# RobotLocomotion/pytorch-dense-correspondence

Measured on AMD Instinct MI355X. Metric: training images/sec, 640x480 D=3 ResNet34-8s, higher is better.
Workload: dtype f32 (f16x3 products)

## Files before the change

include/dcn_hip.h:

```cpp
#ifndef DCN_HIP_H
#define DCN_HIP_H

#include <stddef.h>
#include <stdint.h>

#ifdef __cplusplus
extern "C" {
#endif

#define DCN_OK 0
#define DCN_E_INVALID (-1)
#define DCN_E_LAUNCH (-2)
#define DCN_E_UNSUPPORTED (-3)

const char* dcn_version(void);

void dcn_reload_env(void);

void dcn_release_pooled_buffers(void);


enum { DCN_LIST_MATCH = 0, DCN_LIST_MASKED = 1, DCN_LIST_BACKGROUND = 2, DCN_LIST_BLIND = 3, DCN_NUM_LISTS = 4 };

enum {
    DCN_COMPOSE_WITHIN_SCENE = 0,
    DCN_COMPOSE_DIFFERENT_OBJECT = 1,
    DCN_COMPOSE_ACROSS_SCENE = 2,
    DCN_COMPOSE_RAW_SUMS = 3
};

typedef struct dcn_loss_config {
    float margin[DCN_NUM_LISTS];
    int32_t invert[DCN_NUM_LISTS];
    int32_t pixel_weight[DCN_NUM_LISTS];
    float m_pixel;
    int32_t image_width;
    float match_loss_weight;
    float non_match_loss_weight;
    int32_t scale_by_hard_negatives;
    int32_t compose;
} dcn_loss_config;

size_t dcn_loss_workspace_bytes(int num_pairs, int64_t max_list_len);

int dcn_contrastive_loss_forward(const float* desc_a, const float* desc_b, int num_pairs, int64_t hw, int d,
                                 const int64_t* idx_a, const int64_t* idx_b, const int64_t* offsets_host,
                                 const int64_t* offsets_dev, const dcn_loss_config* cfg, float* terms, float* sums,
                                 int32_t* hard_neg, float* loss, float* per_term, int32_t* status, void* workspace,
                                 void* stream);

int dcn_contrastive_loss_backward(const float* desc_a, const float* desc_b, int num_pairs, int64_t hw, int d,
                                  const int64_t* idx_a, const int64_t* idx_b, const int64_t* offsets_host,
                                  const int64_t* offsets_dev, const dcn_loss_config* cfg, const float* sums,
                                  const int32_t* hard_neg, const float* grad_loss, const float* pair_grad,
                                  float* grad_a, float* grad_b, void* stream);

size_t dcn_loss_saved_floats(int64_t total_pairs, int d);
int dcn_contrastive_loss_forward_save(const float* desc_a, const float* desc_b, int num_pairs, int64_t hw, int d,
                                      const int64_t* idx_a, const int64_t* idx_b, const int64_t* offsets_host,
                                      const int64_t* offsets_dev, const dcn_loss_config* cfg, float* terms, float* sums,
                                      int32_t* hard_neg, float* loss, float* per_term, int32_t* status, void* workspace,
                                      float* pair_records, void* stream);
int dcn_contrastive_loss_backward_saved(int num_pairs, int64_t hw, int d, const int64_t* idx_a, const int64_t* idx_b,
                                        const int64_t* offsets_host, const int64_t* offsets_dev, const dcn_loss_config* cfg,
                                        const int32_t* hard_neg, const float* grad_loss, const float* pair_records,
                                        int prefilled, float* grad_a, float* grad_b, void* stream);

size_t dcn_loss_exact_workspace_bytes(int num_pairs, int64_t hw, int d);
int dcn_contrastive_loss_backward_saved_exact(int num_pairs, int64_t hw, int d, const int64_t* idx_a, const int64_t* idx_b,
                                              const int64_t* offsets_host, const int64_t* offsets_dev,
                                              const dcn_loss_config* cfg, const int32_t* hard_neg, const float* grad_loss,
                                              const float* pair_records, void* workspace, float* grad_a, float* grad_b,
                                              void* stream);
int dcn_fill_bytes(void* p, int byte_value, size_t n, void* stream);

#define DCN_LOSS_NUM_TYPES 5
#define DCN_LOSS_BAD_INDEX 1
#define DCN_LOSS_BAD_TYPE 2
#define DCN_LOSS_BAD_BOUNDS 4
#define DCN_LOSS_BAD_PIXEL_LAYOUT 8
int dcn_contrastive_loss_mixed_forward(const float* desc_a, const float* desc_b, int num_pairs, int64_t hw, int d,
                                       const int64_t* idx_a, const int64_t* idx_b, const int64_t* offsets_dev,
                                       const int32_t* types_dev, const dcn_loss_config* cfgs, int64_t max_list_len,
                                       int64_t max_pair_len, int64_t capacity, float* terms, float* sums, int32_t* hard_neg,
                                       float* loss, int32_t* num_valid, int32_t* status, void* workspace, float* pair_records,
                                       void* stream);
int dcn_contrastive_loss_mixed_backward_saved(int num_pairs, int64_t hw, int d, const int64_t* idx_a, const int64_t* idx_b,
                                              const int64_t* offsets_dev, const int32_t* types_dev, const dcn_loss_config* cfgs,
                                              int64_t max_list_len, int64_t max_pair_len, int64_t capacity,
                                              const int32_t* hard_neg, const int32_t* num_valid, const float* grad_loss,
                                              const float* pair_records, int prefilled, float* grad_a, float* grad_b,
                                              void* stream);
int dcn_contrastive_loss_mixed_backward_saved_exact(int num_pairs, int64_t hw, int d, const int64_t* idx_a, const int64_t* idx_b,
                                                    const int64_t* offsets_dev, const int32_t* types_dev,
                                                    const dcn_loss_config* cfgs, int64_t max_list_len, int64_t max_pair_len,
                                                    int64_t capacity, const int32_t* hard_neg, const int32_t* num_valid,
                                                    const float* grad_loss, const float* pair_records, void* workspace,
                                                    float* grad_a, float* grad_b, void* stream);

size_t dcn_triplet_loss_workspace_bytes(int64_t n);
int dcn_triplet_loss_forward(const float* desc_a, const float* desc_b, int64_t hw, int d, const int64_t* non_a,
                             const int64_t* match_b, const int64_t* non_b, int64_t n, int64_t n_match, float alpha,
                             float* loss, int32_t* status, void* workspace, void* stream);
int dcn_triplet_loss_backward(const float* desc_a, const float* desc_b, int64_t hw, int d, const int64_t* non_a,
                              const int64_t* match_b, const int64_t* non_b, int64_t n, int64_t n_match, float alpha,
                              const float* grad_loss, float* grad_a, float* grad_b, void* stream);


typedef struct dcn_plan dcn_plan;

int dcn_plan_create(const char* arch, int base_width, int n, int h, int w, int d, dcn_plan** out);
int dcn_plan_create_grouped(const char* arch, int base_width, int n, int groups, int h, int w, int d, dcn_plan** out);
void dcn_plan_destroy(dcn_plan* plan);
int dcn_plan_forget_saved(dcn_plan* plan, const void* saved);
int dcn_plan_num_forward_records(const dcn_plan* plan);

#define DCN_CONV_FP32 0
#define DCN_CONV_F16X3 1
int dcn_plan_set_conv_mode(dcn_plan* plan, int mode);
int dcn_plan_conv_mode(const dcn_plan* plan);

int dcn_plan_num_params(const dcn_plan* plan);
int dcn_plan_num_bn(const dcn_plan* plan);
int dcn_plan_param_info(const dcn_plan* plan, int i, char* name, int name_cap, int64_t shape[4], int* ndim);
int dcn_plan_bn_info(const dcn_plan* plan, int j, char* name, int name_cap, int64_t* channels);

int dcn_plan_fused_bn_backward(const dcn_plan* plan);

int dcn_plan_num_activation_slots(const dcn_plan* plan);
size_t dcn_plan_activation_absmax_offset(const dcn_plan* plan);

int dcn_plan_num_grad_buckets(const dcn_plan* plan);
int dcn_plan_grad_bucket_first_param(const dcn_plan* plan, int k);
int dcn_plan_stream_wait_grad_bucket(dcn_plan* plan, int k, void* stream);

size_t dcn_plan_saved_bytes(const dcn_plan* plan);
size_t dcn_plan_workspace_bytes(const dcn_plan* plan);
double dcn_plan_forward_flops(const dcn_plan* plan);

int dcn_backbone_forward(dcn_plan* plan, const float* image, const float* const* params,
                         float* const* bn_running, float momentum, float eps, int training, int normalize,
                         float* descriptors, void* saved, void* workspace, void* stream);

int dcn_backbone_forward_pair(dcn_plan* plan, const float* image_a, const float* image_b, const float* const* params,
                              float* const* bn_running, float momentum, float eps, int training, int normalize,
                              float* descriptors, void* saved, void* workspace, void* stream);

int dcn_plan_profile_begin(dcn_plan* plan);
int dcn_plan_profile_end(dcn_plan* plan, double ms[2], int64_t launches[2], double flops[2]);
int dcn_plan_profile_end3(dcn_plan* plan, double ms[3], int64_t launches[3], double flops[3]);
enum {
    DCN_PROF_GEMM = 0,
    DCN_PROF_WGRAD = 1,
    DCN_PROF_GEMM_HL = 2,
    DCN_PROF_BN_APPLY = 3,
    DCN_PROF_BN_BWD_REDUCE = 4,
    DCN_PROF_BN_BWD_APPLY = 5,
    DCN_PROF_BN_FINALIZE = 6,
    DCN_PROF_RESAMPLE = 7,
    DCN_PROF_OTHER = 8,
    DCN_PROF_NCAT = 9
};
int dcn_plan_profile_end_all(dcn_plan* plan, double ms[DCN_PROF_NCAT], int64_t launches[DCN_PROF_NCAT],
                             double work[DCN_PROF_NCAT]);

int dcn_backbone_backward(dcn_plan* plan, const float* grad_descriptors, const float* const* params,
                          const void* saved, void* workspace, float* const* grads, int normalize, void* stream);
int dcn_backbone_backward_pair(dcn_plan* plan, const float* grad_a, const float* grad_b, const float* const* params,
                               const void* saved, void* workspace, float* const* grads, int normalize, void* stream);


typedef struct dcn_conv_desc {
    int32_t n, hin, win, cin;
    int32_t hout, wout, cout;
    int32_t kh, kw, stride, pad, dil;
    int32_t ldc;
    int32_t group_rows;
} dcn_conv_desc;

int dcn_conv_forward(const dcn_conv_desc* c, const float* in, const float* w, const float* bias, float* out,
                     float* bn_partial, void* workspace, void* stream);
size_t dcn_conv_gemm_workspace(const dcn_conv_desc* c, int dgrad);
int dcn_conv_num_mtiles(const dcn_conv_desc* c);
int dcn_conv_dgrad(const dcn_conv_desc* c, const float* dout, const float* wt, const float* add, float* din,
                   void* workspace, void* stream);
int dcn_conv_wgrad(const dcn_conv_desc* c, const float* in, const float* dout, float* dw, void* slabs, void* stream);
size_t dcn_conv_wgrad_workspace(const dcn_conv_desc* c);
int dcn_transpose_weight(const float* w, float* wt, int cout, int taps, int cin, int ldn, void* stream);

int dcn_f16_kpad(int k);
int dcn_split_rows_f16(const float* w, void* hi, void* lo, int64_t rows, int k, float scale, void* stream);
int dcn_conv_num_mtiles_f16(const dcn_conv_desc* c);
size_t dcn_conv_gemm_workspace_f16(const dcn_conv_desc* c, int dgrad);
int dcn_conv_forward_f16(const dcn_conv_desc* c, const float* in, const float* in_absmax, const void* w_hi, const void* w_lo,
                         float w_scale, const float* bias, float* out, float* bn_partial, void* workspace, void* stream);
int dcn_conv_dgrad_f16(const dcn_conv_desc* c, const float* dout, const void* wt_hi, const void* wt_lo, float w_scale,
                       const float* dout_absmax, const float* add, float* din, void* workspace, void* stream);
int dcn_conv_dgrad_bn_num_mtiles_f16(const dcn_conv_desc* c);
int dcn_conv_dgrad_bn_f16(const dcn_conv_desc* c, const float* dout, const void* wt_hi, const void* wt_lo, float w_scale,
                          const float* dout_absmax, const float* add, float* din, const float* bn_x,
                          const unsigned char* relu_mask, const float* bn_stats, float* bn_partial, void* workspace,
                          void* stream);

int dcn_split_weights_checked_f16(int n, const float* const* w, const float* const* row_scale, void* const* hi, void* const* lo,
                                  const int* cout, const int* taps, const int* cin, float scale, int* status, void* stream);

int dcn_conv_hl_eligible(const dcn_conv_desc* c, int dgrad);
int dcn_conv_num_mtiles_hl(const dcn_conv_desc* c);
int dcn_conv_tile_rows_hl(const dcn_conv_desc* c, int dgrad);
size_t dcn_conv_gemm_workspace_hl(const dcn_conv_desc* c, int dgrad);
int dcn_conv_hl_shape_info(const dcn_conv_desc* c, int dgrad, int* info6);
int dcn_split_act_hl32(const float* src, const float* absmax, void* dst, int64_t rows, int channels, void* stream);
int dcn_split_weights_hl32(int n, const float* const* w, void* const* out, const int* cout, const int* taps, const int* cin,
                           const int* ldn, int transposed, float scale, void* stream);
int dcn_conv_forward_hl(const dcn_conv_desc* c, const void* in_hl, const float* in_absmax, const void* w_hl, float w_scale,
                        const float* bias, float* out, float* bn_partial, void* workspace, void* stream);
int dcn_conv_dgrad_hl(const dcn_conv_desc* c, const void* dout_hl, const void* wt_hl, float w_scale, const float* dout_absmax,
                      const float* add, float* din, void* workspace, void* stream);

int dcn_conv_wgrad_hl_eligible(const dcn_conv_desc* c);
int dcn_conv_wgrad_hl_kind(const dcn_conv_desc* c);
size_t dcn_conv_wgrad_workspace_hl(const dcn_conv_desc* c);
int dcn_conv_wgrad_hl(const dcn_conv_desc* c, const void* x_hl, const float* x_absmax, const void* dout_hl,
                      const float* dout_absmax, float* dw, void* slabs, void* stream);

int dcn_split_stem_weights_f16(const float* w4, void* hi, void* lo, int cout, float scale, void* stream);
int dcn_conv_stem_forward_f16(const dcn_conv_desc* c, const float* in, const float* in_absmax, const void* w_hi, const void* w_lo,
                              float w_scale, float* out, float* bn_partial, void* stream);

int dcn_split_weights_f16(int n, const float* const* w, void* const* hi, void* const* lo, const int* cout, const int* taps,
                          const int* cin, const int* ldn, int transposed, float scale, void* stream);

int dcn_split_weights_scaled_f16(int n, const float* const* w, const float* const* row_scale, void* const* hi,
                                 void* const* lo, const int* cout, const int* taps, const int* cin, const int* ldn,
                                 int transposed, float scale, void* stream);
int dcn_conv_forward_fused_f16(const dcn_conv_desc* c, const float* in, const float* in_absmax, const void* w_hi,
                               const void* w_lo, float w_scale, const float* bias, const float* add, int relu, float* out,
                               float* out_absmax, void* workspace, void* stream);

int dcn_split_act_f16(const float* src, void* xs, int64_t n, void* stream);
size_t dcn_grad_blocked_bytes(int m, int ld);
int dcn_split_grad_blocked_f16(const float* dy, int m, int ld, const float* absmax, void* dq, void* stream);
int dcn_conv_wgrad_f16(const dcn_conv_desc* c, const void* xs, int xs_is_fp32, const float* x_absmax, const void* dq,
                       const float* dout_absmax, float* dw, void* slabs, void* stream);
size_t dcn_conv_wgrad_workspace_f16(const dcn_conv_desc* c);

int dcn_bn_forward(const float* x, const float* bn_partial, int mtiles, int c, int64_t rows, const float* gamma,
                   const float* beta, float* running_mean, float* running_var, float momentum, float eps, int training,
                   const float* res, int relu, float* y, unsigned char* relu_mask, float* stats, void* stream);
size_t dcn_bn_backward_workspace(int64_t rows, int c);
int dcn_bn_backward(const float* dy, const unsigned char* relu_mask, const float* x, const float* stats, const float* gamma,
                    int c, int64_t rows, float* dgamma, float* dbeta, float* dx, float* g_out, void* workspace,
                    void* stream);
int dcn_bn_backward_from_partial(const float* dy, const float* bn_partial, int mtiles, const float* x, const float* stats,
                                 const float* gamma, int c, int64_t rows, float* dgamma, float* dbeta, float* dx,
                                 void* workspace, void* stream);
size_t dcn_bn_backward_full_workspace(int64_t rows, int c, int groups);
int dcn_bn_backward_full(const float* dy, const float* dy2, const float* relu_out, const unsigned char* relu_mask,
                         const float* x, const float* stats, const float* gamma, int c, int64_t rows, int groups,
                         float* dgamma, float* dbeta, float* dx, float* g_out, float* absmax, void* dq, void* hl_dx,
                         int keep_dx, void* workspace, void* stream);
int dcn_maxpool_forward(const float* in, int n, int hin, int win, int c, float* out, unsigned char* argmax, void* stream);
int dcn_maxpool_backward(const float* gout, const unsigned char* argmax, int n, int hin, int win, int c, float* gin,
                         void* stream);

int dcn_upsample_forward(const float* low, int n, int hl, int wl, int ldl, int d, int h, int w, int normalize,
                         float* out, void* stream);
int dcn_upsample_backward(const float* gout, int n, int hl, int wl, int ldl, int d, int h, int w, float* glow,
                          float* tmp, void* stream);
size_t dcn_upsample_backward_tmp_bytes(int n, int hl, int w, int d);

int dcn_maxpool_forward_full(const float* in, const float* bn_stats, int groups, int n, int hin, int win, int c, float* out,
                             unsigned char* argmax, unsigned char* relu_mask, void* stream);
int dcn_maxpool_backward_full(const float* gout, const float* gout2, const unsigned char* argmax, int n, int hin, int win, int c,
                              float* gin, void* stream);
int dcn_normalize_backward(const float* low, int n, int hl, int wl, int ldl, int d, int h, int w, const float* gout, float* gv,
                           void* stream);
int dcn_upsample_backward_full(const float* gout, const float* gout_b, int n, int hl, int wl, int ldl, int d, int h, int w,
                               float* glow, float* tmp, float* absmax, void* stream);
int dcn_image_to_nhwc4(const float* img, int n, int hw, float* out, float* absmax, void* stream);
int dcn_pad_c3_to_c4(const float* src, float* dst, int64_t rows, void* stream);
int dcn_unpad_c4_to_c3(const float* src, float* dst, int64_t rows, void* stream);
int dcn_pad_rows(const float* src, float* dst, int64_t rows, int d, int ld, void* stream);
int dcn_column_sums(const float* m, int64_t rows, int ld, int d, float* out, void* stream);

size_t dcn_match_statistics_workspace(int q);
int dcn_match_statistics(const float* res, int64_t hw, int w, int d, const float* queries, const int64_t* gt_idx, int q,
                         const unsigned char* mask, int64_t* best_idx, float* best_dist, int32_t* count, float* dist_sum,
                         float* gt_dist, void* workspace, void* stream);

int dcn_find_best_match(const float* res, int64_t hw, int d, const float* queries, int q, const unsigned char* mask,
                        int64_t* best_idx, float* best_dist, float* norm_diffs, void* workspace, void* stream);
size_t dcn_find_best_match_workspace(int q);

size_t dcn_find_correspondences_workspace(int64_t n);
int dcn_find_correspondences(const uint16_t* depth_a, const uint16_t* depth_b, int h, int w, const float* K,
                             const float* K_inv, const float* pose_a, const float* pose_b_inv, const int64_t* cand_u,
                             const int64_t* cand_v, int64_t n, int64_t* out_ua, int64_t* out_va, float* out_ub,
                             float* out_vb, int64_t* out_count, void* workspace, void* stream);
size_t dcn_mask_nonzero_workspace(int64_t hw);
int dcn_mask_nonzero(const float* mask, int64_t hw, int64_t* list, int64_t* count, void* workspace, void* stream);
int dcn_sample_pixels(const float* rand, int64_t n, int w, int h, const int64_t* list, const int64_t* count, float* u,
                      float* v, void* stream);

int dcn_adam_step(int n, void* const* param, const void* const* grad, void* const* exp_avg, void* const* exp_avg_sq,
                  const int64_t* numel, double lr, double beta1, double beta2, double eps, double weight_decay,
                  int64_t step, void* stream);

#define DCN_AUG_PARAM_WORDS 16
#define DCN_AUG_FLIP_V 1
#define DCN_AUG_FLIP_H 2
#define DCN_AUG_RANDOMIZE 4
#define DCN_AUG_GRADIENT 8
#define DCN_AUG_VERTICAL 16
#define DCN_AUG_NOISE 32
#define DCN_UV_INT64 0
#define DCN_UV_FLOAT32 1
int dcn_augment_images(int n, int h, int w, const uint8_t* rgb_a, const uint8_t* rgb_b, const uint8_t* mask_a,
                       const uint8_t* mask_b, const int32_t* params, const uint8_t* noise, const float* mean,
                       const float* std, float* net_a, float* net_b, uint8_t* rgb_out_a, uint8_t* rgb_out_b,
                       float* mask_out_a, float* mask_out_b, void* stream);
int dcn_flip_planes(const void* in, void* out, int64_t planes, int h, int w, int bytes_per_pixel, int flip_v, int flip_h,
                    void* stream);
int dcn_flip_uv(int uv_dtype, const void* u_in, const void* v_in, void* u_out, void* v_out, int64_t count, int n_images,
                const int64_t* offsets, const int32_t* params, int flags, int h, int w, void* stream);

#define DCN_MERGE_FG_A 0
#define DCN_MERGE_FG_B 1
#define DCN_MERGE_DROP_EMPTY 1
#define DCN_MERGE_BAD_INDEX 1
#define DCN_MERGE_BAD_OFFSETS 2
int dcn_merge_images(int n, int frames, int h, int w, const int32_t* foreground, const uint8_t* rgb_a1, const uint8_t* rgb_b1,
                     const uint8_t* rgb_a2, const uint8_t* rgb_b2, const uint8_t* mask_a1, const uint8_t* mask_b1,
                     const uint8_t* mask_a2, const uint8_t* mask_b2, const float* mean, const float* std, float* net_1,
                     float* net_2, float* mask_1, float* mask_2, uint8_t* rgb_1, uint8_t* rgb_2, void* stream);
size_t dcn_merge_prune_workspace(int n, int64_t count_a, int64_t count_b);
int dcn_merge_prune(int n, int h, int w, const int32_t* foreground, const uint8_t* mask_a1, const uint8_t* mask_b1,
                    const uint8_t* mask_a2, const uint8_t* mask_b2, const int64_t* u_a1, const int64_t* v_a1,
                    const int64_t* u_a2, const int64_t* v_a2, const int64_t* offsets_a, int64_t count_a, const int64_t* u_b1,
                    const int64_t* v_b1, const int64_t* u_b2, const int64_t* v_b2, const int64_t* offsets_b, int64_t count_b,
                    int flags, int64_t* u_1, int64_t* v_1, int64_t* u_2, int64_t* v_2, int64_t* offsets, uint8_t* empty,
                    int32_t* status, void* workspace, void* stream);

#define DCN_SAMPLE_CAM_FLOATS 50
#define DCN_SAMPLE_SITES 6
#define DCN_SAMPLE_SITE_CAND 0
#define DCN_SAMPLE_SITE_MASKED 1
#define DCN_SAMPLE_SITE_BACKGROUND 2
#define DCN_SAMPLE_SITE_BLIND 3
#define DCN_SAMPLE_SITE_ACROSS_A 4
#define DCN_SAMPLE_SITE_ACROSS_B 5
#define DCN_SAMPLE_ONLY_OFF_MASK 1
#define DCN_SAMPLE_MASK_INV 2
#define DCN_SAMPLE_BAD_INDEX 1
#define DCN_SAMPLE_BAD_DRAWS 2
#define DCN_SAMPLE_BAD_OFFSETS 4
size_t dcn_sample_workspace(int n, int h, int w, int64_t attempts, int64_t match_slots);
int dcn_within_scene_samples(int n, int h, int w, const uint16_t* depth_a, const uint16_t* depth_b, const uint8_t* mask_a,
                             const uint8_t* mask_b, const float* cams, int64_t attempts, int k_masked, int k_background,
                             int flags, const int32_t* aug_params, const int64_t* seeds, const float* rand,
                             const int64_t* rand_offsets, int data_type, int64_t* idx_a, int64_t* idx_b, int64_t capacity,
                             int64_t* offsets, uint8_t* empty, int32_t* type, int32_t* status, void* workspace, void* stream);
int dcn_complete_samples(int n, int h, int w, const int64_t* u_a, const int64_t* v_a, const void* u_b, const void* v_b,
                         int uv_b_dtype, const int64_t* list_offsets, int64_t count, const uint8_t* mask_a,
                         const uint8_t* mask_b, int k_masked, int k_background, int flags, const int32_t* aug_params,
                         const int64_t* seeds, const float* rand, const int64_t* rand_offsets, int data_type, int64_t* idx_a,
                         int64_t* idx_b, int64_t capacity, int64_t* offsets, uint8_t* empty, int32_t* type, int32_t* status,
                         void* workspace, void* stream);
int dcn_across_scene_samples(int n, int h, int w, const uint8_t* mask_a, const uint8_t* mask_b, int64_t num_samples,
                             const int32_t* aug_params, const int64_t* seeds, const float* rand, const int64_t* rand_offsets,
                             int data_type, int64_t* idx_a, int64_t* idx_b, int64_t capacity, int64_t* offsets, uint8_t* empty,
                             int32_t* type, int32_t* status, void* workspace, void* stream);

#define DCN_CONCAT_MAX_GROUPS 8
int dcn_concat_samples(int groups, const int* n, const int64_t* const* idx_a, const int64_t* const* idx_b,
                       const int64_t* const* offsets, const int64_t* capacity_in, const int32_t* const* status_in,
                       int64_t* idx_a_out, int64_t* idx_b_out, int64_t capacity, int64_t* offsets_out, int32_t* status,
                       void* stream);

#define DCN_SYNTHETIC_DATA_TYPE 4
#define DCN_SYNTHETIC_SITES 4
#define DCN_SYNTHETIC_SITE_CAND_A 0
#define DCN_SYNTHETIC_SITE_CAND_B 1
#define DCN_SYNTHETIC_SITE_MASKED 2
#define DCN_SYNTHETIC_SITE_BACKGROUND 3
size_t dcn_synthetic_workspace(int n, int h, int w, int64_t attempts);
int dcn_synthetic_samples(int n, int h, int w, const uint16_t* depth, const uint8_t* mask, const uint8_t* rgb,
                          const float* cams, int64_t attempts, int k_masked, int k_background, int flags,
                          const int32_t* foreground, const uint8_t* empty_in, const int64_t* seeds, const float* rand,
                          const int64_t* rand_offsets, const float* mean, const float* std, float* net_1, float* net_2,
                          float* mask_1, float* mask_2, int64_t* idx_a, int64_t* idx_b, int64_t capacity, int64_t* offsets,
                          uint8_t* empty, int32_t* type, int32_t* status, void* workspace, void* stream);

struct dcn_frame_store {
    int64_t num_frames;
    int32_t num_scenes, num_objects, num_multi, h, w;
    const uint8_t* rgb;
    const uint16_t* depth;
    const uint8_t* mask;
    const int32_t* scene_first_frame;
    const int32_t* scene_object;
    const int32_t* object_scene_offsets;
    const int32_t* object_scenes;
    const int32_t* multi_scenes;
    const float* scene_cams;
    const double* poses;
};
#define DCN_FRAME_CAM_FLOATS 18
#define DCN_FRAME_SLOTS 4
#define DCN_FRAME_DRAW_OBJECT_A 0
#define DCN_FRAME_DRAW_OBJECT_B 1
#define DCN_FRAME_DRAW_SCENE_A 2
#define DCN_FRAME_DRAW_SCENE_B 3
#define DCN_FRAME_DRAW_SCENE_B2 4
#define DCN_FRAME_DRAW_FRAME_A 5
#define DCN_FRAME_DRAW_FRAME_B 6
#define DCN_FRAME_DRAW_HEADER 8
#define DCN_FRAME_BAD_INDEX 1
#define DCN_FRAME_BAD_DRAWS 2
#define DCN_FRAME_NO_CANDIDATES 4
int dcn_select_frames(int n, int data_type, const struct dcn_frame_store* store, int num_attempts, double threshold,
                      double angle_threshold, const int64_t* seeds, const int32_t* draws, int32_t* frames, uint8_t* empty,
                      int32_t* scenes, int32_t* objects, int32_t* status, void* stream);
int dcn_gather_frames(int n, int frames_per_pair, const struct dcn_frame_store* store, const int32_t* frames,
                      const uint8_t* empty, uint8_t* rgb, uint16_t* depth, uint8_t* mask, float* cams, int32_t* status,
                      void* stream);

#define DCN_EVAL_COLUMNS 13
#define DCN_EVAL_COL_NORM_DIFF_DESCRIPTOR_GROUND_TRUTH 0
#define DCN_EVAL_COL_NORM_DIFF_DESCRIPTOR 1
#define DCN_EVAL_COL_NORM_DIFF_DESCRIPTOR_MASKED 2
#define DCN_EVAL_COL_NORM_DIFF_GROUND_TRUTH_3D 3
#define DCN_EVAL_COL_NORM_DIFF_PRED_3D 4
#define DCN_EVAL_COL_NORM_DIFF_PRED_3D_MASKED 5
#define DCN_EVAL_COL_PIXEL_MATCH_ERROR_L2 6
#define DCN_EVAL_COL_PIXEL_MATCH_ERROR_L2_MASKED 7
#define DCN_EVAL_COL_PIXEL_MATCH_ERROR_L1 8
#define DCN_EVAL_COL_FRACTION_CLOSER 9
#define DCN_EVAL_COL_FRACTION_CLOSER_MASKED 10
#define DCN_EVAL_COL_AVERAGE_L2_FALSE_POSITIVES 11
#define DCN_EVAL_COL_AVERAGE_L2_FALSE_POSITIVES_MASKED 12
#define DCN_EVAL_BAD_INDEX 1
#define DCN_EVAL_BAD_OFFSETS 2
#define DCN_EVAL_BAD_DRAWS 4
#define DCN_EVAL_BAD_FRAME 8
size_t dcn_eval_matches_workspace(int n, int h, int w, int64_t attempts);
int dcn_eval_matches(int n, int h, int w, const uint16_t* depth_a, const uint16_t* depth_b, const uint8_t* mask_a,
                     const float* cams, int64_t attempts, const int64_t* seeds, const float* rand, const int64_t* rand_offsets,
                     int num_matches, const int32_t* match_order, const int64_t* order_seeds, int64_t* u_a, int64_t* v_a,
                     float* u_b, float* v_b, int64_t* offsets, int32_t* totals, int32_t* status, void* workspace, void* stream);
size_t dcn_match_statistics_pairs_workspace(int64_t max_rows);
int dcn_match_statistics_pairs(int p, int h, int w, int d, const float* res_a, const float* res_b, const uint8_t* mask_b,
                               const uint16_t* depth_a, const uint16_t* depth_b, const float* cams, const int64_t* u_a,
                               const int64_t* v_a, const float* u_b, const float* v_b, const int64_t* offsets, int64_t max_rows,
                               int max_pair_rows, double* columns, uint8_t* is_valid, int32_t* pred_uv, int32_t* closer,
                               int32_t* row_pair, int32_t* mask_pixels, int32_t* status, void* workspace, void* stream);

#define DCN_ACROSS_TOO_FEW_MASK_PIXELS 16
size_t dcn_across_object_queries_workspace(int p, int h, int w);
int dcn_across_object_queries(int p, int h, int w, int d, const uint8_t* mask_a, const float* res_a, int q,
                              const int32_t* sample_order, const int64_t* order_seeds, int64_t* u_a, int64_t* v_a,
                              float* queries, int64_t* offsets, int32_t* mask_pixels, int32_t* status, void* workspace,
                              void* stream);
size_t dcn_best_match_pairs_workspace(int64_t max_rows);
int dcn_best_match_pairs(int p, int h, int w, int d, const float* res_b, const float* queries, const int64_t* offsets,
                         int64_t max_rows, int max_pair_rows, float* norm_diff, int32_t* best_uv, int32_t* row_pair,
                         int32_t* status, void* workspace, void* stream);

int dcn_reproject_pixels(int v, const struct dcn_frame_store* store, const float* kcam, const int32_t* requests,
                         uint8_t* found, float* u2, float* v2, int32_t* uv, int32_t* status, void* stream);
size_t dcn_match_statistics_groups_workspace(int64_t max_rows);
int dcn_match_statistics_groups(int g, int h, int w, int d, const float* res_b, const uint8_t* mask_b, const uint16_t* depth_b,
                                const float* queries, const int64_t* u_a, const int64_t* v_a, const uint16_t* depth_q,
                                const float* u_b, const float* v_b, const float* cams, const uint8_t* keep,
                                const int64_t* offsets, int64_t max_rows, int max_group_rows, double* columns,
                                uint8_t* is_valid, int32_t* pred_uv, int32_t* closer, int32_t* row_pair, int32_t* mask_pixels,
                                int32_t* status, void* workspace, void* stream);
int dcn_match_statistics_groups_wide(int g, int h, int w, int d, const float* res_b, const uint8_t* mask_b,
                                     const uint16_t* depth_b, const float* queries, const int64_t* u_a, const int64_t* v_a,
                                     const uint16_t* depth_q, const float* u_b, const float* v_b, const float* cams,
                                     const uint8_t* keep, const int64_t* offsets, int64_t max_rows, int max_group_rows,
                                     int64_t strip_pixels, double* columns, uint8_t* is_valid, int32_t* pred_uv, int32_t* closer,
                                     int32_t* row_pair, int32_t* mask_pixels, int32_t* status, void* workspace, void* stream);

size_t dcn_descriptor_statistics_workspace(int n, int h, int w, int d);
int dcn_descriptor_statistics(int n, int h, int w, int d, const float* res, const uint8_t* mask, float* per_image,
                              int32_t* mask_pixels, void* workspace, void* stream);
int dcn_descriptor_statistics_combine(int n, int d, const float* per_image, const int32_t* mask_pixels, int num_images,
                                      float* stats, int32_t* used, void* stream);

struct dcn_train_state {
    int32_t active;
    int32_t reserved;
    int64_t t;
    double lr;
    float step_size;
    float bc2_sqrt;
    int64_t num_active;
    int64_t num_skipped;
};
#define DCN_TRAIN_LOG_COLUMNS 16
int dcn_train_advance(struct dcn_train_state* state, const int32_t* types, int B, int64_t iteration,
                      int64_t steps_between_decay, double decay, double beta1, double beta2, void* stream);
int dcn_adam_step_guarded(int n, void* const* param, const void* const* grad, void* const* exp_avg, void* const* exp_avg_sq,
                          const int64_t* numel, double eps, double weight_decay, double beta1, double beta2,
                          const struct dcn_train_state* state, void* stream);
int dcn_guarded_copy(int n, void* const* dst, const void* const* src, const int64_t* bytes,
                     const struct dcn_train_state* state, int when_active, void* stream);
int dcn_train_log(double* history, int64_t row, int64_t iteration, const struct dcn_train_state* state, const float* loss,
                  const float* terms, const int32_t* types, int B, void* stream);
int dcn_train_advance_ranks(struct dcn_train_state* state, const int32_t* types_all , int G, int B, int rank,
                            float* weight_out , int64_t iteration, int64_t steps_between_decay, double decay,
                            double beta1, double beta2, void* stream);
int dcn_train_log_ranks(double* history, int64_t row, int64_t iteration, const struct dcn_train_state* state,
                        const float* gathered , const int32_t* types_all , int G, int B,
                        void* stream);

#define DCN_CURVE_SUMMARY_DOUBLES 8
#define DCN_CURVE_EMPTY 1
#define DCN_CURVE_NAN 2
#define DCN_CURVE_NONFINITE 4
int dcn_eval_curves(int c, int64_t rows, int64_t ld, const double* values ,
                    const int32_t* row_pair , const uint8_t* drop_nan ,
                    int num_bins, int64_t* cumcount , double* cdf ,
                    double* summary , int32_t* status , void* stream);

#define DCN_PICTURE_EMPTY_RANGE 1
#define DCN_HEAT_WORKSPACE_BYTES 2048
#define DCN_NORM_NONE 0
#define DCN_NORM_PAIR 1
#define DCN_NORM_MASKED_PAIR 2
#define DCN_NORM_STATS 3
#define DCN_NORM_STATS_MASKED 4
#define DCN_NORM_SCALAR 5
struct dcn_picture_family {
    int32_t mode;
    int32_t picture_channels;
    int32_t channel[3];
    int32_t reserved;
    const double* stats;
    void* normed;
    void* picture;
    int64_t side_stride, pair_stride;
};
size_t dcn_descriptor_ranges_workspace(int p, int h, int w, int d);
int dcn_descriptor_ranges(int p, int h, int w, int d, const float* res_a, const float* res_b, const uint8_t* mask_a,
                          const uint8_t* mask_b, float* image_ranges, float* pair_ranges, float* scalar_ranges,
                          int32_t* status, void* workspace, void* stream);
int dcn_descriptor_normalize(int p, int h, int w, int d, const float* res_a, const float* res_b, const uint8_t* mask_a,
                             const uint8_t* mask_b, const float* pair_ranges, const float* scalar_ranges,
                             const struct dcn_picture_family* families , void* stream);
int dcn_heat_maps(int p, int h, int w, int d, const float* res_b, const float* queries, const int64_t* offsets,
                  int64_t max_rows, float variance, const uint8_t* colour_table, uint8_t* out, int32_t* status,
                  void* workspace, void* stream);

#ifdef __cplusplus
}
#endif
#endif
```

pytorch-dense-correspondence_amd/csrc/backbone_engine.hip:

```cpp
#include <algorithm>
#include <cstdio>
#include <cstdlib>
#include <cstring>
#include <mutex>
#include <string>
#include <vector>

#include "dcn_tuning.h"
#include "elementwise_kernels.h"

namespace {

using dcn::ceil_div;

struct ConvL {
    double flops = 0;
    dcn_conv_desc d;
    int w = -1, b = -1;
    int bn = -1;
    size_t x = 0;
    int cin_true = 0;
    size_t wsplit = 0;
    size_t whl = 0;
    bool hl_any = false;
// ... 525 lines not shown
            obs.begin = [](void* c, int cat, double bytes, hipStream_t s) { prof_open(*(dcn_plan*)c, cat, bytes, s); };
            obs.end = [](void* c, hipStream_t s) { prof_close(*(dcn_plan*)c, s); };
            if (on) dcn::launch_observer = &obs;
        }
        ~ObserverGuard() { if (on) dcn::launch_observer = outer; }
    };
    template <class F> int other(F&& launch) { return timed(DCN_PROF_OTHER, 0.0, launch); }

    void* SK(const ConvL& c, int dgrad, Kernel k) const {
        const size_t need = k == Kernel::FP32 ? dcn_conv_gemm_workspace(&c.d, dgrad) : k == Kernel::HL ? dcn_conv_gemm_workspace_hl(&c.d, dgrad)
                                                                                                       : dcn_conv_gemm_workspace_f16(&c.d, dgrad);
        return need <= p.sk_bytes ? (void*)(ws + p.w_sk) : nullptr;
    }
    float* S(size_t off) const { return saved + off; }
    float* A(int a) const { return (p.conv_mode == DCN_CONV_F16X3 && a >= 0) ? saved + p.s_actmax + a : nullptr; }
    unsigned char* M(size_t off) const {
        for (const auto& m : p.relu_masks)
            if (m.first == off) return (unsigned char*)(saved + m.second);
        return nullptr;
    }
    float* Wk(size_t off) const { return ws + off; }
    const float* P(int i) const { return params[i]; }

    int conv_fwd(const ConvL& c, const float* in, const float* w, const float* bias, float* out, float* part) {
        const Kernel k = rt[c.idx].fwd;
        if (k == Kernel::FP32)
            return timed(0, c.flops, [&] { return dcn_conv_forward(&c.d, in, w, bias, out, part, SK(c, 0, k), st); });
        if (k == Kernel::STEM8) {
            _Float16* hi = (_Float16*)Wk(p.w_stem8);
            return timed(0, c.flops, [&] {
                return dcn_conv_stem_forward_f16(&c.d, in, A(c.in_act), hi, hi + (size_t)p.base * 224, kWeightScale, out, part, st);
            });
        }
        if (k == Kernel::HL) {
            return timed(2, c.flops, [&] {
                const float* img = saved_hl_of(in);
                if (!img) {
                    int k = hl_src[0] == in ? 0 : (hl_src[1] == in ? 1 : -1);
                    if (k < 0) {
                        k = 0;
                        DCN_TRY(dcn_split_act_hl32(in, A(c.in_act), hlbuf(0), (int64_t)c.d.n * c.d.hin * c.d.win, c.d.cin, st));
                        hl_src[0] = in;
                    }
                    img = hlbuf(k);
                }
                return dcn_conv_forward_hl(&c.d, img, A(c.in_act), whl(c), kWeightScale, bias, out, part, SK(c, 0, k), st);
            });
        }
        return timed(0, c.flops, [&] {
            return dcn_conv_forward_f16(&c.d, in, A(c.in_act), wimg(p.w_wh, c), wimg(p.w_wl, c), kWeightScale, bias, out, part,
                                        SK(c, 0, k), st);
        });
    }

    float* wh_over = nullptr;
    float* wl_over = nullptr;
    float* whl_over = nullptr;
    void* wimg(size_t plane, const ConvL& c) const {
        float* base = plane == p.w_wh ? (wh_over ? wh_over : Wk(p.w_wh)) : (wl_over ? wl_over : Wk(p.w_wl));
        return (void*)((_Float16*)base + c.wsplit);
    }

    int ensure_saved_hl(const float* y, float* slot, int64_t rows, int C, int act) {
        if (!slot || dcn::tuning().hl_producers != 0) return DCN_OK;
        return other([&] { return dcn_split_act_hl32(y, A(act), slot, rows, C, st); });
    }
    void* whl(const ConvL& c) const { return (void*)((whl_over ? whl_over : Wk(p.w_whl)) + c.whl); }
    float* hlbuf(int k) const { return Wk(k == 0 ? p.w_hl : p.w_hl2); }
    void* hl_image_for(const float* y, int k, const ConvL* consumer_a, const ConvL* consumer_b = nullptr, float* slot = nullptr) {
        if (slot) {
            hl_saved.emplace_back(y, slot);
            return dcn::tuning().hl_producers != 0 ? (void*)slot : nullptr;
        }
        if (dcn::tuning().hl_producers == 0) return nullptr;
        const bool want = (consumer_a && rt[consumer_a->idx].fwd == Kernel::HL) || (consumer_b && rt[consumer_b->idx].fwd == Kernel::HL);
        if (!want) return nullptr;
        hl_src[k] = y;
        return hlbuf(k);
    }
    int fwd_mtiles(const ConvL& c) const {
        const Kernel k = rt[c.idx].fwd;
        return k == Kernel::FP32 ? dcn_conv_num_mtiles(&c.d) : k == Kernel::HL ? dcn_conv_num_mtiles_hl(&c.d) : dcn_conv_num_mtiles_f16(&c.d);
    }
    int split_hl_weights(bool transposed) {
        std::vector<const float*> w;
        std::vector<void*> out;
        std::vector<int> cout, taps, cin, ldn;
        for (const ConvL& c : p.convs) {
            if ((transposed ? rt[c.idx].dgrad : rt[c.idx].fwd) != Kernel::HL) continue;
            w.push_back(P(c.w));
            out.push_back(whl(c));
            cout.push_back(c.d.cout); taps.push_back(c.d.kh * c.d.kw); cin.push_back(c.d.cin); ldn.push_back(c.d.ldc);
        }
        if (w.empty()) return DCN_OK;
        return other([&] {
            return dcn_split_weights_hl32((int)w.size(), w.data(), out.data(), cout.data(), taps.data(), cin.data(), ldn.data(),
                                          transposed ? 1 : 0, kWeightScale, st);
        });
    }

    int split_all_weights(bool transposed, const float* stem_w, bool fold_bn = false) {
        const int n = (int)p.convs.size();
        std::vector<const float*> w, rs;
        std::vector<void*> hi, lo;
        std::vector<int> cout, taps, cin, ldn;
        for (int i = 0; i < n; ++i) {
            const ConvL& c = p.convs[i];
            if (transposed && i == p.stem) continue;
            w.push_back(i == p.stem ? stem_w : P(c.w));
            rs.push_back(fold_bn && c.bn >= 0 ? S(p.bns[c.bn].stats) : nullptr);
            hi.push_back(wimg(p.w_wh, c));
            lo.push_back(wimg(p.w_wl, c));
            cout.push_back(c.d.cout); taps.push_back(c.d.kh * c.d.kw); cin.push_back(c.d.cin); ldn.push_back(c.d.ldc);
        }
        if (!transposed)
            return other([&] {
                return dcn_split_weights_checked_f16((int)w.size(), w.data(), fold_bn ? rs.data() : nullptr, hi.data(), lo.data(),
                                                     cout.data(), taps.data(), cin.data(), kWeightScale,
                                                     (int*)(S(p.s_actmax) + p.n_act), st);
            });
        return other([&] {
            return dcn_split_weights_scaled_f16((int)w.size(), w.data(), nullptr, hi.data(), lo.data(), cout.data(), taps.data(),
                                                cin.data(), ldn.data(), 1, kWeightScale, st);
        });
    }

    int conv_fused(const ConvL& c, const float* in, const float* add, int relu, float* out, int out_act) {
        const float* shift = S(p.bns[c.bn].stats) + p.bns[c.bn].C;
        return timed(0, c.flops, [&] {
            return dcn_conv_forward_fused_f16(&c.d, in, A(c.in_act), wimg(p.w_wh, c), wimg(p.w_wl, c), kWeightScale, shift, add,
                                              relu, out, A(out_act), SK(c, 0, Kernel::F16), st);
        });
    }

    int conv_bn(const ConvL& c, const float* in, const float* w, float* const* bn_running, float momentum, float eps,
                int training, int out_act, int res_act = -1) {
        float* part = training ? Wk(p.w_part) : nullptr;
        DCN_TRY(conv_fwd(c, in, w, nullptr, S(c.x), part));
        const BnL& b = p.bns[c.bn];
        float* stats = S(b.stats);
        float* rm = bn_running ? bn_running[2 * b.idx] : nullptr;
        float* rv = bn_running ? bn_running[2 * b.idx + 1] : nullptr;
        if (!training && (!rm || !rv)) return DCN_E_INVALID;
        const int mtiles = fwd_mtiles(c);
        dcn::launch_bn_finalize(part, mtiles / p.groups, p.groups, b.C, (double)(b.rows / p.groups), P(b.g),
                                P(b.b), rm, rv, momentum, eps, training, stats, training ? A(out_act) : nullptr,
                                training ? A(res_act) : nullptr, st);
        return DCN_OK;
    }
};

}

extern "C" int dcn_plan_create(const char* arch, int base_width, int n, int h, int w, int d, dcn_plan** out) {
    return dcn_plan_create_grouped(arch, base_width, n, 1, h, w, d, out);
}
extern "C" int dcn_plan_create_grouped(const char* arch, int base_width, int n, int groups, int h, int w, int d,
                                       dcn_plan** out) {
    if (!arch || !out || n < 1 || h < 8 || w < 8 || d < 1 || base_width < 4 || (base_width % 4) || groups < 1 ||
        groups > 2 || (n % groups))
        return DCN_E_INVALID;
    dcn_plan* p = new dcn_plan();
    p->arch = arch; p->N = n; p->H = h; p->W = w; p->D = d; p->base = base_width; p->groups = groups;
    const dcn::Tuning& tune = dcn::tuning();
    if (tune.conv_mode_invalid) { delete p; return DCN_E_INVALID; }
    if (tune.conv_mode >= 0) p->conv_mode = tune.conv_mode;
    const int rc = build_plan(*p);
    if (rc != DCN_OK) { delete p; return rc; }
    *out = p;
    return DCN_OK;
}
extern "C" int dcn_plan_forget_saved(dcn_plan* plan, const void* saved) {
    if (!plan) return DCN_E_INVALID;
    int n = 0;
    for (size_t i = 0; i < plan->fwd_records.size();)
        if (plan->fwd_records[i].saved == saved) { plan->fwd_records.erase(plan->fwd_records.begin() + i); ++n; }
        else ++i;
    return n;
}

extern "C" int dcn_plan_num_forward_records(const dcn_plan* plan) {
    return plan ? (int)plan->fwd_records.size() : DCN_E_INVALID;
}

extern "C" void dcn_plan_destroy(dcn_plan* plan) {
    if (!plan) return;
    for (hipEvent_t e : plan->prof_ev) hipEventDestroy(e);
    for (hipEvent_t e : {plan->ev_dq[0], plan->ev_dq[1], plan->ev_wg[0], plan->ev_wg[1], plan->ev_join, plan->ev_ws[0], plan->ev_ws[1]})
        if (e) hipEventDestroy(e);
    for (hipEvent_t e : plan->ev_bucket)
        if (e) hipEventDestroy(e);
    if (plan->ev_bucket_side) hipEventDestroy(plan->ev_bucket_side);
    delete plan;
}
extern "C" int dcn_plan_set_conv_mode(dcn_plan* plan, int mode) {
    if (!plan || (mode != DCN_CONV_FP32 && mode != DCN_CONV_F16X3)) return DCN_E_INVALID;
    plan->conv_mode = mode;
    return DCN_OK;
}
extern "C" int dcn_plan_conv_mode(const dcn_plan* plan) { return plan ? plan->conv_mode : DCN_E_INVALID; }
extern "C" int dcn_plan_profile_begin(dcn_plan* plan) {
    if (!plan) return DCN_E_INVALID;
    plan->prof_on = true;
    plan->prof_used = 0;
    plan->prof_cat.clear();
    plan->prof_flops.clear();
    return DCN_OK;
}
extern "C" int dcn_plan_profile_end_all(dcn_plan* plan, double ms[DCN_PROF_NCAT], int64_t launches[DCN_PROF_NCAT],
                                        double work[DCN_PROF_NCAT]) {
    if (!plan || !ms || !launches || !work) return DCN_E_INVALID;
    plan->prof_on = false;
    for (int c = 0; c < DCN_PROF_NCAT; ++c) { ms[c] = 0; launches[c] = 0; work[c] = 0; }
    int rc = DCN_OK;
    for (size_t i = 0; i < plan->prof_cat.size(); ++i) {
        hipEvent_t e0 = plan->prof_ev[2 * i], e1 = plan->prof_ev[2 * i + 1];
        float t = 0.f;
        if (hipEventSynchronize(e1) != hipSuccess || hipEventElapsedTime(&t, e0, e1) != hipSuccess) { rc = DCN_E_LAUNCH; break; }
        const int c = plan->prof_cat[i];
        if (c < 0 || c >= DCN_PROF_NCAT) continue;
        for (int k : {c == DCN_PROF_GEMM_HL ? (int)DCN_PROF_GEMM : c, c == DCN_PROF_GEMM_HL ? (int)DCN_PROF_GEMM_HL : -1}) {
            if (k < 0) continue;
            ms[k] += (double)t;
            launches[k] += 1;
            work[k] += plan->prof_flops[i];
        }
    }
    plan->prof_used = 0;
    plan->prof_cat.clear();
    plan->prof_flops.clear();
    return rc;
}
extern "C" int dcn_plan_profile_end3(dcn_plan* plan, double ms[3], int64_t launches[3], double flops[3]) {
    if (!ms || !launches || !flops) return DCN_E_INVALID;
    double m[DCN_PROF_NCAT], f[DCN_PROF_NCAT];
    int64_t n[DCN_PROF_NCAT];
    const int rc = dcn_plan_profile_end_all(plan, m, n, f);
    for (int c = 0; c < 3; ++c) { ms[c] = m[c]; launches[c] = n[c]; flops[c] = f[c]; }
    return rc;
}
extern "C" int dcn_plan_profile_end(dcn_plan* plan, double ms[2], int64_t launches[2], double flops[2]) {
    if (!ms || !launches || !flops) return DCN_E_INVALID;
    double m3[3], f3[3];
    int64_t n3[3];
    const int rc = dcn_plan_profile_end3(plan, m3, n3, f3);
    for (int c = 0; c < 2; ++c) { ms[c] = m3[c]; launches[c] = n3[c]; flops[c] = f3[c]; }
    return rc;
}
extern "C" int dcn_plan_num_params(const dcn_plan* plan) { return plan ? (int)plan->params.size() : DCN_E_INVALID; }
extern "C" int dcn_plan_num_bn(const dcn_plan* plan) { return plan ? (int)plan->bns.size() : DCN_E_INVALID; }
extern "C" int dcn_plan_param_info(const dcn_plan* plan, int i, char* name, int name_cap, int64_t shape[4], int* ndim) {
    if (!plan || i < 0 || i >= (int)plan->params.size() || !name || name_cap < 2 || !shape || !ndim) return DCN_E_INVALID;
    const ParamInfo& pi = plan->params[i];
    snprintf(name, (size_t)name_cap, "%s", pi.name.c_str());
    for (int k = 0; k < 4; ++k) shape[k] = pi.shape[k];
    *ndim = pi.ndim;
    return DCN_OK;
}
extern "C" int dcn_plan_bn_info(const dcn_plan* plan, int j, char* name, int name_cap, int64_t* channels) {
    if (!plan || j < 0 || j >= (int)plan->bns.size() || !name || name_cap < 2 || !channels) return DCN_E_INVALID;
    snprintf(name, (size_t)name_cap, "%s", plan->bns[j].name.c_str());
    *channels = plan->bns[j].C;
    return DCN_OK;
}
extern "C" int dcn_plan_num_grad_buckets(const dcn_plan* plan) { return plan ? (int)plan->bucket_first.size() : DCN_E_INVALID; }
extern "C" int dcn_plan_grad_bucket_first_param(const dcn_plan* plan, int k) {
    if (!plan || k < 0 || k >= (int)plan->bucket_first.size()) return DCN_E_INVALID;
    return plan->bucket_first[k];
}
extern "C" int dcn_plan_stream_wait_grad_bucket(dcn_plan* plan, int k, void* stream) {
    if (!plan || k < 0 || k >= (int)plan->bucket_first.size()) return DCN_E_INVALID;
    if (plan->bucket_state != 1) return DCN_E_UNSUPPORTED;
    return hipStreamWaitEvent((hipStream_t)stream, plan->ev_bucket[k], 0) == hipSuccess ? DCN_OK : DCN_E_LAUNCH;
}
extern "C" int dcn_plan_fused_bn_backward(const dcn_plan* plan) { return plan ? plan->fused_bn_bwd : DCN_E_INVALID; }
extern "C" int dcn_plan_num_activation_slots(const dcn_plan* plan) { return plan ? plan->n_act : DCN_E_INVALID; }
extern "C" size_t dcn_plan_activation_absmax_offset(const dcn_plan* plan) { return plan ? plan->s_actmax * sizeof(float) : 0; }
extern "C" size_t dcn_plan_saved_bytes(const dcn_plan* plan) { return plan ? plan->saved_floats * sizeof(float) : 0; }
extern "C" size_t dcn_plan_workspace_bytes(const dcn_plan* plan) { return plan ? plan->ws_floats * sizeof(float) : 0; }
extern "C" double dcn_plan_forward_flops(const dcn_plan* plan) { return plan ? plan->flops : 0.0; }

extern "C" int dcn_column_sums(const float* m, int64_t rows, int ld, int d, float* out, void* stream) {
    if (!m || !out || rows < 1 || d < 1 || ld < d) return DCN_E_INVALID;
    hipLaunchKernelGGL(colsum_kernel, dim3(d), dim3(1024), 0, (hipStream_t)stream, m, rows, ld, out);
    return dcn::check_launch();
}

namespace {

int forward_impl(dcn_plan* plan, const float* image, const float* image_b, const float* const* params,
                 float* const* bn_running, float momentum, float eps, int training, int normalize,
                 float* descriptors, void* saved, void* workspace, void* stream) {
    if (!plan || !image || !params || !descriptors || !saved || !workspace) return DCN_E_INVALID;
    dcn_plan& p = *plan;
    if (image_b && p.groups != 2) return DCN_E_INVALID;
    const std::vector<ConvRoute> routes = conv_routes(p, p.conv_mode);
    Run R{p, params, (float*)saved, (float*)workspace, (hipStream_t)stream, routes};
    Run::ObserverGuard observe(p);
    hipStream_t st = R.st;
    const int N = p.N;

    DCN_TRY(R.other([&] { return dcn::fill_bytes_async(R.S(p.s_actmax), 0, ((size_t)p.n_act + 1) * sizeof(float), st); }));
    const ConvL& stem = p.convs[p.stem];
    if (image_b) {
        dcn::launch_nchw3_to_nhwc4(image, R.S(p.s_in4), N / 2, p.H * p.W, R.A(stem.in_act), st);
        dcn::launch_nchw3_to_nhwc4(image_b, R.S(p.s_in4) + (size_t)(N / 2) * p.H * p.W * 4, N / 2, p.H * p.W, R.A(stem.in_act), st);
    } else {
        dcn::launch_nchw3_to_nhwc4(image, R.S(p.s_in4), N, p.H * p.W, R.A(stem.in_act), st);
    }
    dcn::launch_pad_c3_to_c4(R.P(stem.w), R.Wk(p.w_wstem), (int64_t)p.base * 49, st);
    dcn_plan::FwdRecord rec;
    rec.saved = saved;
    rec.conv_mode = p.conv_mode;
    rec.mid_hl_only.assign(p.convs.size(), 0);
    const bool fused_eval = !training && p.conv_mode == DCN_CONV_F16X3;
    const bool f16_mode = p.conv_mode == DCN_CONV_F16X3;
    if (fused_eval) {
        if (!bn_running) return DCN_E_INVALID;
        for (const BnL& b : p.bns) {
            if (!bn_running[2 * b.idx] || !bn_running[2 * b.idx + 1]) return DCN_E_INVALID;
            dcn::launch_bn_finalize(nullptr, 0, p.groups, b.C, (double)(b.rows / p.groups), R.P(b.g), R.P(b.b),
                                    bn_running[2 * b.idx], bn_running[2 * b.idx + 1], momentum, eps, 0, R.S(b.stats), nullptr,
                                    nullptr, st);
        }
        DCN_TRY(R.split_all_weights(false, R.Wk(p.w_wstem), true));
        DCN_TRY(R.conv_fused(stem, R.S(p.s_in4), nullptr, 1, R.S(p.s_stem_y), p.blocks[0].act_in));
        {
            const BnL& b = p.bns[stem.bn];
            const int hp = (stem.d.hout + 2 - 3) / 2 + 1, wp = (stem.d.wout + 2 - 3) / 2 + 1;
            dcn::launch_maxpool_fwd(R.S(p.s_stem_y), R.S(p.s_pool), (unsigned char*)R.S(p.s_argmax), N, stem.d.hout,
                                    stem.d.wout, hp, wp, b.C, st);
        }
        for (const BlockL& blk : p.blocks) {
            const float* in = R.S(blk.in);
            const float* cur = in;
            for (int i = 0; i + 1 < blk.nconv; ++i) {
                DCN_TRY(R.conv_fused(p.convs[blk.conv[i]], cur, nullptr, 1, R.S(blk.mid[i]), blk.act_mid[i]));
                cur = R.S(blk.mid[i]);
            }
            const ConvL& last = p.convs[blk.conv[blk.nconv - 1]];
            const float* res = in;
            if (blk.down >= 0) {
                const ConvL& dc = p.convs[blk.down];
                DCN_TRY(R.conv_fused(dc, in, nullptr, 0, R.S(dc.x), -1));
                res = R.S(dc.x);
            }
            DCN_TRY(R.conv_fused(last, cur, res, 1, R.S(blk.out), blk.act_out));
        }
    } else {
    const bool stem8 = routes[p.stem].fwd == Kernel::STEM8;
    bool hoist = training && f16_mode && stem8 && !p.prof_on && dcn::tuning().wsplit_overlap != 0 && ensure_side(p);
    if (hoist) {
        hipStreamCaptureStatus cs = hipStreamCaptureStatusNone;
        if (hipStreamIsCapturing(st, &cs) != hipSuccess || cs != hipStreamCaptureStatusNone) hoist = false;
    }
    SideFork side(p, st, p.ev_ws[1]);
    if (p.conv_mode == DCN_CONV_F16X3) {
        if (hoist) {
            Run Rs{p, params, (float*)saved, (float*)workspace, p.side, routes};
            if (!side.fork(p.ev_ws[0])) return DCN_E_LAUNCH;
            DCN_TRY(Rs.split_all_weights(false, Rs.Wk(p.w_wstem)));
            DCN_TRY(Rs.split_hl_weights(false));
            Rs.wh_over = Rs.S(p.s_wht); Rs.wl_over = Rs.S(p.s_wlt); Rs.whl_over = Rs.S(p.s_whlt);
            DCN_TRY(Rs.split_all_weights(true, nullptr));
            DCN_TRY(Rs.split_hl_weights(true));
            rec.wt_saved = true;
            if (!side.record(p.ev_ws[1], p.side)) return DCN_E_LAUNCH;
        } else {
            DCN_TRY(R.split_all_weights(false, R.Wk(p.w_wstem)));
            DCN_TRY(R.split_hl_weights(false));
        }
    }
    if (stem8) {
        _Float16* hi = (_Float16*)R.Wk(p.w_stem8);
        DCN_TRY(R.other([&] { return dcn_split_stem_weights_f16(R.Wk(p.w_wstem), hi, hi + (size_t)p.base * 224, p.base, kWeightScale, st); }));
    }
    DCN_TRY(R.conv_bn(stem, R.S(p.s_in4), R.Wk(p.w_wstem), bn_running, momentum, eps, training, p.blocks[0].act_in));
    {
        const BnL& b = p.bns[stem.bn];
        const float* s = R.S(b.stats);
        const int hp = (stem.d.hout + 2 - 3) / 2 + 1, wp = (stem.d.wout + 2 - 3) / 2 + 1;
        if (dcn::tuning().stem_pool_fused != 0) {
            dcn::launch_maxpool_fwd(R.S(stem.x), R.S(p.s_pool), (unsigned char*)R.S(p.s_argmax), N, stem.d.hout, stem.d.wout, hp,
                                    wp, b.C, st, s, p.groups, R.M(p.s_stem_y));
        } else {
            dcn::launch_bn_apply({.x = R.S(stem.x), .stats = s, .C = b.C, .rows = b.rows, .groups = p.groups, .y = R.S(p.s_stem_y),
                                  .relu_mask = R.M(p.s_stem_y)}, st);
            dcn::launch_maxpool_fwd(R.S(p.s_stem_y), R.S(p.s_pool), (unsigned char*)R.S(p.s_argmax), N, stem.d.hout,
                                    stem.d.wout, hp, wp, b.C, st);
        }
    }
    if (hoist && !side.join_wait(p.ev_ws[1])) return DCN_E_LAUNCH;
    if (training && f16_mode && p.blocks[0].has_hl_in) {
        const BlockL& b0 = p.blocks[0];
        R.hl_saved.emplace_back(R.S(b0.in), R.S(b0.hl_in));
        DCN_TRY(R.other([&] { return dcn_split_act_hl32(R.S(b0.in), R.A(b0.act_in), R.S(b0.hl_in), b0.in_rows, b0.in_c, st); }));
    }
    for (const BlockL& blk : p.blocks) {
        const float* in = R.S(blk.in);
        const float* cur = in;
        if (blk.down >= 0) {
            const ConvL& dc = p.convs[blk.down];
            DCN_TRY(R.conv_bn(dc, in, R.P(dc.w), bn_running, momentum, eps, training, blk.act_down));
        }
        for (int i = 0; i < blk.nconv; ++i) {
            const ConvL& c = p.convs[blk.conv[i]];
            if (i + 1 < blk.nconv) {
                DCN_TRY(R.conv_bn(c, cur, R.P(c.w), bn_running, momentum, eps, training, blk.act_mid[i]));
                const BnL& b = p.bns[c.bn];
                const float* s = R.S(b.stats);
                float* slot = (training && f16_mode && blk.has_hl_mid[i]) ? R.S(blk.hl_mid[i]) : nullptr;
                const ConvL& nxt = p.convs[blk.conv[i + 1]];
                void* hl = training ? R.hl_image_for(R.S(blk.mid[i]), 1, &nxt, nullptr, slot) : nullptr;
                const bool hl_only = hl && slot && hl == (void*)slot && (b.C % 32) == 0 && dcn::tuning().hl_only_mid != 0 &&
                                     routes[nxt.idx].fwd == Kernel::HL && routes[nxt.idx].wgrad == Kernel::HL;
                rec.mid_hl_only[nxt.idx] = hl_only ? 1 : 0;
                dcn::launch_bn_apply({.x = R.S(c.x), .stats = s, .C = b.C, .rows = b.rows, .groups = p.groups,
                                      .y = hl_only ? nullptr : R.S(blk.mid[i]), .relu_mask = R.M(blk.mid[i]), .hl_out = hl,
                                      .hl_absmax = R.A(blk.act_mid[i])}, st);
                DCN_TRY(R.ensure_saved_hl(R.S(blk.mid[i]), slot, b.rows, b.C, blk.act_mid[i]));
                cur = R.S(blk.mid[i]);
            } else {
                DCN_TRY(R.conv_bn(c, cur, R.P(c.w), bn_running, momentum, eps, training, blk.act_out,
                                  blk.down >= 0 ? blk.act_down : blk.act_in));
            }
        }
        const ConvL& last = p.convs[blk.conv[blk.nconv - 1]];
        const BnL& bl = p.bns[last.bn];
        const float* sl = R.S(bl.stats);
        const BlockL* nb = (&blk != &p.blocks.back()) ? &blk + 1 : nullptr;
        float* slot = (training && f16_mode && nb && nb->has_hl_in) ? R.S(nb->hl_in) : nullptr;
        void* hl = (training && nb) ? R.hl_image_for(R.S(blk.out), 0, &p.convs[nb->conv[0]], nb->down >= 0 ? &p.convs[nb->down] : nullptr,
                                                     slot)
                                    : nullptr;
        const ConvL* dc = blk.down >= 0 ? &p.convs[blk.down] : nullptr;
        dcn::launch_bn_apply({.x = R.S(last.x), .stats = sl, .C = bl.C, .rows = bl.rows, .groups = p.groups,
                              .res = dc ? R.S(dc->x) : in, .res_stats = dc ? R.S(p.bns[dc->bn].stats) : nullptr, .y = R.S(blk.out),
                              .relu_mask = R.M(blk.out), .hl_out = hl, .hl_absmax = R.A(blk.act_out)}, st);
        DCN_TRY(R.ensure_saved_hl(R.S(blk.out), slot, bl.rows, bl.C, blk.act_out));
    }
    }
    const ConvL& fc = p.convs[p.fc];
    const size_t low_bytes = (size_t)N * p.hl * p.wl * p.Dp * sizeof(float);
    DCN_TRY(R.other([&] { return dcn::fill_bytes_async(R.S(p.s_low), 0, low_bytes, st); }));
    DCN_TRY(R.conv_fwd(fc, R.S(p.blocks.back().out), R.P(fc.w), R.P(fc.b), R.S(p.s_low), nullptr));
    dcn::launch_upsample_fwd(R.S(p.s_low), N, p.hl, p.wl, p.Dp, p.D, p.H, p.W, normalize, descriptors, st);
    DCN_TRY(R.other([&] {
        hipLaunchKernelGGL(act_status_kernel, dim3(1), dim3(64), 0, st, (const float*)R.S(p.s_actmax), p.n_act,
                           (int*)(R.S(p.s_actmax) + p.n_act));
        return dcn::check_launch();
    }));
    if (training) {
        rec.routes = routes;
        dcn_plan_forget_saved(&p, saved);
        if (p.fwd_records.size() >= dcn_plan::kMaxFwdRecords) p.fwd_records.erase(p.fwd_records.begin());
        p.fwd_records.push_back(std::move(rec));
    }
    return dcn::check_launch();
}

}

extern "C" int dcn_backbone_forward(dcn_plan* plan, const float* image, const float* const* params,
                                    float* const* bn_running, float momentum, float eps, int training, int normalize,
                                    float* descriptors, void* saved, void* workspace, void* stream) {
    return forward_impl(plan, image, nullptr, params, bn_running, momentum, eps, training, normalize, descriptors, saved,
                        workspace, stream);
}
extern "C" int dcn_backbone_forward_pair(dcn_plan* plan, const float* image_a, const float* image_b,
                                         const float* const* params, float* const* bn_running, float momentum, float eps,
                                         int training, int normalize, float* descriptors, void* saved, void* workspace,
                                         void* stream) {
    if (!image_b) return DCN_E_INVALID;
    return forward_impl(plan, image_a, image_b, params, bn_running, momentum, eps, training, normalize, descriptors, saved,
                        workspace, stream);
}

namespace {

struct GradImages {
    Run& R;
    SideFork& side;
    const bool overlap;
    struct Slot {
        float* blocked;
        float* hl;
        hipEvent_t written, read;
        const float* blocked_of = nullptr;
        const float* hl_of = nullptr;
        bool reader_pending = false;
    } slot[2];
    int cur = 0, taken = 0;
    GradImages(Run& run, SideFork& fork, bool on)
        : R(run), side(fork), overlap(on),
          slot{{R.Wk(R.p.w_dq), R.hlbuf(0), R.p.ev_dq[0], R.p.ev_wg[0]}, {R.Wk(R.p.w_dq2), R.hlbuf(1), R.p.ev_dq[1], R.p.ev_wg[1]}} {}

    Slot& take() {
        cur = overlap ? (taken & 1) : 0;
        ++taken;
        if (overlap && slot[cur].reader_pending) side.wait(slot[cur].read);
        return slot[cur];
    }
    void wrote(const float* blocked_of, const float* hl_of) {
        if (overlap) side.record(slot[cur].written, R.st);
        slot[cur].blocked_of = blocked_of;
        slot[cur].hl_of = hl_of;
    }
    template <class L> int read_on_side(const ConvL& c, L&& launch) {
        if (!overlap) return R.timed(1, c.flops, [&] { return launch(R.st); });
        side.side_wait(slot[cur].written);
        DCN_TRY(launch(R.p.side));
        side.record(slot[cur].read, R.p.side);
        slot[cur].reader_pending = true;
        return DCN_OK;
    }
    bool has_blocked(const float* dx) const { return slot[cur].blocked_of == dx; }
    const float* blocked() const { return slot[cur].blocked; }
    const float* hl() const { return slot[cur].hl; }

    template <class S> int hl_for_wgrad(const float* dx, S&& split) {
        Slot& s = slot[cur];
        if (s.hl_of == dx) return DCN_OK;
        DCN_TRY(R.other([&] { return split(s.hl); }));
        if (overlap) side.record(s.written, R.st);
        s.hl_of = dx;
        return DCN_OK;
    }
    template <class S> int hl_for_dgrad(const float* dx, S&& split) {
        Slot& s = slot[cur];
        if (s.hl_of == dx) return DCN_OK;
        DCN_TRY(split(s.hl));
        s.hl_of = dx;
        return DCN_OK;
    }
    template <class S, class G> int blocked_in_line(const ConvL& c, S&& split, G&& gemm) {
        float* image = slot[0].blocked;
        DCN_TRY(R.other([&] { return split(image); }));
        return R.timed(1, c.flops, [&] { return gemm(image, R.st); });
    }
};

int backward_impl(dcn_plan* plan, const float* grad_descriptors, const float* grad_b, const float* const* params,
                  const void* saved, void* workspace, float* const* grads, int normalize, void* stream) {
    if (!plan || !grad_descriptors || !params || !saved || !workspace || !grads) return DCN_E_INVALID;
    dcn_plan& p = *plan;
    if (grad_b && p.groups != 2) return DCN_E_INVALID;
    const std::vector<ConvRoute> routes = conv_routes(p, p.conv_mode);
    Run R{p, params, (float*)saved, (float*)workspace, (hipStream_t)stream, routes};
    Run::ObserverGuard observe(p);
    hipStream_t st = R.st;
    const int N = p.N;
    bool wt_have = false;
    {
        const dcn_plan::FwdRecord* rec = nullptr;
        for (size_t i = p.fwd_records.size(); i-- > 0 && !rec;)
            if (p.fwd_records[i].saved == saved) rec = &p.fwd_records[i];
        if (!rec || rec->conv_mode != p.conv_mode) return DCN_E_INVALID;
        wt_have = rec->wt_saved;
        for (const ConvL& c : p.convs) {
            const ConvRoute &now = routes[c.idx], &was = rec->routes[c.idx];
            if (now.wgrad == Kernel::HL && was.wgrad == Kernel::FP32) return DCN_E_INVALID;
            if (rec->mid_hl_only[c.idx] && now.wgrad != Kernel::HL) return DCN_E_INVALID;
            if (now.dgrad == Kernel::HL && was.dgrad != Kernel::HL) wt_have = false;
        }
    }
    float* part = R.Wk(p.w_part);
    float* k123 = R.Wk(p.w_k123);
    float* wt = R.Wk(p.w_wt);
    float* slab = R.Wk(p.w_slab);
    float* amax = R.Wk(p.w_amax);
    const bool f16 = p.conv_mode == DCN_CONV_F16X3;

    bool overlap = f16 && !p.prof_on && ensure_side(p);
    if (overlap) {
        hipStreamCaptureStatus cs = hipStreamCaptureStatusNone;
        if (hipStreamIsCapturing(st, &cs) != hipSuccess || cs != hipStreamCaptureStatusNone) overlap = false;
    }
    const bool buckets = ensure_bucket_events(p);
    SideFork side(p, st, p.ev_join);
    GradImages img(R, side, overlap);
    const bool fuse_red = f16 && dcn::tuning().bn_bwd_fused != 0;
    p.fused_bn_bwd = 0;
    const float* red_dy = nullptr;
    int red_tiles = 0;
    auto bn_bwd = [&](const ConvL& c, const float* dy, const float* relu_out, float* dx, float* g_out, const float* dy2 = nullptr) {
        const BnL& b = p.bns[c.bn];
        const unsigned char* mask = relu_out ? R.M((size_t)(relu_out - R.saved)) : nullptr;
        GradImages::Slot& slot = img.take();
        const int tiles = (red_dy == dy && dy) ? red_tiles : 0;
        red_dy = nullptr;
        if (tiles > 0) { relu_out = nullptr; mask = nullptr; g_out = nullptr; ++p.fused_bn_bwd; }
        const bool prod = f16 && dcn::tuning().hl_producers != 0;
        const bool hl_d = prod && !fuse_red && routes[c.idx].dgrad == Kernel::HL;
        const bool hl_w = prod && routes[c.idx].wgrad == Kernel::HL;
        const bool want_blocked = f16 && !hl_w, want_hl = hl_d || hl_w;
        dcn::launch_bn_bwd({.dy = dy, .dy2 = dy2, .relu_out = relu_out, .relu_mask = mask, .x = R.S(c.x), .stats = R.S(b.stats),
                            .gamma = R.P(b.g), .C = b.C, .rows = b.rows, .groups = p.groups, .partial = part, .k123 = k123,
                            .reduced_tiles_per_group = tiles, .dgamma = grads[b.g], .dbeta = grads[b.b], .dx = dx, .g_out = g_out,
                            .absmax = f16 ? amax + c.idx : nullptr, .dq = want_blocked ? slot.blocked : nullptr,
                            .hl_dx = want_hl ? slot.hl : nullptr, .skip_fp32_dx = hl_d,
                            .lean = (overlap && dcn::tuning().bn_bwd_lean != 0) ? dcn::tuning().bn_bwd_lean_mask : 0}, st);
        img.wrote(want_blocked ? dx : nullptr, want_hl ? dx : nullptr);
    };
    auto split_hl = [&](const ConvL& c, const float* dx, float* image) {
        return dcn_split_act_hl32(dx, amax + c.idx, image, (int64_t)c.d.n * c.d.hout * c.d.wout, c.d.ldc, st);
    };
    auto wgrad = [&](const ConvL& c, const float* in, const float* dx, float* dw) -> int {
        const Kernel k = routes[c.idx].wgrad;
        if (k == Kernel::FP32) return R.timed(1, c.flops, [&] { return dcn_conv_wgrad(&c.d, in, dx, dw, slab, st); });
        if (k == Kernel::HL) {
            DCN_TRY(img.hl_for_wgrad(dx, [&](float* image) { return split_hl(c, dx, image); }));
            return img.read_on_side(c, [&](hipStream_t s) {
                return dcn_conv_wgrad_hl(&c.d, R.S(c.hl_x), R.A(c.in_act), img.hl(), amax + c.idx, dw, slab, s);
            });
        }
        auto gemm = [&](const float* image, hipStream_t s) {
            return dcn_conv_wgrad_f16(&c.d, in, 1, R.A(c.in_act), image, amax + c.idx, dw, slab, s);
        };
        if (!img.has_blocked(dx))
            return img.blocked_in_line(c, [&](float* image) {
                return dcn_split_grad_blocked_f16(dx, c.d.n * c.d.hout * c.d.wout, c.d.ldc, amax + c.idx, image, st);
            }, gemm);
        return img.read_on_side(c, [&](hipStream_t s) { return gemm(img.blocked(), s); });
    };
    auto dgrad = [&](const ConvL& c, const float* dx, const float* add, float* din, const ConvL* bn_of = nullptr,
                     const float* relu_out = nullptr) -> int {
        const ConvRoute& r = routes[c.idx];
        if (r.dgrad == Kernel::FP32) {
            DCN_TRY(R.other([&] { return dcn_transpose_weight(R.P(c.w), wt, c.d.cout, c.d.kh * c.d.kw, c.d.cin, c.d.ldc, st); }));
            return R.timed(0, c.flops, [&] { return dcn_conv_dgrad(&c.d, dx, wt, add, din, R.SK(c, 1, Kernel::FP32), st); });
        }
        if (fuse_red && bn_of) {
            const BnL& b = p.bns[bn_of->bn];
            const int tiles = dcn_conv_dgrad_bn_num_mtiles_f16(&c.d);
            if (tiles > 0 && tiles % p.groups == 0 && b.C == c.d.cin && b.rows == (int64_t)c.d.n * c.d.hin * c.d.win) {
                const unsigned char* mask = relu_out ? R.M((size_t)(relu_out - R.saved)) : nullptr;
                red_dy = din;
                red_tiles = tiles / p.groups;
                return R.timed(0, c.flops, [&] {
                    return dcn_conv_dgrad_bn_f16(&c.d, dx, R.wimg(p.w_wh, c), R.wimg(p.w_wl, c), kWeightScale, amax + c.idx, add,
                                                 din, R.S(bn_of->x), mask, R.S(b.stats), part, R.SK(c, 1, Kernel::F16), st);
                });
            }
        }
        if (r.dgrad == Kernel::HL) {
            return R.timed(2, c.flops, [&] {
                DCN_TRY(img.hl_for_dgrad(dx, [&](float* image) { return split_hl(c, dx, image); }));
                return dcn_conv_dgrad_hl(&c.d, img.hl(), R.whl(c), kWeightScale, amax + c.idx, add, din, R.SK(c, 1, Kernel::HL), st);
            });
        }
        return R.timed(0, c.flops, [&] {
            return dcn_conv_dgrad_f16(&c.d, dx, R.wimg(p.w_wh, c), R.wimg(p.w_wl, c), kWeightScale, amax + c.idx, add, din,
                                      R.SK(c, 1, Kernel::F16), st);
        });
    };
    if (f16) {
        if (wt_have) {
            R.wh_over = R.S(p.s_wht); R.wl_over = R.S(p.s_wlt); R.whl_over = R.S(p.s_whlt);
        } else {
            DCN_TRY(R.split_all_weights(true, nullptr));
            DCN_TRY(R.split_hl_weights(true));
        }
        DCN_TRY(R.other([&] { return dcn::fill_bytes_async(amax, 0, p.convs.size() * sizeof(float), st); }));
    }

    float* glow = R.Wk(p.w_glow);
    if (normalize) {
        if (grad_b) {
            const size_t lo = (size_t)(N / 2) * p.hl * p.wl * p.Dp, hi = (size_t)(N / 2) * p.H * p.W * p.D;
            dcn::launch_normalize_bwd(R.S(p.s_low), N / 2, p.hl, p.wl, p.Dp, p.D, p.H, p.W, grad_descriptors, R.Wk(p.w_gnorm), st);
            dcn::launch_normalize_bwd(R.S(p.s_low) + lo, N / 2, p.hl, p.wl, p.Dp, p.D, p.H, p.W, grad_b, R.Wk(p.w_gnorm) + hi, st);
            grad_b = nullptr;
        } else {
            dcn::launch_normalize_bwd(R.S(p.s_low), N, p.hl, p.wl, p.Dp, p.D, p.H, p.W, grad_descriptors, R.Wk(p.w_gnorm), st);
        }
        grad_descriptors = R.Wk(p.w_gnorm);
    }
    dcn::launch_upsample_bwd(grad_descriptors, N, p.hl, p.wl, p.Dp, p.D, p.H, p.W, R.Wk(p.w_ups), glow,
                             f16 ? amax + p.convs[p.fc].idx : nullptr, st, grad_b);
    const ConvL& fc = p.convs[p.fc];
    const float* feat = R.S(p.blocks.back().out);
    DCN_TRY(wgrad(fc, feat, glow, grads[fc.w]));
    DCN_TRY(R.other([&] {
        hipLaunchKernelGGL(colsum_kernel, dim3(p.D), dim3(1024), 0, st, (const float*)glow, (int64_t)N * p.hl * p.wl, p.Dp,
                           grads[fc.b]);
        return dcn::check_launch();
    }));
    float* dout = R.Wk(p.w_buf[0]);
    float* dnext = R.Wk(p.w_buf[1]);
    float* gbuf = R.Wk(p.w_buf[2]);
    float* dxa = R.Wk(p.w_buf[3]);
    float* dxb = R.Wk(p.w_buf[4]);
    float* dpart = R.Wk(p.w_buf[5]);
    {
        const BlockL& lb = p.blocks.back();
        DCN_TRY(dgrad(fc, glow, nullptr, dout, &p.convs[lb.conv[lb.nconv - 1]], R.S(lb.out)));
    }

    const bool defer_add = dcn::tuning().defer_residual_add != 0 && !fuse_red;
    const float* dout_add = nullptr;
    const float* next_add = nullptr;
    for (int bi = (int)p.blocks.size() - 1; bi >= 0; --bi) {
        const BlockL& blk = p.blocks[bi];
        const float* in = R.S(blk.in);
        const ConvL& last = p.convs[blk.conv[blk.nconv - 1]];
        const float* gres = (red_dy == dout) ? dout : gbuf;
        bn_bwd(last, dout, R.S(blk.out), dxa, gbuf, dout_add);
        dout_add = nullptr;
        float* dx = dxa;
        float* dy = dxb;
        const ConvL* up_bn = bi > 0 ? &p.convs[p.blocks[bi - 1].conv[p.blocks[bi - 1].nconv - 1]] : nullptr;
        const float* up_relu = bi > 0 ? R.S(p.blocks[bi - 1].out) : nullptr;
        for (int i = blk.nconv - 1; i >= 0; --i) {
            const ConvL& c = p.convs[blk.conv[i]];
            const float* cin = i == 0 ? in : R.S(blk.mid[i - 1]);
            DCN_TRY(wgrad(c, cin, dx, grads[c.w]));
            if (i > 0) {
                const ConvL& prev = p.convs[blk.conv[i - 1]];
                DCN_TRY(dgrad(c, dx, nullptr, dy, &prev, R.S(blk.mid[i - 1])));
                bn_bwd(prev, dy, R.S(blk.mid[i - 1]), dx, nullptr);
            } else if (blk.down >= 0) {
                DCN_TRY(dgrad(c, dx, nullptr, dpart));
            } else if (defer_add) {
                DCN_TRY(dgrad(c, dx, nullptr, dnext));
                next_add = gres;
            } else {
                DCN_TRY(dgrad(c, dx, gres, dnext, up_bn, up_relu));
            }
        }
        if (blk.down >= 0) {
            const ConvL& dc = p.convs[blk.down];
            bn_bwd(dc, gres, nullptr, dxa, nullptr);
            DCN_TRY(wgrad(dc, in, dxa, grads[dc.w]));
            if (defer_add) {
                DCN_TRY(dgrad(dc, dxa, nullptr, dnext));
                next_add = dpart;
            } else {
                DCN_TRY(dgrad(dc, dxa, dpart, dnext, up_bn, up_relu));
            }
        }
        dout_add = next_add;
        next_add = nullptr;
        float* t = dout; dout = dnext; dnext = t;
        for (size_t k = 0; k + 1 < p.bucket_block.size(); ++k)
            if (p.bucket_block[k] == bi && buckets) {
                if (overlap) side.join(p.ev_bucket_side);
                side.record(p.ev_bucket[k], st);
            }
    }
    const ConvL& stem = p.convs[p.stem];
    const BnL& sb = p.bns[stem.bn];
    const int hp = (stem.d.hout + 2 - 3) / 2 + 1, wp = (stem.d.wout + 2 - 3) / 2 + 1;
    dcn::launch_maxpool_bwd(dout, (const unsigned char*)R.S(p.s_argmax), dnext, N, stem.d.hout, stem.d.wout, hp, wp, sb.C,
                            st, dout_add);
    bn_bwd(stem, dnext, R.S(p.s_stem_y), dxa, nullptr);
    DCN_TRY(wgrad(stem, R.S(p.s_in4), dxa, R.Wk(p.w_dwstem)));
    if (overlap) side.join(p.ev_join);
    dcn::launch_unpad_c4_to_c3(R.Wk(p.w_dwstem), grads[stem.w], (int64_t)p.base * 49, st);
    if (buckets) side.record(p.ev_bucket.back(), st);
    if (side.failed) return DCN_E_LAUNCH;
    return dcn::check_launch();
}

}

extern "C" int dcn_backbone_backward(dcn_plan* plan, const float* grad_descriptors, const float* const* params,
                                     const void* saved, void* workspace, float* const* grads, int normalize,
                                     void* stream) {
    return backward_impl(plan, grad_descriptors, nullptr, params, saved, workspace, grads, normalize, stream);
}
extern "C" int dcn_backbone_backward_pair(dcn_plan* plan, const float* grad_a, const float* grad_b,
                                          const float* const* params, const void* saved, void* workspace,
                                          float* const* grads, int normalize, void* stream) {
    if (!grad_b) return DCN_E_INVALID;
    return backward_impl(plan, grad_a, grad_b, params, saved, workspace, grads, normalize, stream);
}
```

pytorch-dense-correspondence_amd/csrc/dcn_tuning.h:

```cpp
#pragma once

namespace dcn {

struct Tuning {
    int conv_mode = -1;
    int conv_mode_invalid = 0;
    int backward_overlap = 1;
    int gemm_tile_m = 0;
    int gemm_sk = -1;
    double gemm_sk_min_gain = 20.0;
    int gemm_uni = 1;
    int stem8 = 1;
    int gemm_sk_inline = 1;
    int bn_bwd_fused = 0;
    int defer_residual_add = 1;
    int wgrad_splits = 0;
    int wgrad_tile = 0;
    int wgrad_deep = 4;
    int gemm_hl = 1;
    int hl_min_k = 128;
    int gemm_hl_rows = 0;
    int gemm_hlx = 1;
    int gemm_hlx_kg = 0;
    int gemm_hlx_splits = 0;
    int gemm_hlx_narrow = 1;
    double hlx_cost1 = 1.32, hlx_cost2 = 1.42, hlx_split_cost = 14.0;
    int hl_setprio = 1;
    int hlx_stagger = 1;
    int hlx_counters = 1;
    int wgrad_hl_min_m = 0;
    int wgrad_hl = 1;
    int wgrad_hlr = 1;
    int wgrad_hlr_min_m = 0;
    int wgrad_hlr_pairs = 1;
    int hl_producers = 1;
    int hl_only_mid = 1;
    int stem_pool_fused = 1;
    int bn_reduce_wide = 32;
    int wsplit_overlap = 1;
    int bn_nt = 0;
    int bn_reverse = 0;
    int bn_bwd_lean = 1;
    int bn_bwd_lean_mask = 7;
    int bn_bwd_lean_depth = 3;
    int wgrad_roles = 1;
};

const Tuning& tuning();

}
```

pytorch-dense-correspondence_amd/csrc/dcn_tuning.hip:

```cpp
#include <atomic>
#include <cstdio>
#include <cstdlib>
#include <cstring>
#include <mutex>

#include "dcn_common.h"
#include "dcn_tuning.h"

namespace dcn {
namespace {

Tuning g_tuning;
std::once_flag g_once;
std::mutex g_mu;

void read_env(Tuning& t) {
    t = Tuning();
    if (const char* m = getenv("DCN_CONV_MODE")) {
        if (!strcmp(m, "fp32")) t.conv_mode = DCN_CONV_FP32;
        else if (!strcmp(m, "f16x3")) t.conv_mode = DCN_CONV_F16X3;
        else t.conv_mode_invalid = 1;
    }
    if (const char* e = getenv("DCN_BACKWARD_OVERLAP")) t.backward_overlap = atoi(e) != 0;
    if (const char* e = getenv("DCN_GEMM_TILE_M")) t.gemm_tile_m = atoi(e);
    if (const char* e = getenv("DCN_GEMM_SK")) t.gemm_sk = atoi(e);
    if (const char* e = getenv("DCN_GEMM_SK_MIN_GAIN")) t.gemm_sk_min_gain = atof(e);
    if (const char* e = getenv("DCN_STEM8")) t.stem8 = atoi(e) != 0;
    if (const char* e = getenv("DCN_GEMM_UNI")) t.gemm_uni = atoi(e) != 0;
    if (const char* e = getenv("DCN_GEMM_SK_FIXUP")) t.gemm_sk_inline = strcmp(e, "kernel") != 0;
    if (const char* e = getenv("DCN_BN_BWD_FUSED")) t.bn_bwd_fused = atoi(e) != 0;
    if (const char* e = getenv("DCN_DEFER_RESIDUAL_ADD")) t.defer_residual_add = atoi(e) != 0;
    if (const char* e = getenv("DCN_WGRAD_DEEP")) t.wgrad_deep = atoi(e);
    if (const char* e = getenv("DCN_WGRAD_ROLES")) t.wgrad_roles = atoi(e);
    if (const char* e = getenv("DCN_WGRAD_TILE")) t.wgrad_tile = atoi(e);
    if (const char* e = getenv("DCN_WGRAD_SPLITS")) t.wgrad_splits = atoi(e);
    if (const char* e = getenv("DCN_GEMM_HL")) t.gemm_hl = atoi(e);
    if (const char* e = getenv("DCN_GEMM_HL_ROWS")) t.gemm_hl_rows = atoi(e);
    if (const char* e = getenv("DCN_HL_MIN_K")) { const int v = atoi(e); if (v >= 32) t.hl_min_k = v; }
    if (const char* e = getenv("DCN_GEMM_HLX")) {
        int a = 0, b = 0;
        if (strchr(e, ',')) {
            if (sscanf(e, "%d,%d", &a, &b) == 2) {
                t.gemm_hlx = 1;
                t.gemm_hlx_kg = (a == 1 || a == 2) ? a : 0;
                t.gemm_hlx_splits = b > 0 ? b : 0;
            }
        } else {
            t.gemm_hlx = atoi(e) != 0;
        }
    }
    if (const char* e = getenv("DCN_GEMM_HLX_NARROW")) t.gemm_hlx_narrow = atoi(e) != 0;
    if (const char* e = getenv("DCN_HLX_COST")) {
        double a = 0, b = 0, c = 0;
        if (sscanf(e, "%lf,%lf,%lf", &a, &b, &c) == 3 && a > 0 && b > 0 && c >= 0) { t.hlx_cost1 = a; t.hlx_cost2 = b; t.hlx_split_cost = c; }
    }
    if (const char* e = getenv("DCN_HL_ONLY_MID")) t.hl_only_mid = atoi(e);
    if (const char* e = getenv("DCN_STEM_POOL_FUSED")) t.stem_pool_fused = atoi(e);
    if (const char* e = getenv("DCN_WGRAD_HL")) t.wgrad_hl = atoi(e);
    if (const char* e = getenv("DCN_HL_SETPRIO")) t.hl_setprio = atoi(e) != 0;
    if (const char* e = getenv("DCN_HLX_STAGGER")) { const int v = atoi(e); t.hlx_stagger = (v >= 0 && v <= 2) ? v : 1; }
    if (const char* e = getenv("DCN_HLX_COUNTERS")) t.hlx_counters = atoi(e) != 0;
    if (const char* e = getenv("DCN_WGRAD_HL_MIN_M")) t.wgrad_hl_min_m = atoi(e);
    if (const char* e = getenv("DCN_WGRAD_HLR")) t.wgrad_hlr = atoi(e);
    if (const char* e = getenv("DCN_WGRAD_HLR_MIN_M")) t.wgrad_hlr_min_m = atoi(e);
    if (const char* e = getenv("DCN_WGRAD_HLR_PAIRS")) t.wgrad_hlr_pairs = atoi(e);
    if (const char* e = getenv("DCN_HL_PRODUCERS")) t.hl_producers = atoi(e) != 0;
    if (const char* e = getenv("DCN_BN_REVERSE")) t.bn_reverse = atoi(e);
    if (const char* e = getenv("DCN_BN_NT")) t.bn_nt = atoi(e);
    if (const char* e = getenv("DCN_WSPLIT_OVERLAP")) t.wsplit_overlap = atoi(e) != 0;
    if (const char* e = getenv("DCN_BN_REDUCE_WIDE")) t.bn_reduce_wide = atoi(e);
    if (const char* e = getenv("DCN_BN_BWD_LEAN")) t.bn_bwd_lean = atoi(e) != 0;
    if (const char* e = getenv("DCN_BN_BWD_LEAN_MASK")) t.bn_bwd_lean_mask = atoi(e) & 7;
    if (const char* e = getenv("DCN_BN_BWD_LEAN_DEPTH")) { const int v = atoi(e); t.bn_bwd_lean_depth = v < 1 ? 1 : (v > 3 ? 3 : v); }
}

}

const Tuning& tuning() {
    std::call_once(g_once, [] { read_env(g_tuning); });
    return g_tuning;
}

}

extern "C" void dcn_reload_env(void) {
    (void)dcn::tuning();
    std::lock_guard<std::mutex> lock(dcn::g_mu);
    dcn::read_env(dcn::g_tuning);
}
```

pytorch-dense-correspondence_amd/csrc/elementwise_kernels.h:

```cpp
#pragma once
#include "dcn_common.h"

namespace dcn {

struct LaunchObserver {
    void* ctx;
    void (*begin)(void* ctx, int cat, double bytes, hipStream_t st);
    void (*end)(void* ctx, hipStream_t st);
};
extern thread_local const LaunchObserver* launch_observer;
struct ObservedLaunch {
    hipStream_t st;
    const LaunchObserver* o;
    ObservedLaunch(int cat, double bytes, hipStream_t s) : st(s), o(launch_observer) { if (o) o->begin(o->ctx, cat, bytes, st); }
    ~ObservedLaunch() { if (o) o->end(o->ctx, st); }
    ObservedLaunch(const ObservedLaunch&) = delete;
    ObservedLaunch& operator=(const ObservedLaunch&) = delete;
};

void launch_nchw3_to_nhwc4(const float* img, float* out, int n, int hw, float* absmax, hipStream_t st);
void launch_pad_c3_to_c4(const float* w, float* wp, int64_t rows, hipStream_t st);
void launch_unpad_c4_to_c3(const float* wp, float* w, int64_t rows, hipStream_t st);
void launch_pad_rows(const float* src, float* dst, int64_t rows, int d, int ld, hipStream_t st);

void launch_bn_finalize(const float* partial, int tiles_per_group, int groups, int C, double count_per_group,
                        const float* gamma, const float* beta, float* rmean, float* rvar, float momentum, float eps,
                        int training, float* stats, float* out_bound, const float* res_bound, hipStream_t st);
struct BnApplyArgs {
    const float* x;
    const float* stats;
    int C;
    int64_t rows;
    int groups = 1;
    int relu = 1;
    const float* res = nullptr;
    const float* res_stats = nullptr;
    float* y = nullptr;
    unsigned char* relu_mask = nullptr;
    void* hl_out = nullptr;
    const float* hl_absmax = nullptr;
};
void launch_bn_apply(const BnApplyArgs& a, hipStream_t st);
int bn_bwd_chunks(int64_t rows_per_group);
struct BnBwdArgs {
    const float* dy;
    const float* dy2 = nullptr;
    const float* relu_out = nullptr;
    const unsigned char* relu_mask = nullptr;
    const float* x;
    const float* stats;
    const float* gamma;
    int C;
    int64_t rows;
    int groups = 1;
    float* partial;
    float* k123;
    int reduced_tiles_per_group = 0;
    float* dgamma;
    float* dbeta;
    float* dx;
    float* g_out = nullptr;
    float* absmax = nullptr;
    void* dq = nullptr;
    void* hl_dx = nullptr;
    bool skip_fp32_dx = false;
    int lean = 0;
};
void launch_bn_bwd(const BnBwdArgs& a, hipStream_t st);
void launch_add(const float* a, const float* b, float* out, int64_t n, hipStream_t st);

void launch_maxpool_fwd(const float* in, float* out, unsigned char* argmax, int n, int hin, int win, int hout,
                        int wout, int C, hipStream_t st, const float* bn_stats = nullptr, int groups = 1,
                        unsigned char* relu_mask = nullptr);
void launch_maxpool_bwd(const float* gout, const unsigned char* argmax, float* gin, int n, int hin, int win, int hout,
                        int wout, int C, hipStream_t st, const float* gout2 = nullptr);

void launch_upsample_fwd(const float* low, int n, int hl, int wl, int ldl, int d, int h, int w, int normalize,
                         float* out, hipStream_t st);
size_t upsample_bwd_tmp_bytes(int n, int hl, int w, int d);
void launch_normalize_bwd(const float* low, int n, int hl, int wl, int ldl, int d, int h, int w, const float* gout,
                          float* gv, hipStream_t st);
void launch_upsample_bwd(const float* gout, int n, int hl, int wl, int ldl, int d, int h, int w, float* tmp,
                         float* glow, float* absmax, hipStream_t st, const float* gout_b = nullptr);

}
```

pytorch-dense-correspondence_amd/csrc/elementwise_kernels.hip:

```cpp
#include "dcn_tuning.h"
#include "elementwise_kernels.h"
#include "f16_split.h"

namespace dcn {

__device__ __forceinline__ void wave_atomic_absmax(float amax, float* absmax) {
#pragma unroll
    for (int o = 32; o > 0; o >>= 1) amax = fmaxf(amax, __shfl_xor(amax, o));
    if ((threadIdx.x & 63) == 0 && amax > 0.f) {
        const unsigned bits = __float_as_uint(amax);
        if (bits > __atomic_load_n(reinterpret_cast<unsigned*>(absmax), __ATOMIC_RELAXED))
            atomicMax(reinterpret_cast<unsigned*>(absmax), bits);
    }
}

__global__ void __launch_bounds__(256)
nchw3_to_nhwc4_kernel(const float* __restrict__ img, float* __restrict__ out, int hw, int64_t total,
                      float* __restrict__ absmax) {
    __shared__ float s_m[4];
    float m = 0.f;
    for (int64_t i = (int64_t)blockIdx.x * 256 + threadIdx.x; i < total; i += (int64_t)gridDim.x * 256) {
        const int64_t n = i / hw, p = i - n * hw;
        const float* s = img + n * 3 * hw + p;
        const float4 v = make_float4(s[0], s[hw], s[2 * (int64_t)hw], 0.f);
// ... 602 lines not shown
    const unsigned lim = nrow * uc4n - 1u;
    const float* x_b = x + eb * 4;
    const float* dy_b = dy + eb * 4;
    const float* dy2_b = DY2 ? dy2 + eb * 4 : dy2;
    const unsigned char* mask_b = MASK ? relu_mask + eb : relu_mask;
    const unsigned rel = (unsigned)(j0 - q0 * c4n) + threadIdx.x;
    const unsigned qr = rel / uc4n, cq = rel - qr * uc4n;
    unsigned er = qr * 4u * uc4n + cq;
    unsigned sec = qr * 4u >= grow ? 1u : 0u;
    DCN_OPAQUE_INT(sec);
    unsigned ks = (sec << 7) + cq;
    unsigned row0 = qr * 4u, rows_l = rel < nlive ? nrow : 0u;
    DCN_OPAQUE_INT(er); DCN_OPAQUE_INT(ks);
    if (GUARD) { DCN_OPAQUE_INT(row0); DCN_OPAQUE_INT(rows_l); }
    const float4* kp = s_k + ks;
    BnBwdRow w[4];
    float o[4][4];
    auto issue = [&](int r) {
        const unsigned e = er + (unsigned)r * uc4n;
        bn_bwd_row_issue<DY2, MASK>(w[r], x_b, dy_b, dy2_b, mask_b, GUARD ? (e < lim ? e : lim) : e);
    };
#pragma unroll
    for (int r = 0; r < D; ++r) issue(r);
    DCN_SCHED_FENCE();
#pragma unroll
    for (int r = 0; r < 4; ++r) {
        float4 g = bn_bwd_row_grad<DY2, MASK>(w[r]);
        float4 t = w[r].v, u, k;
        DCN_OPAQUE_F4(g); DCN_OPAQUE_F4(t);
        k = kp[0];                 t = make_float4(t.x - k.x, t.y - k.y, t.z - k.z, t.w - k.w); DCN_OPAQUE_F4(t); DCN_SCHED_FENCE();
        k = kp[kBnDeepPitch];      t = make_float4(t.x * k.x, t.y * k.y, t.z * k.z, t.w * k.w); DCN_OPAQUE_F4(t); DCN_SCHED_FENCE();
        k = kp[2 * kBnDeepPitch];  t = make_float4(t.x * k.x, t.y * k.y, t.z * k.z, t.w * k.w); DCN_OPAQUE_F4(t); DCN_SCHED_FENCE();
        k = kp[3 * kBnDeepPitch];  u = make_float4(g.x - k.x, g.y - k.y, g.z - k.z, g.w - k.w); DCN_OPAQUE_F4(u); DCN_SCHED_FENCE();
        k = kp[4 * kBnDeepPitch];
        t = make_float4(k.x * (u.x - t.x), k.y * (u.y - t.y), k.z * (u.z - t.z), k.w * (u.w - t.w)); DCN_OPAQUE_F4(t);
        const bool in = !GUARD || row0 + (unsigned)r < rows_l;
        if (DQ) {
            o[r][0] = in ? t.x : 0.f; o[r][1] = in ? t.y : 0.f; o[r][2] = in ? t.z : 0.f; o[r][3] = in ? t.w : 0.f;
        }
        if (in) {
            unsigned e = er;
            DCN_OPAQUE_INT(e);
            e += (unsigned)r * uc4n;
            if (DX == 1 || (DX == 2 && dx)) *reinterpret_cast<float4*>(const_cast<float*>(bn_at(dx + eb * 4, 16u * e))) = t;
            if (GOUT == 1 || (GOUT == 2 && g_out)) *reinterpret_cast<float4*>(const_cast<float*>(bn_at(g_out + eb * 4, 16u * e))) = g;
            if (HL == 1 || (HL == 2 && hl)) {
                __builtin_amdgcn_sched_barrier(0);
                dcnsplit::h2 a0, b0, a1, b1;
                dcnsplit::split2(t.x * s, t.y * s, a0, b0);
                __builtin_amdgcn_sched_barrier(0);
                dcnsplit::split2(t.z * s, t.w * s, a1, b1);
                const dcnsplit::h4 ha = {a0[0], a0[1], a1[0], a1[1]}, hb = {b0[0], b0[1], b1[0], b1[1]};
                dcnsplit::u32x2* line = reinterpret_cast<dcnsplit::u32x2*>(reinterpret_cast<char*>(hl + (eb >> 3) * 16) +
                                                                             8u * ((e >> 3) * 16u + (e & 7u)));
                line[0] = __builtin_bit_cast(dcnsplit::u32x2, ha);
                line[8] = __builtin_bit_cast(dcnsplit::u32x2, hb);
            }
        }
        if (DQ) { DCN_OPAQUE_INT(o[r][0]); DCN_OPAQUE_INT(o[r][1]); DCN_OPAQUE_INT(o[r][2]); DCN_OPAQUE_INT(o[r][3]); }
        DCN_SCHED_FENCE();
        if (r + D < 4) { issue(r + D); DCN_SCHED_FENCE(); }
    }
    if (DQ && dq && (!GUARD || row0 < rows_l))
        dcnsplit::store_blocked_quad(reinterpret_cast<dcnsplit::u32x4*>(reinterpret_cast<char*>(dq + eb) + 16u * er), 0, 0, c4n, o, s);
}
template <int D, bool DQ>
__global__ void __launch_bounds__(256) DCN_MAX_VGPRS(48)
bn_bwd_apply_blocked_deep_kernel(DCN_BN_APB_ARGS) {
    __shared__ float4 s_k[5 * kBnDeepPitch];
    const int ng = rows_per_group < rows ? 2 : 1;
    for (int i = threadIdx.x; i < ng * 5 * c4n; i += 256) {
        const int g = i / (5 * c4n), n = (i - g * 5 * c4n) / c4n, cq = i - (g * 5 + n) * c4n;
        const float* src = n == 0 ? mean + g * gstride : (n == 1 ? invstd + g * gstride : ((n == 2 ? k3 : (n == 3 ? k2 : k1)) + g * kstride));
        s_k[n * kBnDeepPitch + g * 128 + cq] = *reinterpret_cast<const float4*>(src + 4 * cq);
    }
    __syncthreads();
    const float s = __builtin_bit_cast(float, __builtin_amdgcn_readfirstlane(__builtin_bit_cast(int, dcnsplit::pow2_scale(*absmax))));
    const int64_t total = ((rows + 3) >> 2) * c4n;
    for (int64_t j0 = (int64_t)blockIdx.x * 256; j0 < total; j0 += (int64_t)gridDim.x * 256) {
        const bool whole = j0 + 256 <= total && ((j0 + 255) / c4n) * 4 + 3 < rows;
#define DCN_BN_DEEP(DD, DY2, MASK, GOUT, DX, HL, GUARD)                                                                        \
        bn_bwd_apply_deep_body<DD, DQ, DY2, MASK, GOUT, DX, HL, GUARD>(j0, dy, dy2, relu_mask, x, dx, g_out, dq, s, c4n, rows,  \
                                                                       rows_per_group, hl, s_k)
#define DCN_BN_DEEP_DX(DD, DY2, MASK, HL)                                                                                      \
        do {                                                                                                                   \
            if (g_out) { if (dx) DCN_BN_DEEP(DD, DY2, MASK, 1, 1, HL, false); else DCN_BN_DEEP(DD, DY2, MASK, 1, 0, HL, false); } \
            else { if (dx) DCN_BN_DEEP(DD, DY2, MASK, 0, 1, HL, false); else DCN_BN_DEEP(DD, DY2, MASK, 0, 0, HL, false); }     \
        } while (0)
#define DCN_BN_DEEP_OUT(DD, DY2, MASK)                                                                                         \
        do {                                                                                                                   \
            if (!whole) DCN_BN_DEEP(((DQ && DY2) ? 1 : DD), DY2, MASK, 2, 2, 2, true);                                                            \
            else if (DQ && !hl) DCN_BN_DEEP_DX(DD, DY2, MASK, 0);                                                              \
            else DCN_BN_DEEP_DX(DD, DY2, MASK, 1);                                                                             \
        } while (0)
        if (relu_mask) { if (dy2) DCN_BN_DEEP_OUT(2, true, true); else DCN_BN_DEEP_OUT(D, false, true); }
        else { if (dy2) DCN_BN_DEEP_OUT(2, true, false); else DCN_BN_DEEP_OUT(D, false, false); }
#undef DCN_BN_DEEP_OUT
#undef DCN_BN_DEEP_DX
#undef DCN_BN_DEEP
    }
}
#undef DCN_BN_APB_ARGS
#undef DCN_BN_APB_PASS

__global__ void __launch_bounds__(256)
absmax_kernel(const float* __restrict__ v, int64_t total, float* __restrict__ absmax) {
    float amax = 0.f;
    for (int64_t i = (int64_t)blockIdx.x * 256 + threadIdx.x; i < total; i += (int64_t)gridDim.x * 256)
        amax = fmaxf(amax, fabsf(v[i]));
    wave_atomic_absmax(amax, absmax);
}

__global__ void __launch_bounds__(256)
add_kernel(const float* __restrict__ a, const float* __restrict__ b, float* __restrict__ out, int64_t total4) {
    for (int64_t i = (int64_t)blockIdx.x * 256 + threadIdx.x; i < total4; i += (int64_t)gridDim.x * 256) {
        const float4 u = reinterpret_cast<const float4*>(a)[i], v = reinterpret_cast<const float4*>(b)[i];
        reinterpret_cast<float4*>(out)[i] = make_float4(u.x + v.x, u.y + v.y, u.z + v.z, u.w + v.w);
    }
}

__global__ void __launch_bounds__(256)
maxpool_fwd_kernel(const float* __restrict__ in, float* __restrict__ out, unsigned char* __restrict__ argmax, int hin,
                   int win, int hout, int wout, int c4n, int64_t total4, const float* __restrict__ scale,
                   const float* __restrict__ shift, int gstride, int64_t group_n, unsigned char* __restrict__ relu_mask) {
    const int64_t i = (int64_t)blockIdx.x * 256 + threadIdx.x;
    if (i >= total4) return;
    const int c4 = (int)(i % c4n);
    int64_t pix = i / c4n;
    const int ox = (int)(pix % wout); pix /= wout;
    const int oy = (int)(pix % hout);
    const int64_t n = pix / hout;
    float4 sc = make_float4(1.f, 1.f, 1.f, 1.f), sh = make_float4(0.f, 0.f, 0.f, 0.f);
    if (scale) {
        const int c = c4 * 4 + (n >= group_n ? gstride : 0);
        sc = *reinterpret_cast<const float4*>(scale + c);
        sh = *reinterpret_cast<const float4*>(shift + c);
    }
    float4 best = make_float4(-INFINITY, -INFINITY, -INFINITY, -INFINITY);
    int bx = -1, by = -1, bz = -1, bw = -1;
    for (int r = 0; r < 3; ++r) {
        const int iy = oy * 2 - 1 + r;
        if (iy < 0 || iy >= hin) continue;
        for (int s = 0; s < 3; ++s) {
            const int ix = ox * 2 - 1 + s;
            if (ix < 0 || ix >= win) continue;
            const int64_t src = ((n * hin + iy) * win + ix) * c4n + c4;
            float4 v = reinterpret_cast<const float4*>(in)[src];
            if (scale) {
                v = make_float4(v.x * sc.x + sh.x, v.y * sc.y + sh.y, v.z * sc.z + sh.z, v.w * sc.w + sh.w);
                v.x = fmaxf(v.x, 0.f); v.y = fmaxf(v.y, 0.f); v.z = fmaxf(v.z, 0.f); v.w = fmaxf(v.w, 0.f);
                if (relu_mask)
                    relu_mask[src] = (unsigned char)((v.x > 0.f ? 1 : 0) | (v.y > 0.f ? 2 : 0) | (v.z > 0.f ? 4 : 0) | (v.w > 0.f ? 8 : 0));
            }
            const int t = r * 3 + s;
            if (v.x > best.x || bx < 0 || v.x != v.x) { best.x = v.x; bx = t; }
            if (v.y > best.y || by < 0 || v.y != v.y) { best.y = v.y; by = t; }
            if (v.z > best.z || bz < 0 || v.z != v.z) { best.z = v.z; bz = t; }
            if (v.w > best.w || bw < 0 || v.w != v.w) { best.w = v.w; bw = t; }
        }
    }
    reinterpret_cast<float4*>(out)[i] = best;
    if (argmax) {
        unsigned char* a = argmax + i * 4;
        a[0] = (unsigned char)bx; a[1] = (unsigned char)by; a[2] = (unsigned char)bz; a[3] = (unsigned char)bw;
    }
}

__global__ void __launch_bounds__(256)
maxpool_bwd_kernel(const float* __restrict__ gout, const float* __restrict__ gout2, const unsigned char* __restrict__ argmax,
                   float* __restrict__ gin, int hin, int win, int hout, int wout, int c4n, int64_t total4) {
    const int64_t i = (int64_t)blockIdx.x * 256 + threadIdx.x;
    if (i >= total4) return;
    const int c4 = (int)(i % c4n);
    int64_t pix = i / c4n;
    const int ix = (int)(pix % win); pix /= win;
    const int iy = (int)(pix % hin);
    const int64_t n = pix / hin;
    float4 acc = make_float4(0.f, 0.f, 0.f, 0.f);
    for (int oy = iy / 2; oy <= (iy + 1) / 2; ++oy) {
        if (oy >= hout) continue;
        const int r = iy - (oy * 2 - 1);
        if (r < 0 || r > 2) continue;
        for (int ox = ix / 2; ox <= (ix + 1) / 2; ++ox) {
            if (ox >= wout) continue;
            const int s = ix - (ox * 2 - 1);
            if (s < 0 || s > 2) continue;
            const int t = r * 3 + s;
            const int64_t o = ((n * hout + oy) * wout + ox) * c4n + c4;
            float4 g = reinterpret_cast<const float4*>(gout)[o];
            if (gout2) {
                const float4 h = reinterpret_cast<const float4*>(gout2)[o];
                g.x += h.x; g.y += h.y; g.z += h.z; g.w += h.w;
            }
            const unsigned char* a = argmax + o * 4;
            if (a[0] == t) acc.x += g.x;
            if (a[1] == t) acc.y += g.y;
            if (a[2] == t) acc.z += g.z;
            if (a[3] == t) acc.w += g.w;
        }
    }
    reinterpret_cast<float4*>(gin)[i] = acc;
}

__device__ __forceinline__ void src_index(int dst, float scale, int in_size, int& i0, int& i1, float& l1) {
    const float s = scale * (float)dst;
    i0 = (int)s;
    if (i0 > in_size - 1) i0 = in_size - 1;
    i1 = i0 < in_size - 1 ? i0 + 1 : i0;
    l1 = s - (float)i0;
}

__global__ void __launch_bounds__(256)
upsample_fwd_kernel(const float* __restrict__ low, int hl, int wl, int ldl, int d, int h, int w, float sh, float sw,
                    int normalize, float* __restrict__ out, int64_t total) {
    const int64_t i = (int64_t)blockIdx.x * 256 + threadIdx.x;
    if (i >= total) return;
    const int x = (int)(i % w);
    const int64_t t = i / w;
    const int y = (int)(t % h);
    const int64_t n = t / h;
    int y0, y1, x0, x1;
    float ly, lx;
    src_index(y, sh, hl, y0, y1, ly);
    src_index(x, sw, wl, x0, x1, lx);
    const float hy = 1.f - ly, hx = 1.f - lx;
    const float* p00 = low + ((n * hl + y0) * wl + x0) * ldl;
    const float* p01 = low + ((n * hl + y0) * wl + x1) * ldl;
    const float* p10 = low + ((n * hl + y1) * wl + x0) * ldl;
    const float* p11 = low + ((n * hl + y1) * wl + x1) * ldl;
    float* o = out + i * d;
    if (!normalize) {
        for (int k = 0; k < d; ++k) o[k] = hy * (hx * p00[k] + lx * p01[k]) + ly * (hx * p10[k] + lx * p11[k]);
    } else {
        float ss = 0.f;
        for (int k = 0; k < d; ++k) {
            const float v = hy * (hx * p00[k] + lx * p01[k]) + ly * (hx * p10[k] + lx * p11[k]);
            ss = fmaf(v, v, ss);
        }
        const float nrm = sqrtf(ss);
        for (int k = 0; k < d; ++k)
            o[k] = (hy * (hx * p00[k] + lx * p01[k]) + ly * (hx * p10[k] + lx * p11[k])) / nrm;
    }
}

__global__ void __launch_bounds__(256)
normalize_bwd_kernel(const float* __restrict__ low, int hl, int wl, int ldl, int d, int h, int w, float sh, float sw,
                     const float* __restrict__ gout, float* __restrict__ gv, int64_t total) {
    const int64_t i = (int64_t)blockIdx.x * 256 + threadIdx.x;
    if (i >= total) return;
    const int x = (int)(i % w);
    const int64_t t = i / w;
    const int y = (int)(t % h);
    const int64_t n = t / h;
    int y0, y1, x0, x1;
    float ly, lx;
    src_index(y, sh, hl, y0, y1, ly);
    src_index(x, sw, wl, x0, x1, lx);
    const float hy = 1.f - ly, hx = 1.f - lx;
    const float* p00 = low + ((n * hl + y0) * wl + x0) * ldl;
    const float* p01 = low + ((n * hl + y0) * wl + x1) * ldl;
    const float* p10 = low + ((n * hl + y1) * wl + x0) * ldl;
    const float* p11 = low + ((n * hl + y1) * wl + x1) * ldl;
    const float* g = gout + i * d;
    float ss = 0.f, dot = 0.f;
    for (int k = 0; k < d; ++k) {
        const float v = hy * (hx * p00[k] + lx * p01[k]) + ly * (hx * p10[k] + lx * p11[k]);
        ss = fmaf(v, v, ss);
        dot = fmaf(v, g[k], dot);
    }
    const float nrm = sqrtf(ss), inv = 1.f / nrm;
    dot *= inv;
    for (int k = 0; k < d; ++k) {
        const float v = hy * (hx * p00[k] + lx * p01[k]) + ly * (hx * p10[k] + lx * p11[k]);
        gv[i * d + k] = (g[k] - v * inv * dot) * inv;
    }
}

__global__ void __launch_bounds__(256)
upsample_bwd_rows_kernel(const float* __restrict__ gout, int hl, int d, int h, int w, float sh, float* __restrict__ tmp,
                         int64_t total) {
    const int64_t i = (int64_t)blockIdx.x * 256 + threadIdx.x;
    if (i >= total) return;
    const int64_t wd = (int64_t)w * d;
    const int64_t xd = i % wd;
    const int64_t t = i / wd;
    const int iy = (int)(t % hl);
    const int64_t n = t / hl;
    const float inv = sh > 0.f ? 1.f / sh : 0.f;
    int ylo = (int)floorf(((float)iy - 1.f) * inv) - 1, yhi = (int)ceilf(((float)iy + 1.f) * inv) + 1;
    if (ylo < 0) ylo = 0;
    if (yhi > h - 1 || sh <= 0.f) yhi = h - 1;
    float acc = 0.f;
    for (int y = ylo; y <= yhi; ++y) {
        int y0, y1;
        float ly;
        src_index(y, sh, hl, y0, y1, ly);
        float wgt = 0.f;
        if (y0 == iy) wgt += 1.f - ly;
        if (y1 == iy) wgt += ly;
        if (wgt != 0.f) acc = fmaf(wgt, gout[(n * h + y) * wd + xd], acc);
    }
    tmp[i] = acc;
}
__global__ void __launch_bounds__(256)
upsample_bwd_cols_kernel(const float* __restrict__ tmp, int hl, int wl, int ldl, int d, int w, float sw,
                         float* __restrict__ glow, int64_t total) {
    const int64_t i = (int64_t)blockIdx.x * 256 + threadIdx.x;
    if (i >= total) return;
    const int k = (int)(i % ldl);
    const int64_t t = i / ldl;
    const int ix = (int)(t % wl);
    const int64_t row = t / wl;
    if (k >= d) { glow[i] = 0.f; return; }
    const float inv = sw > 0.f ? 1.f / sw : 0.f;
    int xlo = (int)floorf(((float)ix - 1.f) * inv) - 1, xhi = (int)ceilf(((float)ix + 1.f) * inv) + 1;
    if (xlo < 0) xlo = 0;
    if (xhi > w - 1 || sw <= 0.f) xhi = w - 1;
    float acc = 0.f;
    for (int x = xlo; x <= xhi; ++x) {
        int x0, x1;
        float lx;
        src_index(x, sw, wl, x0, x1, lx);
        float wgt = 0.f;
        if (x0 == ix) wgt += 1.f - lx;
        if (x1 == ix) wgt += lx;
        if (wgt != 0.f) acc = fmaf(wgt, tmp[(row * w + x) * d + k], acc);
    }
    glow[i] = acc;
}

static inline unsigned blocks_for(int64_t n, int cap = 0) {
    int64_t b = ceil_div64(n, 256);
    if (cap > 0 && b > cap) b = cap;
    if (b < 1) b = 1;
    return (unsigned)b;
}
constexpr int kGridCap = 256 * 8;

thread_local const LaunchObserver* launch_observer = nullptr;

void launch_nchw3_to_nhwc4(const float* img, float* out, int n, int hw, float* absmax, hipStream_t st) {
    const int64_t total = (int64_t)n * hw;
    ObservedLaunch obs(DCN_PROF_RESAMPLE, 28.0 * (double)total, st);
    hipLaunchKernelGGL(nchw3_to_nhwc4_kernel, dim3(blocks_for(total, kGridCap)), dim3(256), 0, st, img, out, hw, total, absmax);
}
void launch_pad_c3_to_c4(const float* w, float* wp, int64_t rows, hipStream_t st) {
    ObservedLaunch obs(DCN_PROF_OTHER, 28.0 * (double)rows, st);
    hipLaunchKernelGGL(pad_c3_to_c4_kernel, dim3(blocks_for(rows)), dim3(256), 0, st, w, wp, rows);
}
void launch_unpad_c4_to_c3(const float* wp, float* w, int64_t rows, hipStream_t st) {
    ObservedLaunch obs(DCN_PROF_OTHER, 28.0 * (double)rows, st);
    hipLaunchKernelGGL(unpad_c4_to_c3_kernel, dim3(blocks_for(rows)), dim3(256), 0, st, wp, w, rows);
}
void launch_pad_rows(const float* src, float* dst, int64_t rows, int d, int ld, hipStream_t st) {
    ObservedLaunch obs(DCN_PROF_OTHER, 4.0 * (double)rows * (d + ld), st);
    hipLaunchKernelGGL(pad_rows_kernel, dim3(blocks_for(rows * ld)), dim3(256), 0, st, src, dst, rows, d, ld);
}
void launch_bn_finalize(const float* partial, int tiles_per_group, int groups, int C, double count_per_group,
                        const float* gamma, const float* beta, float* rmean, float* rvar, float momentum, float eps,
                        int training, float* stats, float* out_bound, const float* res_bound, hipStream_t st) {
    ObservedLaunch obs(DCN_PROF_BN_FINALIZE, training ? 12.0 * (double)tiles_per_group * groups * C : 0.0, st);
    hipLaunchKernelGGL(bn_finalize_kernel, dim3(ceil_div(C, 4)), dim3(256), 0, st, partial, tiles_per_group, groups, C,
                       count_per_group, gamma, beta, rmean, rvar, momentum, eps, training, stats, stats + C, stats + 2 * C,
                       stats + 3 * C, 4 * C, out_bound, res_bound);
}
void launch_bn_apply(const BnApplyArgs& a, hipStream_t st) {
    const int C = a.C;
    const int64_t total4 = a.rows * (C / 4);
    void* hl_out = ((C % 32) == 0 && a.hl_absmax) ? a.hl_out : nullptr;
    ObservedLaunch obs(DCN_PROF_BN_APPLY, (double)a.rows * C * (4.0 + (a.res ? 4.0 : 0.0) + (a.y ? 4.0 : 0.0) + (hl_out ? 4.0 : 0.0) +
                                                               (a.relu_mask ? 0.25 : 0.0)), st);
    hipLaunchKernelGGL(bn_apply_kernel, dim3(blocks_for(total4, kGridCap)), dim3(256), 0, st, a.x, a.stats, a.stats + C, a.res,
                       a.res_stats, a.res_stats ? a.res_stats + C : nullptr, a.relu, a.y, a.relu_mask, C / 4, total4,
                       total4 / a.groups, 4 * C, (dcnsplit::u32x2*)hl_out, a.hl_absmax, tuning().bn_reverse & 1, tuning().bn_nt & 1);
}
int bn_bwd_chunks(int64_t rows_per_group) {
    const int rows = rows_per_group >= 16384 ? 128 : (rows_per_group >= 8192 ? 64 : 32);
    int64_t chunks = ceil_div64(rows_per_group, rows);
    if (chunks > 1024) chunks = 1024;
    if (chunks < 1) chunks = 1;
    return (int)chunks;
}
static decltype(&bn_bwd_apply_blocked_kernel) bn_bwd_blocked_apply_instance(int lean, bool deep, int depth, bool with_dq);
void launch_bn_bwd(const BnBwdArgs& a, hipStream_t st) {
    const int C = a.C, groups = a.groups, lean = a.lean;
    const int64_t rows = a.rows, rpg = rows / groups;
    const float *dy = a.dy, *dy2 = a.dy2, *relu_out = a.relu_out, *x = a.x;
    const unsigned char* relu_mask = a.relu_mask;
    const float* mean = a.stats + 2 * C;
    const float* invstd = a.stats + 3 * C;
    float *partial = a.partial, *k123 = a.k123, *g_out = a.g_out, *absmax = a.absmax;
    void* hl = (a.hl_dx && (C % 32) == 0) ? a.hl_dx : nullptr;
    void* dq = a.dq;
    const bool blocked = (dq || hl) && absmax;
    float* dx = (blocked && hl && a.skip_fp32_dx) ? nullptr : a.dx;
    int chunks = a.reduced_tiles_per_group;
    const int depth = tuning().bn_bwd_lean_depth;
    const bool deep = depth > 1 && !(relu_out && !relu_mask) && C <= 512 && groups <= 2;
    const double in_bytes = 8.0 + (dy2 ? 4.0 : 0.0) + (relu_mask ? 0.25 : (relu_out ? 4.0 : 0.0));
    const double out_bytes = (dx ? 4.0 : 0.0) + (g_out ? 4.0 : 0.0) + (blocked && dq ? 4.0 : 0.0) + (blocked && hl ? 4.0 : 0.0);
    if (chunks <= 0) {
        chunks = bn_bwd_chunks(rpg);
        const int rpc = (int)ceil_div64(rpg, chunks);
        ObservedLaunch obs(DCN_PROF_BN_BWD_REDUCE, (double)rows * C * in_bytes, st);
        const int cap = tuning().bn_reduce_wide;
        const int cq = ((C % 512) == 0 && cap >= 128) ? 128 : (((C % 256) == 0 && cap >= 64) ? 64 : (((C % 128) == 0 && cap >= 32) ? 32 : 16));
#define DCN_BN_RED(K, CQ)                                                                                                     \
        hipLaunchKernelGGL(K<CQ>, dim3(ceil_div(C, 4 * CQ), chunks * groups), dim3(256), 0, st, dy, dy2, relu_out,            \
                           relu_mask, x, mean, invstd, C, rpg, chunks, 4 * C, rpc, partial)
#define DCN_BN_RED_CQ(K)                                                                                                      \
        if (cq == 128) DCN_BN_RED(K, 128);                                                                                    \
        else if (cq == 64) DCN_BN_RED(K, 64);                                                                                 \
        else if (cq == 32) DCN_BN_RED(K, 32);                                                                                 \
        else DCN_BN_RED(K, 16)
        if (lean & 1) { DCN_BN_RED_CQ(bn_bwd_reduce_lean_kernel); }
        else { DCN_BN_RED_CQ(bn_bwd_reduce_kernel); }
#undef DCN_BN_RED_CQ
#undef DCN_BN_RED
    }
    {
        ObservedLaunch obs(DCN_PROF_BN_FINALIZE, 16.0 * (double)chunks * groups * C, st);
        const auto kernel = (lean & 2) ? bn_bwd_finalize_lean_kernel : bn_bwd_finalize_kernel;
        hipLaunchKernelGGL(kernel, dim3(ceil_div(C, 4)), dim3(256), 0, st,
                           (const float*)partial, chunks, groups, C, (double)rpg, a.gamma, invstd, 4 * C, a.dgamma, a.dbeta, k123, absmax);
    }
    const int64_t total4 = rows * (C / 4);
    ObservedLaunch obs(DCN_PROF_BN_BWD_APPLY, (double)rows * C * (in_bytes + out_bytes), st);
    if (blocked) {
        const auto kernel = bn_bwd_blocked_apply_instance(lean, deep, depth, dq != nullptr);
        hipLaunchKernelGGL(kernel, dim3(blocks_for(((rows + 3) / 4) * (C / 4), kGridCap)), dim3(256), 0, st,
                           dy, dy2, relu_out, relu_mask, x, mean, invstd, (const float*)k123, (const float*)(k123 + C),
                           (const float*)(k123 + 2 * C), dx, g_out, (dcnsplit::u32x4*)dq, (const float*)absmax, C / 4, rows, rpg,
                           4 * C, 3 * C, (dcnsplit::u32x2*)hl, (tuning().bn_reverse >> 1) & 1, (tuning().bn_nt >> 1) & 1);
        return;
    }
    hipLaunchKernelGGL(bn_bwd_apply_kernel, dim3(blocks_for(total4, kGridCap)), dim3(256), 0, st, dy, dy2, relu_out, relu_mask,
                       x, mean, invstd, (const float*)k123, (const float*)(k123 + C), (const float*)(k123 + 2 * C), dx, g_out,
                       C / 4, total4, total4 / groups, 4 * C, 3 * C, (tuning().bn_reverse >> 1) & 1);
}
static decltype(&bn_bwd_apply_blocked_kernel) bn_bwd_blocked_apply_instance(int lean, bool deep, int depth, bool with_dq) {
    if (!(lean & 4)) return bn_bwd_apply_blocked_kernel;
    if (!deep) return with_dq ? bn_bwd_apply_blocked_lean_kernel<true> : bn_bwd_apply_blocked_lean_kernel<false>;
    if (!with_dq) return depth > 2 ? bn_bwd_apply_blocked_deep_kernel<3, false> : bn_bwd_apply_blocked_deep_kernel<2, false>;
    return bn_bwd_apply_blocked_deep_kernel<2, true>;
}
void launch_add(const float* a, const float* b, float* out, int64_t n, hipStream_t st) {
    ObservedLaunch obs(DCN_PROF_OTHER, 12.0 * (double)n, st);
    hipLaunchKernelGGL(add_kernel, dim3(blocks_for(n / 4, kGridCap)), dim3(256), 0, st, a, b, out, n / 4);
}
void launch_maxpool_fwd(const float* in, float* out, unsigned char* argmax, int n, int hin, int win, int hout,
                        int wout, int C, hipStream_t st, const float* bn_stats, int groups, unsigned char* relu_mask) {
    const int64_t total4 = (int64_t)n * hout * wout * (C / 4);
    ObservedLaunch obs(DCN_PROF_RESAMPLE, (double)n * C * ((double)hin * win * (4.0 + (bn_stats && relu_mask ? 0.25 : 0.0)) +
                                                          (double)hout * wout * (4.0 + (argmax ? 1.0 : 0.0))), st);
    hipLaunchKernelGGL(maxpool_fwd_kernel, dim3(blocks_for(total4)), dim3(256), 0, st, in, out, argmax, hin, win, hout,
                       wout, C / 4, total4, bn_stats, bn_stats ? bn_stats + C : nullptr, 4 * C,
                       (int64_t)(groups > 1 ? n / groups : n), bn_stats ? relu_mask : nullptr);
}
void launch_maxpool_bwd(const float* gout, const unsigned char* argmax, float* gin, int n, int hin, int win, int hout,
                        int wout, int C, hipStream_t st, const float* gout2) {
    const int64_t total4 = (int64_t)n * hin * win * (C / 4);
    ObservedLaunch obs(DCN_PROF_RESAMPLE, (double)n * C * ((double)hin * win * 4.0 + (double)hout * wout * (5.0 + (gout2 ? 4.0 : 0.0))), st);
    hipLaunchKernelGGL(maxpool_bwd_kernel, dim3(blocks_for(total4)), dim3(256), 0, st, gout, gout2, argmax, gin, hin, win,
                       hout, wout, C / 4, total4);
}
static inline float ac_scale(int in, int out) { return out > 1 ? (float)(in - 1) / (float)(out - 1) : 0.f; }
void launch_upsample_fwd(const float* low, int n, int hl, int wl, int ldl, int d, int h, int w, int normalize,
                         float* out, hipStream_t st) {
    const int64_t total = (int64_t)n * h * w;
    ObservedLaunch obs(DCN_PROF_RESAMPLE, 4.0 * ((double)n * hl * wl * ldl + (double)total * d), st);
    hipLaunchKernelGGL(upsample_fwd_kernel, dim3(blocks_for(total)), dim3(256), 0, st, low, hl, wl, ldl, d, h, w,
                       ac_scale(hl, h), ac_scale(wl, w), normalize, out, total);
}
size_t upsample_bwd_tmp_bytes(int n, int hl, int w, int d) { return (size_t)n * hl * w * d * sizeof(float); }
void launch_normalize_bwd(const float* low, int n, int hl, int wl, int ldl, int d, int h, int w, const float* gout,
                          float* gv, hipStream_t st) {
    const int64_t total = (int64_t)n * h * w;
    ObservedLaunch obs(DCN_PROF_RESAMPLE, 4.0 * ((double)n * hl * wl * ldl + 2.0 * (double)total * d), st);
    hipLaunchKernelGGL(normalize_bwd_kernel, dim3(blocks_for(total)), dim3(256), 0, st, low, hl, wl, ldl, d, h, w,
                       ac_scale(hl, h), ac_scale(wl, w), gout, gv, total);
}
void launch_upsample_bwd(const float* gout, int n, int hl, int wl, int ldl, int d, int h, int w, float* tmp,
                         float* glow, float* absmax, hipStream_t st, const float* gout_b) {
    const int64_t t1 = (int64_t)n * hl * w * d;
    if (gout_b) {
        const int64_t th = t1 / 2;
        for (int k = 0; k < 2; ++k) {
            ObservedLaunch obs(DCN_PROF_RESAMPLE, 4.0 * ((double)(n / 2) * h * w * d + (double)th), st);
            hipLaunchKernelGGL(upsample_bwd_rows_kernel, dim3(blocks_for(th)), dim3(256), 0, st, k ? gout_b : gout, hl, d, h, w,
                               ac_scale(hl, h), tmp + k * th, th);
        }
    } else {
        ObservedLaunch obs(DCN_PROF_RESAMPLE, 4.0 * ((double)n * h * w * d + (double)t1), st);
        hipLaunchKernelGGL(upsample_bwd_rows_kernel, dim3(blocks_for(t1)), dim3(256), 0, st, gout, hl, d, h, w,
                           ac_scale(hl, h), tmp, t1);
    }
    const int64_t t2 = (int64_t)n * hl * wl * ldl;
    {
        ObservedLaunch obs(DCN_PROF_RESAMPLE, 4.0 * ((double)t1 + (double)t2), st);
        hipLaunchKernelGGL(upsample_bwd_cols_kernel, dim3(blocks_for(t2)), dim3(256), 0, st, (const float*)tmp, hl, wl, ldl,
                           d, w, ac_scale(wl, w), glow, t2);
    }
    if (absmax) {
        ObservedLaunch obs(DCN_PROF_OTHER, 4.0 * (double)t2, st);
        hipLaunchKernelGGL(absmax_kernel, dim3(blocks_for(t2, 256)), dim3(256), 0, st, (const float*)glow, t2, absmax);
    }
}

}

extern "C" int dcn_upsample_forward(const float* low, int n, int hl, int wl, int ldl, int d, int h, int w, int normalize,
                                    float* out, void* stream) {
    if (!low || !out || n < 1 || hl < 1 || wl < 1 || d < 1 || ldl < d || h < 1 || w < 1) return DCN_E_INVALID;
    dcn::launch_upsample_fwd(low, n, hl, wl, ldl, d, h, w, normalize, out, (hipStream_t)stream);
    return dcn::check_launch();
}

extern "C" size_t dcn_upsample_backward_tmp_bytes(int n, int hl, int w, int d) {
    return dcn::upsample_bwd_tmp_bytes(n, hl, w, d);
}

extern "C" int dcn_upsample_backward(const float* gout, int n, int hl, int wl, int ldl, int d, int h, int w, float* glow,
                                     float* tmp, void* stream) {
    if (!gout || !glow || !tmp || n < 1 || hl < 1 || wl < 1 || d < 1 || ldl < d || h < 1 || w < 1) return DCN_E_INVALID;
    dcn::launch_upsample_bwd(gout, n, hl, wl, ldl, d, h, w, tmp, glow, nullptr, (hipStream_t)stream);
    return dcn::check_launch();
}

extern "C" int dcn_bn_forward(const float* x, const float* bn_partial, int mtiles, int c, int64_t rows, const float* gamma,
                              const float* beta, float* running_mean, float* running_var, float momentum, float eps,
                              int training, const float* res, int relu, float* y, unsigned char* relu_mask, float* stats,
                              void* stream) {
    if (!x || !gamma || !beta || !y || !stats || c < 4 || (c % 4) != 0 || rows < 1) return DCN_E_INVALID;
    if (training ? (!bn_partial || mtiles < 1) : (!running_mean || !running_var)) return DCN_E_INVALID;
    hipStream_t st = (hipStream_t)stream;
    dcn::launch_bn_finalize(bn_partial, mtiles, 1, c, (double)rows, gamma, beta, running_mean, running_var, momentum, eps,
                            training, stats, nullptr, nullptr, st);
    dcn::launch_bn_apply({.x = x, .stats = stats, .C = c, .rows = rows, .relu = relu, .res = res, .y = y, .relu_mask = relu_mask}, st);
    return dcn::check_launch();
}

static int standalone_lean() { return dcn::tuning().bn_bwd_lean ? dcn::tuning().bn_bwd_lean_mask : 0; }

extern "C" size_t dcn_bn_backward_workspace(int64_t rows, int c) {
    if (rows < 1 || c < 4) return 0;
    return ((size_t)dcn::bn_bwd_chunks(rows) * 4 * (size_t)c + 3 * (size_t)c) * sizeof(float);
}

extern "C" int dcn_bn_backward(const float* dy, const unsigned char* relu_mask, const float* x, const float* stats,
                               const float* gamma, int c, int64_t rows, float* dgamma, float* dbeta, float* dx, float* g_out,
                               void* workspace, void* stream) {
    if (!dy || !x || !stats || !gamma || !dgamma || !dbeta || !dx || !workspace || c < 4 || (c % 4) != 0 || rows < 1)
        return DCN_E_INVALID;
    float* partial = (float*)workspace;
    float* k123 = partial + (size_t)dcn::bn_bwd_chunks(rows) * 4 * c;
    dcn::launch_bn_bwd({.dy = dy, .relu_mask = relu_mask, .x = x, .stats = stats, .gamma = gamma, .C = c, .rows = rows,
                        .partial = partial, .k123 = k123, .dgamma = dgamma, .dbeta = dbeta, .dx = dx, .g_out = g_out,
                        .lean = standalone_lean()}, (hipStream_t)stream);
    return dcn::check_launch();
}

extern "C" int dcn_bn_backward_from_partial(const float* dy, const float* bn_partial, int mtiles, const float* x,
                                            const float* stats, const float* gamma, int c, int64_t rows, float* dgamma,
                                            float* dbeta, float* dx, void* workspace, void* stream) {
    if (!dy || !bn_partial || mtiles < 1 || !x || !stats || !gamma || !dgamma || !dbeta || !dx || !workspace || c < 4 ||
        (c % 4) != 0 || rows < 1)
        return DCN_E_INVALID;
    dcn::launch_bn_bwd({.dy = dy, .x = x, .stats = stats, .gamma = gamma, .C = c, .rows = rows,
                        .partial = const_cast<float*>(bn_partial), .k123 = (float*)workspace, .reduced_tiles_per_group = mtiles,
                        .dgamma = dgamma, .dbeta = dbeta, .dx = dx, .lean = standalone_lean()}, (hipStream_t)stream);
    return dcn::check_launch();
}

extern "C" size_t dcn_bn_backward_full_workspace(int64_t rows, int c, int groups) {
    if (rows < 1 || c < 4 || groups < 1 || (rows % groups) != 0) return 0;
    return ((size_t)groups * dcn::bn_bwd_chunks(rows / groups) * 4 * (size_t)c + (size_t)groups * 3 * (size_t)c) * sizeof(float);
}

extern "C" int dcn_bn_backward_full(const float* dy, const float* dy2, const float* relu_out, const unsigned char* relu_mask,
                                    const float* x, const float* stats, const float* gamma, int c, int64_t rows, int groups,
                                    float* dgamma, float* dbeta, float* dx, float* g_out, float* absmax, void* dq, void* hl_dx,
                                    int keep_dx, void* workspace, void* stream) {
    if (!dy || !x || !stats || !gamma || !dgamma || !dbeta || !workspace || c < 4 || (c % 4) != 0 || rows < 1) return DCN_E_INVALID;
    if ((groups != 1 && groups != 2) || (rows % groups) != 0) return DCN_E_INVALID;
    const bool blocked = (dq || (hl_dx && (c % 32) == 0)) && absmax;
    if ((dq || hl_dx) && !absmax) return DCN_E_INVALID;
    if (hl_dx && (c % 32) != 0) return DCN_E_INVALID;
    if (blocked && groups == 2 && ((rows / groups) % 4) != 0) return DCN_E_INVALID;
    if (!dx && !(hl_dx && !keep_dx)) return DCN_E_INVALID;
    float* partial = (float*)workspace;
    float* k123 = partial + (size_t)groups * dcn::bn_bwd_chunks(rows / groups) * 4 * c;
    dcn::launch_bn_bwd({.dy = dy, .dy2 = dy2, .relu_out = relu_out, .relu_mask = relu_mask, .x = x, .stats = stats, .gamma = gamma,
                        .C = c, .rows = rows, .groups = groups, .partial = partial, .k123 = k123, .dgamma = dgamma, .dbeta = dbeta,
                        .dx = dx, .g_out = g_out, .absmax = absmax, .dq = dq, .hl_dx = hl_dx, .skip_fp32_dx = !keep_dx,
                        .lean = standalone_lean()}, (hipStream_t)stream);
    return dcn::check_launch();
}

extern "C" int dcn_maxpool_forward(const float* in, int n, int hin, int win, int c, float* out, unsigned char* argmax,
                                   void* stream) {
    if (!in || !out || n < 1 || hin < 1 || win < 1 || c < 4 || (c % 4) != 0) return DCN_E_INVALID;
    dcn::launch_maxpool_fwd(in, out, argmax, n, hin, win, (hin + 2 - 3) / 2 + 1, (win + 2 - 3) / 2 + 1, c, (hipStream_t)stream);
    return dcn::check_launch();
}

extern "C" int dcn_maxpool_backward(const float* gout, const unsigned char* argmax, int n, int hin, int win, int c,
                                    float* gin, void* stream) {
    if (!gout || !argmax || !gin || n < 1 || hin < 1 || win < 1 || c < 4 || (c % 4) != 0) return DCN_E_INVALID;
    dcn::launch_maxpool_bwd(gout, argmax, gin, n, hin, win, (hin + 2 - 3) / 2 + 1, (win + 2 - 3) / 2 + 1, c, (hipStream_t)stream);
    return dcn::check_launch();
}

extern "C" int dcn_maxpool_forward_full(const float* in, const float* bn_stats, int groups, int n, int hin, int win, int c,
                                        float* out, unsigned char* argmax, unsigned char* relu_mask, void* stream) {
    if (!in || !out || n < 1 || hin < 1 || win < 1 || c < 4 || (c % 4) != 0) return DCN_E_INVALID;
    if ((groups != 1 && groups != 2) || (n % groups) != 0) return DCN_E_INVALID;
    if (relu_mask && !bn_stats) return DCN_E_INVALID;
    dcn::launch_maxpool_fwd(in, out, argmax, n, hin, win, (hin + 2 - 3) / 2 + 1, (win + 2 - 3) / 2 + 1, c, (hipStream_t)stream,
                            bn_stats, groups, relu_mask);
    return dcn::check_launch();
}

extern "C" int dcn_maxpool_backward_full(const float* gout, const float* gout2, const unsigned char* argmax, int n, int hin,
                                         int win, int c, float* gin, void* stream) {
    if (!gout || !argmax || !gin || n < 1 || hin < 1 || win < 1 || c < 4 || (c % 4) != 0) return DCN_E_INVALID;
    dcn::launch_maxpool_bwd(gout, argmax, gin, n, hin, win, (hin + 2 - 3) / 2 + 1, (win + 2 - 3) / 2 + 1, c, (hipStream_t)stream,
                            gout2);
    return dcn::check_launch();
}

extern "C" int dcn_normalize_backward(const float* low, int n, int hl, int wl, int ldl, int d, int h, int w, const float* gout,
                                      float* gv, void* stream) {
    if (!low || !gout || !gv || n < 1 || hl < 1 || wl < 1 || d < 1 || ldl < d || h < 1 || w < 1) return DCN_E_INVALID;
    dcn::launch_normalize_bwd(low, n, hl, wl, ldl, d, h, w, gout, gv, (hipStream_t)stream);
    return dcn::check_launch();
}

extern "C" int dcn_upsample_backward_full(const float* gout, const float* gout_b, int n, int hl, int wl, int ldl, int d, int h,
                                          int w, float* glow, float* tmp, float* absmax, void* stream) {
    if (!gout || !glow || !tmp || n < 1 || hl < 1 || wl < 1 || d < 1 || ldl < d || h < 1 || w < 1) return DCN_E_INVALID;
    if (gout_b && (n % 2) != 0) return DCN_E_INVALID;
    dcn::launch_upsample_bwd(gout, n, hl, wl, ldl, d, h, w, tmp, glow, absmax, (hipStream_t)stream, gout_b);
    return dcn::check_launch();
}

extern "C" int dcn_image_to_nhwc4(const float* img, int n, int hw, float* out, float* absmax, void* stream) {
    if (!img || !out || n < 1 || hw < 1) return DCN_E_INVALID;
    dcn::launch_nchw3_to_nhwc4(img, out, n, hw, absmax, (hipStream_t)stream);
    return dcn::check_launch();
}

extern "C" int dcn_pad_c3_to_c4(const float* src, float* dst, int64_t rows, void* stream) {
    if (!src || !dst || rows < 1) return DCN_E_INVALID;
    dcn::launch_pad_c3_to_c4(src, dst, rows, (hipStream_t)stream);
    return dcn::check_launch();
}

extern "C" int dcn_unpad_c4_to_c3(const float* src, float* dst, int64_t rows, void* stream) {
    if (!src || !dst || rows < 1) return DCN_E_INVALID;
    dcn::launch_unpad_c4_to_c3(src, dst, rows, (hipStream_t)stream);
    return dcn::check_launch();
}

extern "C" int dcn_pad_rows(const float* src, float* dst, int64_t rows, int d, int ld, void* stream) {
    if (!src || !dst || rows < 1 || d < 1 || ld < d) return DCN_E_INVALID;
    dcn::launch_pad_rows(src, dst, rows, d, ld, (hipStream_t)stream);
    return dcn::check_launch();
}
```

pytorch-dense-correspondence_amd/dcn_hip/_lib.py:

```python
import atexit
import ctypes
import os

import torch

HERE = os.path.dirname(os.path.abspath(__file__))
DEFAULT_PATH = os.path.join(HERE, "libdcn_hip.so")

_lib = None
_info = {"path": None, "version": None, "hostemu": False}
_reset_hooks = []

c_void_p, c_int, c_int64, c_size_t, c_float, c_char_p = (ctypes.c_void_p, ctypes.c_int, ctypes.c_int64,
                                                         ctypes.c_size_t, ctypes.c_float, ctypes.c_char_p)


class LossConfig(ctypes.Structure):
    _fields_ = [("margin", c_float * 4), ("invert", ctypes.c_int32 * 4), ("pixel_weight", ctypes.c_int32 * 4),
                ("m_pixel", c_float), ("image_width", ctypes.c_int32), ("match_loss_weight", c_float),
                ("non_match_loss_weight", c_float), ("scale_by_hard_negatives", ctypes.c_int32),
                ("compose", ctypes.c_int32)]


class ConvDesc(ctypes.Structure):
    _fields_ = [(k, ctypes.c_int32) for k in ("n", "hin", "win", "cin", "hout", "wout", "cout", "kh", "kw", "stride",
                                              "pad", "dil", "ldc", "group_rows")]


class FrameStoreDesc(ctypes.Structure):
    _fields_ = [("num_frames", c_int64)] + [(k, ctypes.c_int32) for k in ("num_scenes", "num_objects", "num_multi", "h", "w")] \
        + [(k, c_void_p) for k in ("rgb", "depth", "mask", "scene_first_frame", "scene_object", "object_scene_offsets",
                                   "object_scenes", "multi_scenes", "scene_cams", "poses")]


class PictureFamily(ctypes.Structure):
    _fields_ = [("mode", ctypes.c_int32), ("picture_channels", ctypes.c_int32), ("channel", ctypes.c_int32 * 3),
                ("reserved", ctypes.c_int32), ("stats", c_void_p), ("normed", c_void_p), ("picture", c_void_p),
                ("side_stride", c_int64), ("pair_stride", c_int64)]


SYMBOLS = {
    "dcn_version": (c_char_p, []),
    "dcn_reload_env": (None, []),
    "dcn_release_pooled_buffers": (None, []),
    "dcn_plan_num_activation_slots": (c_int, [c_void_p]),
    "dcn_plan_fused_bn_backward": (c_int, [c_void_p]),
    "dcn_plan_activation_absmax_offset": (c_size_t, [c_void_p]),
    "dcn_plan_num_grad_buckets": (c_int, [c_void_p]),
    "dcn_plan_grad_bucket_first_param": (c_int, [c_void_p, c_int]),
    "dcn_plan_stream_wait_grad_bucket": (c_int, [c_void_p, c_int, c_void_p]),
    "dcn_bn_forward": (c_int, [c_void_p, c_void_p, c_int, c_int, c_int64, c_void_p, c_void_p, c_void_p, c_void_p, c_float,
                               c_float, c_int, c_void_p, c_int, c_void_p, c_void_p, c_void_p, c_void_p]),
    "dcn_bn_backward_workspace": (c_size_t, [c_int64, c_int]),
    "dcn_bn_backward": (c_int, [c_void_p, c_void_p, c_void_p, c_void_p, c_void_p, c_int, c_int64, c_void_p, c_void_p, c_void_p,
                                c_void_p, c_void_p, c_void_p]),
    "dcn_maxpool_forward": (c_int, [c_void_p, c_int, c_int, c_int, c_int, c_void_p, c_void_p, c_void_p]),
    "dcn_maxpool_backward": (c_int, [c_void_p, c_void_p, c_int, c_int, c_int, c_int, c_void_p, c_void_p]),
    "dcn_loss_workspace_bytes": (c_size_t, [c_int, c_int64]),
    "dcn_contrastive_loss_forward": (c_int, [c_void_p, c_void_p, c_int, c_int64, c_int, c_void_p, c_void_p, c_void_p,
                                             c_void_p, ctypes.POINTER(LossConfig), c_void_p, c_void_p, c_void_p,
                                             c_void_p, c_void_p, c_void_p, c_void_p, c_void_p]),
    "dcn_contrastive_loss_backward": (c_int, [c_void_p, c_void_p, c_int, c_int64, c_int, c_void_p, c_void_p, c_void_p,
                                              c_void_p, ctypes.POINTER(LossConfig), c_void_p, c_void_p, c_void_p,
                                              c_void_p, c_void_p, c_void_p, c_void_p]),
    "dcn_loss_saved_floats": (c_size_t, [c_int64, c_int]),
    "dcn_contrastive_loss_forward_save": (c_int, [c_void_p, c_void_p, c_int, c_int64, c_int, c_void_p, c_void_p, c_void_p,
                                                  c_void_p, ctypes.POINTER(LossConfig), c_void_p, c_void_p, c_void_p,
                                                  c_void_p, c_void_p, c_void_p, c_void_p, c_void_p, c_void_p]),
    "dcn_contrastive_loss_backward_saved": (c_int, [c_int, c_int64, c_int, c_void_p, c_void_p, c_void_p, c_void_p,
                                                    ctypes.POINTER(LossConfig), c_void_p, c_void_p, c_void_p, c_int, c_void_p,
                                                    c_void_p, c_void_p]),
    "dcn_loss_exact_workspace_bytes": (c_size_t, [c_int, c_int64, c_int]),
    "dcn_contrastive_loss_backward_saved_exact": (c_int, [c_int, c_int64, c_int, c_void_p, c_void_p, c_void_p, c_void_p,
                                                          ctypes.POINTER(LossConfig), c_void_p, c_void_p, c_void_p, c_void_p,
                                                          c_void_p, c_void_p, c_void_p]),
    "dcn_contrastive_loss_mixed_forward": (c_int, [c_void_p, c_void_p, c_int, c_int64, c_int] + [c_void_p] * 4
                                           + [ctypes.POINTER(LossConfig), c_int64, c_int64, c_int64] + [c_void_p] * 9),
    "dcn_contrastive_loss_mixed_backward_saved": (c_int, [c_int, c_int64, c_int] + [c_void_p] * 4
                                                  + [ctypes.POINTER(LossConfig), c_int64, c_int64, c_int64] + [c_void_p] * 4
                                                  + [c_int, c_void_p, c_void_p, c_void_p]),
    "dcn_contrastive_loss_mixed_backward_saved_exact": (c_int, [c_int, c_int64, c_int] + [c_void_p] * 4
                                                        + [ctypes.POINTER(LossConfig), c_int64, c_int64, c_int64]
                                                        + [c_void_p] * 8),
    "dcn_fill_bytes": (c_int, [c_void_p, c_int, c_size_t, c_void_p]),
    "dcn_plan_create": (c_int, [c_char_p, c_int, c_int, c_int, c_int, c_int, ctypes.POINTER(c_void_p)]),
    "dcn_plan_destroy": (None, [c_void_p]),
    "dcn_plan_forget_saved": (c_int, [c_void_p, c_void_p]),
    "dcn_plan_num_forward_records": (c_int, [c_void_p]),
    "dcn_plan_num_params": (c_int, [c_void_p]),
    "dcn_plan_num_bn": (c_int, [c_void_p]),
    "dcn_plan_param_info": (c_int, [c_void_p, c_int, c_char_p, c_int, ctypes.POINTER(c_int64), ctypes.POINTER(c_int)]),
    "dcn_plan_bn_info": (c_int, [c_void_p, c_int, c_char_p, c_int, ctypes.POINTER(c_int64)]),
    "dcn_plan_saved_bytes": (c_size_t, [c_void_p]),
    "dcn_plan_workspace_bytes": (c_size_t, [c_void_p]),
    "dcn_plan_forward_flops": (ctypes.c_double, [c_void_p]),
    "dcn_plan_profile_begin": (c_int, [c_void_p]),
    "dcn_plan_profile_end": (c_int, [c_void_p, ctypes.POINTER(ctypes.c_double), ctypes.POINTER(c_int64),
                                     ctypes.POINTER(ctypes.c_double)]),
    "dcn_plan_profile_end3": (c_int, [c_void_p, ctypes.POINTER(ctypes.c_double), ctypes.POINTER(c_int64),
                                      ctypes.POINTER(ctypes.c_double)]),
    "dcn_plan_profile_end_all": (c_int, [c_void_p, ctypes.POINTER(ctypes.c_double), ctypes.POINTER(c_int64),
                                         ctypes.POINTER(ctypes.c_double)]),
    "dcn_backbone_forward": (c_int, [c_void_p, c_void_p, c_void_p, c_void_p, c_float, c_float, c_int, c_int, c_void_p,
                                     c_void_p, c_void_p, c_void_p]),
    "dcn_backbone_backward": (c_int, [c_void_p, c_void_p, c_void_p, c_void_p, c_void_p, c_void_p, c_int, c_void_p]),
    "dcn_backbone_forward_pair": (c_int, [c_void_p, c_void_p, c_void_p, c_void_p, c_void_p, c_float, c_float, c_int, c_int,
                                          c_void_p, c_void_p, c_void_p, c_void_p]),
    "dcn_backbone_backward_pair": (c_int, [c_void_p, c_void_p, c_void_p, c_void_p, c_void_p, c_void_p, c_void_p, c_int,
                                           c_void_p]),
    "dcn_conv_forward": (c_int, [ctypes.POINTER(ConvDesc), c_void_p, c_void_p, c_void_p, c_void_p, c_void_p, c_void_p,
                                 c_void_p]),
    "dcn_conv_gemm_workspace": (c_size_t, [ctypes.POINTER(ConvDesc), c_int]),
    "dcn_conv_num_mtiles": (c_int, [ctypes.POINTER(ConvDesc)]),
    "dcn_conv_dgrad": (c_int, [ctypes.POINTER(ConvDesc), c_void_p, c_void_p, c_void_p, c_void_p, c_void_p, c_void_p]),
    "dcn_conv_wgrad": (c_int, [ctypes.POINTER(ConvDesc), c_void_p, c_void_p, c_void_p, c_void_p, c_void_p]),
    "dcn_conv_wgrad_workspace": (c_size_t, [ctypes.POINTER(ConvDesc)]),
    "dcn_transpose_weight": (c_int, [c_void_p, c_void_p, c_int, c_int, c_int, c_int, c_void_p]),
    "dcn_f16_kpad": (c_int, [c_int]),
    "dcn_split_rows_f16": (c_int, [c_void_p, c_void_p, c_void_p, c_int64, c_int, c_float, c_void_p]),
    "dcn_conv_num_mtiles_f16": (c_int, [ctypes.POINTER(ConvDesc)]),
    "dcn_conv_gemm_workspace_f16": (c_size_t, [ctypes.POINTER(ConvDesc), c_int]),
    "dcn_conv_forward_f16": (c_int, [ctypes.POINTER(ConvDesc), c_void_p, c_void_p, c_void_p, c_void_p, c_float, c_void_p,
                                     c_void_p, c_void_p, c_void_p, c_void_p]),
    "dcn_conv_dgrad_f16": (c_int, [ctypes.POINTER(ConvDesc), c_void_p, c_void_p, c_void_p, c_float, c_void_p, c_void_p,
                                   c_void_p, c_void_p, c_void_p]),
    "dcn_split_stem_weights_f16": (c_int, [c_void_p, c_void_p, c_void_p, c_int, c_float, c_void_p]),
    "dcn_conv_stem_forward_f16": (c_int, [ctypes.POINTER(ConvDesc), c_void_p, c_void_p, c_void_p, c_void_p, c_float, c_void_p,
                                          c_void_p, c_void_p]),
    "dcn_conv_dgrad_bn_num_mtiles_f16": (c_int, [ctypes.POINTER(ConvDesc)]),
    "dcn_conv_dgrad_bn_f16": (c_int, [ctypes.POINTER(ConvDesc), c_void_p, c_void_p, c_void_p, c_float, c_void_p, c_void_p,
                                      c_void_p, c_void_p, c_void_p, c_void_p, c_void_p, c_void_p, c_void_p]),
    "dcn_bn_backward_from_partial": (c_int, [c_void_p, c_void_p, c_int, c_void_p, c_void_p, c_void_p, c_int, c_int64,
                                             c_void_p, c_void_p, c_void_p, c_void_p, c_void_p]),
    "dcn_bn_backward_full_workspace": (c_size_t, [c_int64, c_int, c_int]),
    "dcn_bn_backward_full": (c_int, [c_void_p] * 7 + [c_int, c_int64, c_int] + [c_void_p] * 7 + [c_int, c_void_p, c_void_p]),
    "dcn_triplet_loss_workspace_bytes": (c_size_t, [c_int64]),
    "dcn_triplet_loss_forward": (c_int, [c_void_p, c_void_p, c_int64, c_int, c_void_p, c_void_p, c_void_p, c_int64, c_int64,
                                         c_float, c_void_p, c_void_p, c_void_p, c_void_p]),
    "dcn_triplet_loss_backward": (c_int, [c_void_p, c_void_p, c_int64, c_int, c_void_p, c_void_p, c_void_p, c_int64, c_int64,
                                          c_float, c_void_p, c_void_p, c_void_p, c_void_p]),
    "dcn_find_correspondences_workspace": (c_size_t, [c_int64]),
    "dcn_find_correspondences": (c_int, [c_void_p, c_void_p, c_int, c_int, c_void_p, c_void_p, c_void_p, c_void_p, c_void_p,
                                         c_void_p, c_int64, c_void_p, c_void_p, c_void_p, c_void_p, c_void_p, c_void_p,
                                         c_void_p]),
    "dcn_mask_nonzero_workspace": (c_size_t, [c_int64]),
    "dcn_mask_nonzero": (c_int, [c_void_p, c_int64, c_void_p, c_void_p, c_void_p, c_void_p]),
    "dcn_sample_pixels": (c_int, [c_void_p, c_int64, c_int, c_int, c_void_p, c_void_p, c_void_p, c_void_p, c_void_p]),
    "dcn_adam_step": (c_int, [c_int, c_void_p, c_void_p, c_void_p, c_void_p, c_void_p, ctypes.c_double, ctypes.c_double,
                              ctypes.c_double, ctypes.c_double, ctypes.c_double, c_int64, c_void_p]),
    "dcn_plan_create_grouped": (c_int, [c_char_p, c_int, c_int, c_int, c_int, c_int, c_int, ctypes.POINTER(c_void_p)]),
    "dcn_plan_set_conv_mode": (c_int, [c_void_p, c_int]),
    "dcn_plan_conv_mode": (c_int, [c_void_p]),
    "dcn_conv_wgrad_f16": (c_int, [ctypes.POINTER(ConvDesc), c_void_p, c_int, c_void_p, c_void_p, c_void_p, c_void_p, c_void_p,
                                   c_void_p]),
    "dcn_split_weights_f16": (c_int, [c_int, c_void_p, c_void_p, c_void_p, c_void_p, c_void_p, c_void_p, c_void_p, c_int,
                                      c_float, c_void_p]),
    "dcn_split_weights_scaled_f16": (c_int, [c_int, c_void_p, c_void_p, c_void_p, c_void_p, c_void_p, c_void_p, c_void_p,
                                             c_void_p, c_int, c_float, c_void_p]),
    "dcn_conv_forward_fused_f16": (c_int, [ctypes.POINTER(ConvDesc), c_void_p, c_void_p, c_void_p, c_void_p, c_float, c_void_p,
                                           c_void_p, c_int, c_void_p, c_void_p, c_void_p, c_void_p]),
    "dcn_split_act_f16": (c_int, [c_void_p, c_void_p, c_int64, c_void_p]),
    "dcn_grad_blocked_bytes": (c_size_t, [c_int, c_int]),
    "dcn_split_grad_blocked_f16": (c_int, [c_void_p, c_int, c_int, c_void_p, c_void_p, c_void_p]),
    "dcn_conv_wgrad_workspace_f16": (c_size_t, [ctypes.POINTER(ConvDesc)]),
    "dcn_match_statistics_workspace": (c_size_t, [c_int]),
    "dcn_match_statistics": (c_int, [c_void_p, c_int64, c_int, c_int, c_void_p, c_void_p, c_int, c_void_p, c_void_p, c_void_p,
                                     c_void_p, c_void_p, c_void_p, c_void_p, c_void_p]),
    "dcn_find_best_match": (c_int, [c_void_p, c_int64, c_int, c_void_p, c_int, c_void_p, c_void_p, c_void_p, c_void_p,
                                    c_void_p, c_void_p]),
    "dcn_find_best_match_workspace": (c_size_t, [c_int]),
    "dcn_upsample_forward": (c_int, [c_void_p, c_int, c_int, c_int, c_int, c_int, c_int, c_int, c_int, c_void_p,
                                     c_void_p]),
    "dcn_upsample_backward": (c_int, [c_void_p, c_int, c_int, c_int, c_int, c_int, c_int, c_int, c_void_p, c_void_p,
                                      c_void_p]),
    "dcn_upsample_backward_tmp_bytes": (c_size_t, [c_int, c_int, c_int, c_int]),
    "dcn_maxpool_forward_full": (c_int, [c_void_p, c_void_p, c_int, c_int, c_int, c_int, c_int, c_void_p, c_void_p, c_void_p,
                                         c_void_p]),
    "dcn_maxpool_backward_full": (c_int, [c_void_p, c_void_p, c_void_p, c_int, c_int, c_int, c_int, c_void_p, c_void_p]),
    "dcn_normalize_backward": (c_int, [c_void_p] + [c_int] * 7 + [c_void_p, c_void_p, c_void_p]),
    "dcn_upsample_backward_full": (c_int, [c_void_p, c_void_p] + [c_int] * 7 + [c_void_p] * 4),
    "dcn_image_to_nhwc4": (c_int, [c_void_p, c_int, c_int, c_void_p, c_void_p, c_void_p]),
    "dcn_pad_c3_to_c4": (c_int, [c_void_p, c_void_p, c_int64, c_void_p]),
    "dcn_unpad_c4_to_c3": (c_int, [c_void_p, c_void_p, c_int64, c_void_p]),
    "dcn_pad_rows": (c_int, [c_void_p, c_void_p, c_int64, c_int, c_int, c_void_p]),
    "dcn_column_sums": (c_int, [c_void_p, c_int64, c_int, c_int, c_void_p, c_void_p]),
    "dcn_split_weights_checked_f16": (c_int, [c_int, c_void_p, c_void_p, c_void_p, c_void_p, c_void_p, c_void_p, c_void_p,
                                              c_float, c_void_p, c_void_p]),
    "dcn_conv_wgrad_hl_eligible": (c_int, [ctypes.POINTER(ConvDesc)]),
    "dcn_conv_wgrad_hl_kind": (c_int, [ctypes.POINTER(ConvDesc)]),
    "dcn_conv_wgrad_workspace_hl": (c_size_t, [ctypes.POINTER(ConvDesc)]),
    "dcn_conv_wgrad_hl": (c_int, [ctypes.POINTER(ConvDesc), c_void_p, c_void_p, c_void_p, c_void_p, c_void_p, c_void_p, c_void_p]),
    "dcn_conv_hl_eligible": (c_int, [ctypes.POINTER(ConvDesc), c_int]),
    "dcn_conv_num_mtiles_hl": (c_int, [ctypes.POINTER(ConvDesc)]),
    "dcn_conv_tile_rows_hl": (c_int, [ctypes.POINTER(ConvDesc), c_int]),
    "dcn_conv_gemm_workspace_hl": (c_size_t, [ctypes.POINTER(ConvDesc), c_int]),
    "dcn_conv_hl_shape_info": (c_int, [ctypes.POINTER(ConvDesc), c_int, ctypes.POINTER(c_int)]),
    "dcn_split_act_hl32": (c_int, [c_void_p, c_void_p, c_void_p, c_int64, c_int, c_void_p]),
    "dcn_split_weights_hl32": (c_int, [c_int, c_void_p, c_void_p, c_void_p, c_void_p, c_void_p, c_void_p, c_int, c_float,
                                       c_void_p]),
    "dcn_conv_forward_hl": (c_int, [ctypes.POINTER(ConvDesc), c_void_p, c_void_p, c_void_p, c_float, c_void_p, c_void_p,
                                    c_void_p, c_void_p, c_void_p]),
    "dcn_conv_dgrad_hl": (c_int, [ctypes.POINTER(ConvDesc), c_void_p, c_void_p, c_float, c_void_p, c_void_p, c_void_p,
                                  c_void_p, c_void_p]),
    "dcn_augment_images": (c_int, [c_int, c_int, c_int, c_void_p, c_void_p, c_void_p, c_void_p, c_void_p, c_void_p, c_void_p,
                                   c_void_p, c_void_p, c_void_p, c_void_p, c_void_p, c_void_p, c_void_p, c_void_p]),
    "dcn_flip_planes": (c_int, [c_void_p, c_void_p, c_int64, c_int, c_int, c_int, c_int, c_int, c_void_p]),
    "dcn_flip_uv": (c_int, [c_int, c_void_p, c_void_p, c_void_p, c_void_p, c_int64, c_int, c_void_p, c_void_p, c_int, c_int,
                            c_int, c_void_p]),
    "dcn_merge_images": (c_int, [c_int, c_int, c_int, c_int] + [c_void_p] * 18),
    "dcn_merge_prune_workspace": (c_size_t, [c_int, c_int64, c_int64]),
    "dcn_sample_workspace": (c_size_t, [c_int, c_int, c_int, c_int64, c_int64]),
    "dcn_within_scene_samples": (c_int, [c_int, c_int, c_int] + [c_void_p] * 5 + [c_int64, c_int, c_int, c_int]
                                 + [c_void_p] * 4 + [c_int, c_void_p, c_void_p, c_int64] + [c_void_p] * 6),
    "dcn_complete_samples": (c_int, [c_int, c_int, c_int] + [c_void_p] * 4 + [c_int, c_void_p, c_int64, c_void_p, c_void_p,
                                                                              c_int, c_int, c_int] + [c_void_p] * 4
                             + [c_int, c_void_p, c_void_p, c_int64] + [c_void_p] * 6),
    "dcn_across_scene_samples": (c_int, [c_int, c_int, c_int, c_void_p, c_void_p, c_int64] + [c_void_p] * 4
                                 + [c_int, c_void_p, c_void_p, c_int64] + [c_void_p] * 6),
    "dcn_synthetic_workspace": (c_size_t, [c_int, c_int, c_int, c_int64]),
    "dcn_synthetic_samples": (c_int, [c_int, c_int, c_int] + [c_void_p] * 4 + [c_int64, c_int, c_int, c_int] + [c_void_p] * 13
                              + [c_int64] + [c_void_p] * 6),
    "dcn_concat_samples": (c_int, [c_int] + [c_void_p] * 8 + [c_int64, c_void_p, c_void_p, c_void_p]),
    "dcn_merge_prune": (c_int, [c_int, c_int, c_int] + [c_void_p] * 10 + [c_int64] + [c_void_p] * 5 + [c_int64, c_int]
                        + [c_void_p] * 9),
    "dcn_select_frames": (c_int, [c_int, c_int, ctypes.POINTER(FrameStoreDesc), c_int, ctypes.c_double, ctypes.c_double]
                          + [c_void_p] * 8),
    "dcn_gather_frames": (c_int, [c_int, c_int, ctypes.POINTER(FrameStoreDesc)] + [c_void_p] * 8),
    "dcn_eval_matches_workspace": (c_size_t, [c_int, c_int, c_int, c_int64]),
    "dcn_eval_matches": (c_int, [c_int, c_int, c_int] + [c_void_p] * 4 + [c_int64] + [c_void_p] * 3 + [c_int]
                         + [c_void_p] * 11),
    "dcn_match_statistics_pairs_workspace": (c_size_t, [c_int64]),
    "dcn_match_statistics_pairs": (c_int, [c_int, c_int, c_int, c_int] + [c_void_p] * 11 + [c_int64, c_int]
                                   + [c_void_p] * 9),
    "dcn_across_object_queries_workspace": (c_size_t, [c_int, c_int, c_int]),
    "dcn_across_object_queries": (c_int, [c_int, c_int, c_int, c_int, c_void_p, c_void_p, c_int] + [c_void_p] * 10),
    "dcn_best_match_pairs_workspace": (c_size_t, [c_int64]),
    "dcn_best_match_pairs": (c_int, [c_int, c_int, c_int, c_int, c_void_p, c_void_p, c_void_p, c_int64, c_int]
                             + [c_void_p] * 6),
    "dcn_reproject_pixels": (c_int, [c_int, ctypes.POINTER(FrameStoreDesc)] + [c_void_p] * 8),
    "dcn_match_statistics_groups_workspace": (c_size_t, [c_int64]),
    "dcn_match_statistics_groups": (c_int, [c_int, c_int, c_int, c_int] + [c_void_p] * 12 + [c_int64, c_int]
                                    + [c_void_p] * 9),
    "dcn_match_statistics_groups_wide": (c_int, [c_int, c_int, c_int, c_int] + [c_void_p] * 12 + [c_int64, c_int, c_int64]
                                         + [c_void_p] * 9),
    "dcn_descriptor_statistics_workspace": (c_size_t, [c_int, c_int, c_int, c_int]),
    "dcn_descriptor_statistics": (c_int, [c_int, c_int, c_int, c_int] + [c_void_p] * 6),
    "dcn_descriptor_statistics_combine": (c_int, [c_int, c_int, c_void_p, c_void_p, c_int, c_void_p, c_void_p, c_void_p]),
    "dcn_train_advance": (c_int, [c_void_p, c_void_p, c_int, c_int64, c_int64, ctypes.c_double, ctypes.c_double,
                                  ctypes.c_double, c_void_p]),
    "dcn_adam_step_guarded": (c_int, [c_int, c_void_p, c_void_p, c_void_p, c_void_p, c_void_p, ctypes.c_double,
                                      ctypes.c_double, ctypes.c_double, ctypes.c_double, c_void_p, c_void_p]),
    "dcn_guarded_copy": (c_int, [c_int, c_void_p, c_void_p, c_void_p, c_void_p, c_int, c_void_p]),
    "dcn_train_log": (c_int, [c_void_p, c_int64, c_int64, c_void_p, c_void_p, c_void_p, c_void_p, c_int, c_void_p]),
    "dcn_train_advance_ranks": (c_int, [c_void_p, c_void_p, c_int, c_int, c_int, c_void_p, c_int64, c_int64, ctypes.c_double,
                                        ctypes.c_double, ctypes.c_double, c_void_p]),
    "dcn_train_log_ranks": (c_int, [c_void_p, c_int64, c_int64, c_void_p, c_void_p, c_void_p, c_int, c_int, c_void_p]),
    "dcn_eval_curves": (c_int, [c_int, c_int64, c_int64, c_void_p, c_void_p, c_void_p, c_int] + [c_void_p] * 5),
    "dcn_descriptor_ranges_workspace": (c_size_t, [c_int, c_int, c_int, c_int]),
    "dcn_descriptor_ranges": (c_int, [c_int, c_int, c_int, c_int] + [c_void_p] * 10),
    "dcn_descriptor_normalize": (c_int, [c_int, c_int, c_int, c_int] + [c_void_p] * 6 + [ctypes.POINTER(PictureFamily * 2),
                                                                                        c_void_p]),
    "dcn_heat_maps": (c_int, [c_int, c_int, c_int, c_int, c_void_p, c_void_p, c_void_p, c_int64, c_float] + [c_void_p] * 5),
}

ERRORS = {-1: "DCN_E_INVALID (bad argument)", -2: "DCN_E_LAUNCH (kernel launch failed)",
          -3: "DCN_E_UNSUPPORTED"}


def load(path=None):
    global _lib
    if _lib is not None and (path is None or os.path.abspath(path) == _info["path"]):
        return _lib
    p = os.path.abspath(path or os.environ.get("DCN_HIP_LIBRARY", DEFAULT_PATH))
    if not os.path.exists(p):
        raise RuntimeError(
            "dcn_hip: %s not found.  Build the gfx950 kernels first: `python __graft_entry__.py` "
            "(or dcn_hip.build.build_library()).  There is no CPU / PyTorch fallback for this path." % p)
    lib = ctypes.CDLL(p)
    for name, (res, args) in SYMBOLS.items():
        fn = getattr(lib, name)
        fn.restype = res
        fn.argtypes = args
    ver = lib.dcn_version().decode()
    for hook in _reset_hooks:
        hook()
    atexit.register(lib.dcn_release_pooled_buffers)
    _lib = lib
    _info.update(path=p, version=ver, hostemu=("hostemu" in ver))
    return _lib


def get():
    return _lib if _lib is not None else load()


def library_info():
    get()
    return dict(_info)


def is_hostemu():
    get()
    return _info["hostemu"]


def check(rc, what):
    if rc != 0:
        raise RuntimeError("dcn_hip: %s failed: %s" % (what, ERRORS.get(rc, rc)))


def require_device(*tensors):
    emu = is_hostemu()
    for t in tensors:
        if t is None:
            continue
        if emu and t.is_cuda:
            raise RuntimeError("dcn_hip (host-emulation test build) got a GPU tensor")
        if not emu and not t.is_cuda:
            raise RuntimeError("dcn_hip: tensor is on %s -- the dense-correspondence hot path runs on the MI355X only "
                               "(no CPU fallback); move the module and its inputs with .cuda()" % t.device)


def stream_ptr():
    if is_hostemu():
        return None
    return c_void_p(torch.cuda.current_stream().cuda_stream)


def ptr(t):
    return None if t is None else c_void_p(t.data_ptr())


def host_ptr(a):
    return a.ctypes.data_as(c_void_p)
```

Before: 464.8.

## Add v2 resample kernels fusing pool hl split, image pair conversion, upsample backward

Adds a resample_v2 path, on by default, that replaces several resampling kernels. The stem maxpool forward now writes the hi/lo split activations for block 0 directly, so the separate split pass can be skipped. Paired images are converted to NHWC4 in a single launch, and maxpool backward and upsample backward get row-strip kernels that vectorise across four channels and fold in the absmax reduction. The stem BN backward can also skip writing its fp32 dx when nothing reads it. The cost is a wider set of kernel variants and new correctness edge cases around alignment, element-count limits and the hl split.

```diff
diff --git a/include/dcn_hip.h b/include/dcn_hip.h
--- a/include/dcn_hip.h
+++ b/include/dcn_hip.h
@@ -272,6 +272,8 @@
 
 int dcn_maxpool_forward_full(const float* in, const float* bn_stats, int groups, int n, int hin, int win, int c, float* out,
                              unsigned char* argmax, unsigned char* relu_mask, void* stream);
+int dcn_maxpool_forward_hl(const float* in, const float* bn_stats, int groups, int n, int hin, int win, int c, float* out,
+                           unsigned char* argmax, unsigned char* relu_mask, void* hl_out, const float* hl_absmax, void* stream);
 int dcn_maxpool_backward_full(const float* gout, const float* gout2, const unsigned char* argmax, int n, int hin, int win, int c,
                               float* gin, void* stream);
 int dcn_normalize_backward(const float* low, int n, int hl, int wl, int ldl, int d, int h, int w, const float* gout, float* gv,
@@ -279,6 +281,7 @@
 int dcn_upsample_backward_full(const float* gout, const float* gout_b, int n, int hl, int wl, int ldl, int d, int h, int w,
                                float* glow, float* tmp, float* absmax, void* stream);
 int dcn_image_to_nhwc4(const float* img, int n, int hw, float* out, float* absmax, void* stream);
+int dcn_image_pair_to_nhwc4(const float* img, const float* img_b, int n, int hw, float* out, float* absmax, void* stream);
 int dcn_pad_c3_to_c4(const float* src, float* dst, int64_t rows, void* stream);
 int dcn_unpad_c4_to_c3(const float* src, float* dst, int64_t rows, void* stream);
 int dcn_pad_rows(const float* src, float* dst, int64_t rows, int d, int ld, void* stream);
diff --git a/pytorch-dense-correspondence_amd/csrc/backbone_engine.hip b/pytorch-dense-correspondence_amd/csrc/backbone_engine.hip
--- a/pytorch-dense-correspondence_amd/csrc/backbone_engine.hip
+++ b/pytorch-dense-correspondence_amd/csrc/backbone_engine.hip
@@ -851,12 +851,7 @@
 
     DCN_TRY(R.other([&] { return dcn::fill_bytes_async(R.S(p.s_actmax), 0, ((size_t)p.n_act + 1) * sizeof(float), st); }));
     const ConvL& stem = p.convs[p.stem];
-    if (image_b) {
-        dcn::launch_nchw3_to_nhwc4(image, R.S(p.s_in4), N / 2, p.H * p.W, R.A(stem.in_act), st);
-        dcn::launch_nchw3_to_nhwc4(image_b, R.S(p.s_in4) + (size_t)(N / 2) * p.H * p.W * 4, N / 2, p.H * p.W, R.A(stem.in_act), st);
-    } else {
-        dcn::launch_nchw3_to_nhwc4(image, R.S(p.s_in4), N, p.H * p.W, R.A(stem.in_act), st);
-    }
+    dcn::launch_nchw3_to_nhwc4(image, R.S(p.s_in4), N, p.H * p.W, R.A(stem.in_act), st, image_b);
     dcn::launch_pad_c3_to_c4(R.P(stem.w), R.Wk(p.w_wstem), (int64_t)p.base * 49, st);
     dcn_plan::FwdRecord rec;
     rec.saved = saved;
@@ -925,25 +920,30 @@
         DCN_TRY(R.other([&] { return dcn_split_stem_weights_f16(R.Wk(p.w_wstem), hi, hi + (size_t)p.base * 224, p.base, kWeightScale, st); }));
     }
     DCN_TRY(R.conv_bn(stem, R.S(p.s_in4), R.Wk(p.w_wstem), bn_running, momentum, eps, training, p.blocks[0].act_in));
+    bool pool_wrote_hl = false;
     {
         const BnL& b = p.bns[stem.bn];
         const float* s = R.S(b.stats);
         const int hp = (stem.d.hout + 2 - 3) / 2 + 1, wp = (stem.d.wout + 2 - 3) / 2 + 1;
+        const BlockL& b0 = p.blocks[0];
+        const bool pool_hl = training && f16_mode && b0.has_hl_in;
+        float* hl_img = pool_hl ? R.S(b0.hl_in) : nullptr;
+        const float* hl_bound = pool_hl ? R.A(b0.act_in) : nullptr;
         if (dcn::tuning().stem_pool_fused != 0) {
-            dcn::launch_maxpool_fwd(R.S(stem.x), R.S(p.s_pool), (unsigned char*)R.S(p.s_argmax), N, stem.d.hout, stem.d.wout, hp,
-                                    wp, b.C, st, s, p.groups, R.M(p.s_stem_y));
+            pool_wrote_hl = dcn::launch_maxpool_fwd(R.S(stem.x), R.S(p.s_pool), (unsigned char*)R.S(p.s_argmax), N, stem.d.hout,
+                                                    stem.d.wout, hp, wp, b.C, st, s, p.groups, R.M(p.s_stem_y), hl_img, hl_bound);
         } else {
             dcn::launch_bn_apply({.x = R.S(stem.x), .stats = s, .C = b.C, .rows = b.rows, .groups = p.groups, .y = R.S(p.s_stem_y),
                                   .relu_mask = R.M(p.s_stem_y)}, st);
-            dcn::launch_maxpool_fwd(R.S(p.s_stem_y), R.S(p.s_pool), (unsigned char*)R.S(p.s_argmax), N, stem.d.hout,
-                                    stem.d.wout, hp, wp, b.C, st);
+            pool_wrote_hl = dcn::launch_maxpool_fwd(R.S(p.s_stem_y), R.S(p.s_pool), (unsigned char*)R.S(p.s_argmax), N, stem.d.hout,
+                                                    stem.d.wout, hp, wp, b.C, st, nullptr, 1, nullptr, hl_img, hl_bound);
         }
     }
     if (hoist && !side.join_wait(p.ev_ws[1])) return DCN_E_LAUNCH;
     if (training && f16_mode && p.blocks[0].has_hl_in) {
         const BlockL& b0 = p.blocks[0];
         R.hl_saved.emplace_back(R.S(b0.in), R.S(b0.hl_in));
-        DCN_TRY(R.other([&] { return dcn_split_act_hl32(R.S(b0.in), R.A(b0.act_in), R.S(b0.hl_in), b0.in_rows, b0.in_c, st); }));
+        if (!pool_wrote_hl) DCN_TRY(R.other([&] { return dcn_split_act_hl32(R.S(b0.in), R.A(b0.act_in), R.S(b0.hl_in), b0.in_rows, b0.in_c, st); }));
     }
     for (const BlockL& blk : p.blocks) {
         const float* in = R.S(blk.in);
@@ -1143,11 +1143,13 @@
         const bool hl_d = prod && !fuse_red && routes[c.idx].dgrad == Kernel::HL;
         const bool hl_w = prod && routes[c.idx].wgrad == Kernel::HL;
         const bool want_blocked = f16 && !hl_w, want_hl = hl_d || hl_w;
+        const bool no_reader = dcn::tuning().resample_v2 != 0 && c.idx == p.convs[p.stem].idx && want_blocked &&
+                               routes[c.idx].wgrad == Kernel::F16;
         dcn::launch_bn_bwd({.dy = dy, .dy2 = dy2, .relu_out = relu_out, .relu_mask = mask, .x = R.S(c.x), .stats = R.S(b.stats),
                             .gamma = R.P(b.g), .C = b.C, .rows = b.rows, .groups = p.groups, .partial = part, .k123 = k123,
                             .reduced_tiles_per_group = tiles, .dgamma = grads[b.g], .dbeta = grads[b.b], .dx = dx, .g_out = g_out,
                             .absmax = f16 ? amax + c.idx : nullptr, .dq = want_blocked ? slot.blocked : nullptr,
-                            .hl_dx = want_hl ? slot.hl : nullptr, .skip_fp32_dx = hl_d,
+                            .hl_dx = want_hl ? slot.hl : nullptr, .skip_fp32_dx = hl_d, .no_fp32_reader = no_reader,
                             .lean = (overlap && dcn::tuning().bn_bwd_lean != 0) ? dcn::tuning().bn_bwd_lean_mask : 0}, st);
         img.wrote(want_blocked ? dx : nullptr, want_hl ? dx : nullptr);
     };
diff --git a/pytorch-dense-correspondence_amd/csrc/dcn_tuning.h b/pytorch-dense-correspondence_amd/csrc/dcn_tuning.h
--- a/pytorch-dense-correspondence_amd/csrc/dcn_tuning.h
+++ b/pytorch-dense-correspondence_amd/csrc/dcn_tuning.h
@@ -43,6 +43,7 @@
     int bn_bwd_lean = 1;
     int bn_bwd_lean_mask = 7;
     int bn_bwd_lean_depth = 3;
+    int resample_v2 = 1;
     int wgrad_roles = 1;
 };
 
diff --git a/pytorch-dense-correspondence_amd/csrc/dcn_tuning.hip b/pytorch-dense-correspondence_amd/csrc/dcn_tuning.hip
--- a/pytorch-dense-correspondence_amd/csrc/dcn_tuning.hip
+++ b/pytorch-dense-correspondence_amd/csrc/dcn_tuning.hip
@@ -71,6 +71,7 @@
     if (const char* e = getenv("DCN_BN_REDUCE_WIDE")) t.bn_reduce_wide = atoi(e);
     if (const char* e = getenv("DCN_BN_BWD_LEAN")) t.bn_bwd_lean = atoi(e) != 0;
     if (const char* e = getenv("DCN_BN_BWD_LEAN_MASK")) t.bn_bwd_lean_mask = atoi(e) & 7;
+    if (const char* e = getenv("DCN_RESAMPLE_V2")) t.resample_v2 = atoi(e) != 0;
     if (const char* e = getenv("DCN_BN_BWD_LEAN_DEPTH")) { const int v = atoi(e); t.bn_bwd_lean_depth = v < 1 ? 1 : (v > 3 ? 3 : v); }
 }
 
diff --git a/pytorch-dense-correspondence_amd/csrc/elementwise_kernels.h b/pytorch-dense-correspondence_amd/csrc/elementwise_kernels.h
--- a/pytorch-dense-correspondence_amd/csrc/elementwise_kernels.h
+++ b/pytorch-dense-correspondence_amd/csrc/elementwise_kernels.h
@@ -18,7 +18,8 @@
     ObservedLaunch& operator=(const ObservedLaunch&) = delete;
 };
 
-void launch_nchw3_to_nhwc4(const float* img, float* out, int n, int hw, float* absmax, hipStream_t st);
+void launch_nchw3_to_nhwc4(const float* img, float* out, int n, int hw, float* absmax, hipStream_t st,
+                           const float* img_b = nullptr);
 void launch_pad_c3_to_c4(const float* w, float* wp, int64_t rows, hipStream_t st);
 void launch_unpad_c4_to_c3(const float* wp, float* w, int64_t rows, hipStream_t st);
 void launch_pad_rows(const float* src, float* dst, int64_t rows, int d, int ld, hipStream_t st);
@@ -64,14 +65,15 @@
     void* dq = nullptr;
     void* hl_dx = nullptr;
     bool skip_fp32_dx = false;
+    bool no_fp32_reader = false;
     int lean = 0;
 };
 void launch_bn_bwd(const BnBwdArgs& a, hipStream_t st);
 void launch_add(const float* a, const float* b, float* out, int64_t n, hipStream_t st);
 
-void launch_maxpool_fwd(const float* in, float* out, unsigned char* argmax, int n, int hin, int win, int hout,
+bool launch_maxpool_fwd(const float* in, float* out, unsigned char* argmax, int n, int hin, int win, int hout,
                         int wout, int C, hipStream_t st, const float* bn_stats = nullptr, int groups = 1,
-                        unsigned char* relu_mask = nullptr);
+                        unsigned char* relu_mask = nullptr, void* hl_out = nullptr, const float* hl_absmax = nullptr);
 void launch_maxpool_bwd(const float* gout, const unsigned char* argmax, float* gin, int n, int hin, int win, int hout,
                         int wout, int C, hipStream_t st, const float* gout2 = nullptr);
 
diff --git a/pytorch-dense-correspondence_amd/csrc/elementwise_kernels.hip b/pytorch-dense-correspondence_amd/csrc/elementwise_kernels.hip
--- a/pytorch-dense-correspondence_amd/csrc/elementwise_kernels.hip
+++ b/pytorch-dense-correspondence_amd/csrc/elementwise_kernels.hip
@@ -928,16 +928,13 @@
     }
     tmp[i] = acc;
 }
-__global__ void __launch_bounds__(256)
-upsample_bwd_cols_kernel(const float* __restrict__ tmp, int hl, int wl, int ldl, int d, int w, float sw,
-                         float* __restrict__ glow, int64_t total) {
-    const int64_t i = (int64_t)blockIdx.x * 256 + threadIdx.x;
-    if (i >= total) return;
+__device__ __forceinline__ float upsample_bwd_cols_value(const float* __restrict__ tmp, int wl, int ldl, int d, int w, float sw,
+                                                         int64_t i) {
     const int k = (int)(i % ldl);
     const int64_t t = i / ldl;
     const int ix = (int)(t % wl);
     const int64_t row = t / wl;
-    if (k >= d) { glow[i] = 0.f; return; }
+    if (k >= d) return 0.f;
     const float inv = sw > 0.f ? 1.f / sw : 0.f;
     int xlo = (int)floorf(((float)ix - 1.f) * inv) - 1, xhi = (int)ceilf(((float)ix + 1.f) * inv) + 1;
     if (xlo < 0) xlo = 0;
@@ -952,7 +949,321 @@
         if (x1 == ix) wgt += lx;
         if (wgt != 0.f) acc = fmaf(wgt, tmp[(row * w + x) * d + k], acc);
     }
-    glow[i] = acc;
+    return acc;
+}
+__global__ void __launch_bounds__(256)
+upsample_bwd_cols_kernel(const float* __restrict__ tmp, int hl, int wl, int ldl, int d, int w, float sw,
+                         float* __restrict__ glow, int64_t total) {
+    const int64_t i = (int64_t)blockIdx.x * 256 + threadIdx.x;
+    if (i >= total) return;
+    glow[i] = upsample_bwd_cols_value(tmp, wl, ldl, d, w, sw, i);
+}
+
+
+__device__ __forceinline__ void block_atomic_absmax(float m, float* absmax) {
+    __shared__ float s_m[4];
+#pragma unroll
+    for (int o = 32; o > 0; o >>= 1) m = fmaxf(m, __shfl_xor(m, o));
+    if ((threadIdx.x & 63) == 0) s_m[threadIdx.x >> 6] = m;
+    __syncthreads();
+    if (threadIdx.x == 0) {
+        m = fmaxf(fmaxf(s_m[0], s_m[1]), fmaxf(s_m[2], s_m[3]));
+        const unsigned bits = __float_as_uint(m);
+        if (m > 0.f && bits > __atomic_load_n(reinterpret_cast<unsigned*>(absmax), __ATOMIC_RELAXED))
+            atomicMax(reinterpret_cast<unsigned*>(absmax), bits);
+    }
+}
+
+__global__ void __launch_bounds__(256)
+upsample_bwd_cols_v2_kernel(const float* __restrict__ tmp, int hl, int wl, int ldl, int d, int w, float sw,
+                            float* __restrict__ glow, int nq, int64_t total, float* __restrict__ absmax) {
+    const int64_t i = (int64_t)blockIdx.x * 256 + threadIdx.x;
+    float m = 0.f;
+    if (i < total) {
+        const int q = (int)(i % nq);
+        const int64_t t = i / nq;
+        const int ix = (int)(t % wl);
+        const int64_t row = t / wl;
+        const float inv = sw > 0.f ? 1.f / sw : 0.f;
+        int xlo = (int)floorf(((float)ix - 1.f) * inv) - 1, xhi = (int)ceilf(((float)ix + 1.f) * inv) + 1;
+        if (xlo < 0) xlo = 0;
+        if (xhi > w - 1 || sw <= 0.f) xhi = w - 1;
+        float acc[4] = {0.f, 0.f, 0.f, 0.f};
+        for (int x = xlo; x <= xhi; ++x) {
+            int x0, x1;
+            float lx;
+            src_index(x, sw, wl, x0, x1, lx);
+            float wgt = 0.f;
+            if (x0 == ix) wgt += 1.f - lx;
+            if (x1 == ix) wgt += lx;
+            if (wgt != 0.f) {
+                const float* src = tmp + (row * w + x) * d;
+#pragma unroll
+                for (int e = 0; e < 4; ++e)
+                    if (4 * q + e < d) acc[e] = fmaf(wgt, src[4 * q + e], acc[e]);
+            }
+        }
+#pragma unroll
+        for (int e = 0; e < 4; ++e) {
+            const int k = 4 * q + e;
+            if (k >= ldl) break;
+            const float v = k < d ? acc[e] : 0.f;
+            glow[t * ldl + k] = v;
+            m = fmaxf(m, fabsf(v));
+        }
+    }
+    if (absmax) block_atomic_absmax(m, absmax);
+}
+
+constexpr int kUpsRows = 64;
+template <bool VEC>
+__global__ void __launch_bounds__(256)
+upsample_bwd_rows_v2_kernel(const float* __restrict__ gout, const float* __restrict__ gout_b, int n_a, int hl, int h, int wd,
+                            float sh, float* __restrict__ tmp, int xblocks) {
+    __shared__ float s_w[kUpsRows];
+    const int row = blockIdx.x / xblocks, xb = blockIdx.x - row * xblocks;
+    const int n = row / hl, iy = row - n * hl;
+    const float* g = n < n_a ? gout + (int64_t)n * h * wd : gout_b + (int64_t)(n - n_a) * h * wd;
+    float* o = tmp + (int64_t)row * wd;
+    const int x = (xb * 256 + (int)threadIdx.x) * 4;
+    const float inv = sh > 0.f ? 1.f / sh : 0.f;
+    int ylo = (int)floorf(((float)iy - 1.f) * inv) - 1, yhi = (int)ceilf(((float)iy + 1.f) * inv) + 1;
+    if (ylo < 0) ylo = 0;
+    if (yhi > h - 1 || sh <= 0.f) yhi = h - 1;
+    float acc[4] = {0.f, 0.f, 0.f, 0.f};
+    for (int yc = ylo; yc <= yhi; yc += kUpsRows) {
+        const int cnt = yhi - yc + 1 < kUpsRows ? yhi - yc + 1 : kUpsRows;
+        __syncthreads();
+        if ((int)threadIdx.x < cnt) {
+            int y0, y1;
+            float ly;
+            src_index(yc + (int)threadIdx.x, sh, hl, y0, y1, ly);
+            float wgt = 0.f;
+            if (y0 == iy) wgt += 1.f - ly;
+            if (y1 == iy) wgt += ly;
+            s_w[threadIdx.x] = wgt;
+        }
+        __syncthreads();
+        if (x < wd) {
+            const float* gy = g + (int64_t)yc * wd + x;
+            for (int k = 0; k < cnt; ++k, gy += wd) {
+                const float wgt = s_w[k];
+                if (wgt == 0.f) continue;
+                if (VEC) {
+                    const float4 v = *reinterpret_cast<const float4*>(gy);
+                    acc[0] = fmaf(wgt, v.x, acc[0]); acc[1] = fmaf(wgt, v.y, acc[1]);
+                    acc[2] = fmaf(wgt, v.z, acc[2]); acc[3] = fmaf(wgt, v.w, acc[3]);
+                } else {
+#pragma unroll
+                    for (int e = 0; e < 4; ++e)
+                        if (x + e < wd) acc[e] = fmaf(wgt, gy[e], acc[e]);
+                }
+            }
+        }
+    }
+    if (x < wd) {
+        if (VEC) {
+            *reinterpret_cast<float4*>(o + x) = make_float4(acc[0], acc[1], acc[2], acc[3]);
+        } else {
+#pragma unroll
+            for (int e = 0; e < 4; ++e)
+                if (x + e < wd) o[x + e] = acc[e];
+        }
+    }
+}
+
+template <bool VEC>
+__global__ void __launch_bounds__(256)
+nchw3_to_nhwc4_v2_kernel(const float* __restrict__ img, const float* __restrict__ img_b, int n_a, float* __restrict__ out, int hw,
+                         int total, float* __restrict__ absmax) {
+    __shared__ float s_px[VEC ? 3 * 1024 : 1];
+    const int base = (int)blockIdx.x * 1024, t = (int)threadIdx.x;
+    float m = 0.f;
+    if (VEC) {
+        const int i = base + 4 * t;
+        if (i < total) {
+            const int n = i / hw, p = i - n * hw;
+            const float* s = (n < n_a ? img + (int64_t)n * 3 * hw : img_b + (int64_t)(n - n_a) * 3 * hw) + p;
+            reinterpret_cast<float4*>(s_px)[t] = *reinterpret_cast<const float4*>(s);
+            reinterpret_cast<float4*>(s_px + 1024)[t] = *reinterpret_cast<const float4*>(s + hw);
+            reinterpret_cast<float4*>(s_px + 2048)[t] = *reinterpret_cast<const float4*>(s + 2 * (int64_t)hw);
+        }
+        __syncthreads();
+    }
+#pragma unroll
+    for (int e = 0; e < 4; ++e) {
+        const int l = 256 * e + t, i = base + l;
+        if (i >= total) break;
+        float4 v;
+        if (VEC) {
+            v = make_float4(s_px[l], s_px[1024 + l], s_px[2048 + l], 0.f);
+        } else {
+            const int n = i / hw, p = i - n * hw;
+            const float* s = (n < n_a ? img + (int64_t)n * 3 * hw : img_b + (int64_t)(n - n_a) * 3 * hw) + p;
+            v = make_float4(s[0], s[hw], s[2 * (int64_t)hw], 0.f);
+        }
+        reinterpret_cast<float4*>(out)[i] = v;
+        m = fmaxf(m, fmaxf(fmaxf(fabsf(v.x), fabsf(v.y)), fabsf(v.z)));
+        if (v.x != v.x || v.y != v.y || v.z != v.z) m = __builtin_huge_valf();
+    }
+    if (absmax) block_atomic_absmax(m, absmax);
+}
+
+constexpr int kPoolTY = 2, kPoolTX = 2;
+__device__ __forceinline__ void pool_take(float v, int t, float& best, int& b) {
+    if (v > best || b < 0 || v != v) { best = v; b = t; }
+}
+template <bool BN>
+__global__ void __launch_bounds__(256)
+maxpool_fwd_v2_kernel(const float* __restrict__ in, float* __restrict__ out, unsigned char* __restrict__ argmax, int hin, int win,
+                      int hout, int wout, int c4n, int ystrips, int xblocks, int items, const float* __restrict__ scale,
+                      const float* __restrict__ shift, int gstride, int group_n, unsigned char* __restrict__ relu_mask,
+                      dcnsplit::u32x2* __restrict__ hl_out, const float* __restrict__ hl_absmax) {
+    const int row = blockIdx.x / xblocks, xb = blockIdx.x - row * xblocks;
+    const int n = row / ystrips, oy0 = (row - n * ystrips) * kPoolTY;
+    const int j = xb * 256 + (int)threadIdx.x;
+    if (j >= items) return;
+    const int q = j / c4n, c4 = j - q * c4n;
+    const int ox0 = q * kPoolTX;
+    const int64_t img = (int64_t)n * hin * win * c4n;
+    const float4* src = reinterpret_cast<const float4*>(in) + img;
+    float4 sc = make_float4(1.f, 1.f, 1.f, 1.f), sh = make_float4(0.f, 0.f, 0.f, 0.f);
+    if (BN) {
+        const int c = c4 * 4 + (n >= group_n ? gstride : 0);
+        sc = *reinterpret_cast<const float4*>(scale + c);
+        sh = *reinterpret_cast<const float4*>(shift + c);
+    }
+    const float hl_scale = hl_out ? dcnsplit::pow2_scale(*hl_absmax) : 1.f;
+    float4 best[kPoolTY][kPoolTX];
+    int bx[kPoolTY][kPoolTX], by[kPoolTY][kPoolTX], bz[kPoolTY][kPoolTX], bw[kPoolTY][kPoolTX];
+#pragma unroll
+    for (int ty = 0; ty < kPoolTY; ++ty)
+#pragma unroll
+        for (int tx = 0; tx < kPoolTX; ++tx) {
+            best[ty][tx] = make_float4(-INFINITY, -INFINITY, -INFINITY, -INFINITY);
+            bx[ty][tx] = by[ty][tx] = bz[ty][tx] = bw[ty][tx] = -1;
+        }
+#pragma unroll
+    for (int k = 0; k <= 2 * kPoolTY; ++k) {
+        const int iy = oy0 * 2 - 1 + k;
+        const bool row_in = iy >= 0 && iy < hin;
+        float4 v[2 * kPoolTX + 1];
+        bool ok[2 * kPoolTX + 1];
+#pragma unroll
+        for (int m = 0; m <= 2 * kPoolTX; ++m) {
+            const int ix = ox0 * 2 - 1 + m;
+            ok[m] = row_in && ix >= 0 && ix < win;
+            v[m] = make_float4(0.f, 0.f, 0.f, 0.f);
+            if (ok[m]) v[m] = src[(iy * win + ix) * c4n + c4];
+        }
+#pragma unroll
+        for (int m = 0; m <= 2 * kPoolTX; ++m) {
+            if (!ok[m]) continue;
+            float4 u = v[m];
+            if (BN) {
+                u = make_float4(u.x * sc.x + sh.x, u.y * sc.y + sh.y, u.z * sc.z + sh.z, u.w * sc.w + sh.w);
+                u.x = fmaxf(u.x, 0.f); u.y = fmaxf(u.y, 0.f); u.z = fmaxf(u.z, 0.f); u.w = fmaxf(u.w, 0.f);
+                if (k >= 1 && m >= 1 && relu_mask)
+                    relu_mask[img + (iy * win + (ox0 * 2 - 1 + m)) * c4n + c4] =
+                        (unsigned char)((u.x > 0.f ? 1 : 0) | (u.y > 0.f ? 2 : 0) | (u.z > 0.f ? 4 : 0) | (u.w > 0.f ? 8 : 0));
+            }
+#pragma unroll
+            for (int ty = 0; ty < kPoolTY; ++ty) {
+                const int r = k - 2 * ty;
+                if (r < 0 || r > 2) continue;
+#pragma unroll
+                for (int tx = 0; tx < kPoolTX; ++tx) {
+                    const int s = m - 2 * tx;
+                    if (s < 0 || s > 2) continue;
+                    const int t = r * 3 + s;
+                    pool_take(u.x, t, best[ty][tx].x, bx[ty][tx]);
+                    pool_take(u.y, t, best[ty][tx].y, by[ty][tx]);
+                    pool_take(u.z, t, best[ty][tx].z, bz[ty][tx]);
+                    pool_take(u.w, t, best[ty][tx].w, bw[ty][tx]);
+                }
+            }
+        }
+    }
+#pragma unroll
+    for (int ty = 0; ty < kPoolTY; ++ty) {
+        const int oy = oy0 + ty;
+        if (oy >= hout) continue;
+#pragma unroll
+        for (int tx = 0; tx < kPoolTX; ++tx) {
+            const int ox = ox0 + tx;
+            if (ox >= wout) continue;
+            const int64_t o = (int64_t)n * hout * wout * c4n + ((oy * wout + ox) * c4n + c4);
+            reinterpret_cast<float4*>(out)[o] = best[ty][tx];
+            if (argmax)
+                reinterpret_cast<unsigned*>(argmax)[o] = (unsigned)bx[ty][tx] | ((unsigned)by[ty][tx] << 8) |
+                                                         ((unsigned)bz[ty][tx] << 16) | ((unsigned)bw[ty][tx] << 24);
+            if (hl_out) {
+                dcnsplit::h4 hi, lo;
+                dcnsplit::split4(best[ty][tx], hl_scale, hi, lo);
+                const int64_t unit = ((int64_t)n * hout * wout + (oy * wout + ox)) * (c4n >> 1) + (c4 >> 1);
+                dcnsplit::u32x2* line = hl_out + ((unit >> 2) * 8 + (unit & 3)) * 2 + (c4 & 1);
+                line[0] = __builtin_bit_cast(dcnsplit::u32x2, hi);
+                line[8] = __builtin_bit_cast(dcnsplit::u32x2, lo);
+            }
+        }
+    }
+}
+
+__global__ void __launch_bounds__(256)
+maxpool_bwd_v2_kernel(const float* __restrict__ gout, const float* __restrict__ gout2, const unsigned char* __restrict__ argmax,
+                      float* __restrict__ gin, int hin, int win, int hout, int wout, int c4n, int xblocks, int items) {
+    const int row = blockIdx.x / xblocks, xb = blockIdx.x - row * xblocks;
+    const int n = row / hout, a = row - n * hout;
+    const int j = xb * 256 + (int)threadIdx.x;
+    if (j >= items) return;
+    const int q = j / c4n, c4 = j - q * c4n;
+    const int64_t obase = (int64_t)n * hout * wout * c4n;
+    float4 g[2][3];
+    unsigned am[2][3];
+#pragma unroll
+    for (int dy = 0; dy < 2; ++dy)
+#pragma unroll
+        for (int dx = 0; dx < 3; ++dx) {
+            const int oy = a + dy, ox = 2 * q + dx;
+            g[dy][dx] = make_float4(0.f, 0.f, 0.f, 0.f);
+            am[dy][dx] = 0xFFFFFFFFu;
+            if (oy < hout && ox < wout) {
+                const int64_t o = obase + ((oy * wout + ox) * c4n + c4);
+                g[dy][dx] = reinterpret_cast<const float4*>(gout)[o];
+                if (gout2) {
+                    const float4 h = reinterpret_cast<const float4*>(gout2)[o];
+                    g[dy][dx].x += h.x; g[dy][dx].y += h.y; g[dy][dx].z += h.z; g[dy][dx].w += h.w;
+                }
+                am[dy][dx] = reinterpret_cast<const unsigned*>(argmax)[o];
+            }
+        }
+#pragma unroll
+    for (int ry = 0; ry < 2; ++ry) {
+        const int iy = 2 * a + ry;
+        if (iy >= hin) continue;
+#pragma unroll
+        for (int cx = 0; cx < 4; ++cx) {
+            const int ix = 4 * q + cx;
+            if (ix >= win) continue;
+            float4 acc = make_float4(0.f, 0.f, 0.f, 0.f);
+#pragma unroll
+            for (int dy = 0; dy < 2; ++dy) {
+                const int r = ry - 2 * dy + 1;
+                if (r < 0 || r > 2) continue;
+#pragma unroll
+                for (int dx = 0; dx < 3; ++dx) {
+                    const int s = cx - 2 * dx + 1;
+                    if (s < 0 || s > 2) continue;
+                    const unsigned t = (unsigned)(r * 3 + s), w4 = am[dy][dx];
+                    if ((w4 & 0xFFu) == t) acc.x += g[dy][dx].x;
+                    if (((w4 >> 8) & 0xFFu) == t) acc.y += g[dy][dx].y;
+                    if (((w4 >> 16) & 0xFFu) == t) acc.z += g[dy][dx].z;
+                    if ((w4 >> 24) == t) acc.w += g[dy][dx].w;
+                }
+            }
+            reinterpret_cast<float4*>(gin)[(int64_t)n * hin * win * c4n + ((iy * win + ix) * c4n + c4)] = acc;
+        }
+    }
 }
 
 static inline unsigned blocks_for(int64_t n, int cap = 0) {
@@ -965,10 +1276,26 @@
 
 thread_local const LaunchObserver* launch_observer = nullptr;
 
-void launch_nchw3_to_nhwc4(const float* img, float* out, int n, int hw, float* absmax, hipStream_t st) {
+static inline bool aligned16(const void* p) { return (reinterpret_cast<uintptr_t>(p) & 15) == 0; }
+constexpr int64_t kV2MaxElems = (int64_t)1 << 30;
+
+void launch_nchw3_to_nhwc4(const float* img, float* out, int n, int hw, float* absmax, hipStream_t st, const float* img_b) {
     const int64_t total = (int64_t)n * hw;
-    ObservedLaunch obs(DCN_PROF_RESAMPLE, 28.0 * (double)total, st);
-    hipLaunchKernelGGL(nchw3_to_nhwc4_kernel, dim3(blocks_for(total, kGridCap)), dim3(256), 0, st, img, out, hw, total, absmax);
+    if (tuning().resample_v2 && total <= kV2MaxElems) {
+        ObservedLaunch obs(DCN_PROF_RESAMPLE, 28.0 * (double)total, st);
+        const bool vec = (hw & 3) == 0 && aligned16(img) && aligned16(img_b) && aligned16(out);
+        const int n_a = img_b ? n / 2 : n;
+        auto layout_v2_kernel = vec ? nchw3_to_nhwc4_v2_kernel<true> : nchw3_to_nhwc4_v2_kernel<false>;
+        hipLaunchKernelGGL(layout_v2_kernel, dim3((unsigned)ceil_div64(total, 1024)), dim3(256), 0, st, img, img_b, n_a, out, hw, (int)total, absmax);
+        return;
+    }
+    const int halves = img_b ? 2 : 1;
+    const int64_t th = total / halves;
+    for (int k = 0; k < halves; ++k) {
+        ObservedLaunch obs(DCN_PROF_RESAMPLE, 28.0 * (double)th, st);
+        hipLaunchKernelGGL(nchw3_to_nhwc4_kernel, dim3(blocks_for(th, kGridCap)), dim3(256), 0, st, k ? img_b : img, out + k * th * 4,
+                           hw, th, absmax);
+    }
 }
 void launch_pad_c3_to_c4(const float* w, float* wp, int64_t rows, hipStream_t st) {
     ObservedLaunch obs(DCN_PROF_OTHER, 28.0 * (double)rows, st);
@@ -1019,7 +1346,7 @@
     void* hl = (a.hl_dx && (C % 32) == 0) ? a.hl_dx : nullptr;
     void* dq = a.dq;
     const bool blocked = (dq || hl) && absmax;
-    float* dx = (blocked && hl && a.skip_fp32_dx) ? nullptr : a.dx;
+    float* dx = (blocked && ((hl && a.skip_fp32_dx) || a.no_fp32_reader)) ? nullptr : a.dx;
     int chunks = a.reduced_tiles_per_group;
     const int depth = tuning().bn_bwd_lean_depth;
     const bool deep = depth > 1 && !(relu_out && !relu_mask) && C <= 512 && groups <= 2;
@@ -1074,19 +1401,38 @@
     ObservedLaunch obs(DCN_PROF_OTHER, 12.0 * (double)n, st);
     hipLaunchKernelGGL(add_kernel, dim3(blocks_for(n / 4, kGridCap)), dim3(256), 0, st, a, b, out, n / 4);
 }
-void launch_maxpool_fwd(const float* in, float* out, unsigned char* argmax, int n, int hin, int win, int hout,
-                        int wout, int C, hipStream_t st, const float* bn_stats, int groups, unsigned char* relu_mask) {
+bool launch_maxpool_fwd(const float* in, float* out, unsigned char* argmax, int n, int hin, int win, int hout,
+                        int wout, int C, hipStream_t st, const float* bn_stats, int groups, unsigned char* relu_mask,
+                        void* hl_out, const float* hl_absmax) {
     const int64_t total4 = (int64_t)n * hout * wout * (C / 4);
     ObservedLaunch obs(DCN_PROF_RESAMPLE, (double)n * C * ((double)hin * win * (4.0 + (bn_stats && relu_mask ? 0.25 : 0.0)) +
                                                           (double)hout * wout * (4.0 + (argmax ? 1.0 : 0.0))), st);
+    if (tuning().resample_v2 && (int64_t)n * hin * win * C <= kV2MaxElems && aligned16(argmax)) {
+        const int c4n = C / 4, ystrips = ceil_div(hout, kPoolTY), items = ceil_div(wout, kPoolTX) * c4n, xblocks = ceil_div(items, 256);
+        const float* shift = bn_stats ? bn_stats + C : nullptr;
+        const int group_n = groups > 1 ? n / groups : n;
+        void* hl = (hl_out && hl_absmax && (C % 32) == 0) ? hl_out : nullptr;
+        auto maxpool_fwd_v2 = bn_stats ? maxpool_fwd_v2_kernel<true> : maxpool_fwd_v2_kernel<false>;
+        hipLaunchKernelGGL(maxpool_fwd_v2, dim3((unsigned)(n * ystrips * xblocks)),
+                           dim3(256), 0, st, in, out, argmax, hin, win, hout, wout, c4n, ystrips, xblocks, items, bn_stats, shift,
+                           4 * C, group_n, bn_stats ? relu_mask : nullptr, (dcnsplit::u32x2*)hl, hl_absmax);
+        return hl != nullptr;
+    }
     hipLaunchKernelGGL(maxpool_fwd_kernel, dim3(blocks_for(total4)), dim3(256), 0, st, in, out, argmax, hin, win, hout,
                        wout, C / 4, total4, bn_stats, bn_stats ? bn_stats + C : nullptr, 4 * C,
                        (int64_t)(groups > 1 ? n / groups : n), bn_stats ? relu_mask : nullptr);
+    return false;
 }
 void launch_maxpool_bwd(const float* gout, const unsigned char* argmax, float* gin, int n, int hin, int win, int hout,
                         int wout, int C, hipStream_t st, const float* gout2) {
     const int64_t total4 = (int64_t)n * hin * win * (C / 4);
     ObservedLaunch obs(DCN_PROF_RESAMPLE, (double)n * C * ((double)hin * win * 4.0 + (double)hout * wout * (5.0 + (gout2 ? 4.0 : 0.0))), st);
+    if (tuning().resample_v2 && total4 * 4 <= kV2MaxElems && aligned16(argmax)) {
+        const int c4n = C / 4, items = ceil_div(win, 4) * c4n, xblocks = ceil_div(items, 256);
+        hipLaunchKernelGGL(maxpool_bwd_v2_kernel, dim3((unsigned)(n * hout * xblocks)), dim3(256), 0, st, gout, gout2, argmax, gin, hin,
+                           win, hout, wout, c4n, xblocks, items);
+        return;
+    }
     hipLaunchKernelGGL(maxpool_bwd_kernel, dim3(blocks_for(total4)), dim3(256), 0, st, gout, gout2, argmax, gin, hin, win,
                        hout, wout, C / 4, total4);
 }
@@ -1109,6 +1455,23 @@
 void launch_upsample_bwd(const float* gout, int n, int hl, int wl, int ldl, int d, int h, int w, float* tmp,
                          float* glow, float* absmax, hipStream_t st, const float* gout_b) {
     const int64_t t1 = (int64_t)n * hl * w * d;
+    const int64_t t2 = (int64_t)n * hl * wl * ldl;
+    if (tuning().resample_v2 && (int64_t)n * h * w * d <= kV2MaxElems && t2 <= kV2MaxElems) {
+        const int wd = w * d, xblocks = ceil_div(wd, 1024);
+        const bool vec = (wd & 3) == 0 && aligned16(gout) && aligned16(gout_b) && aligned16(tmp);
+        {
+            ObservedLaunch obs(DCN_PROF_RESAMPLE, 4.0 * ((double)n * h * w * d + (double)t1), st);
+            auto upsample_bwd_rows_v2 = vec ? upsample_bwd_rows_v2_kernel<true> : upsample_bwd_rows_v2_kernel<false>;
+            hipLaunchKernelGGL(upsample_bwd_rows_v2, dim3((unsigned)(n * hl * xblocks)), dim3(256), 0, st, gout, gout_b, gout_b ? n / 2 : n, hl, h, wd,
+                               ac_scale(hl, h), tmp, xblocks);
+        }
+        ObservedLaunch obs(DCN_PROF_RESAMPLE, 4.0 * ((double)t1 + (double)t2), st);
+        const int nq = ceil_div(ldl, 4);
+        const int64_t items = (int64_t)n * hl * wl * nq;
+        hipLaunchKernelGGL(upsample_bwd_cols_v2_kernel, dim3(blocks_for(items)), dim3(256), 0, st, (const float*)tmp, hl, wl, ldl, d, w,
+                           ac_scale(wl, w), glow, nq, items, absmax);
+        return;
+    }
     if (gout_b) {
         const int64_t th = t1 / 2;
         for (int k = 0; k < 2; ++k) {
@@ -1121,7 +1484,6 @@
         hipLaunchKernelGGL(upsample_bwd_rows_kernel, dim3(blocks_for(t1)), dim3(256), 0, st, gout, hl, d, h, w,
                            ac_scale(hl, h), tmp, t1);
     }
-    const int64_t t2 = (int64_t)n * hl * wl * ldl;
     {
         ObservedLaunch obs(DCN_PROF_RESAMPLE, 4.0 * ((double)t1 + (double)t2), st);
         hipLaunchKernelGGL(upsample_bwd_cols_kernel, dim3(blocks_for(t2)), dim3(256), 0, st, (const float*)tmp, hl, wl, ldl,
@@ -1213,13 +1575,13 @@
     if ((dq || hl_dx) && !absmax) return DCN_E_INVALID;
     if (hl_dx && (c % 32) != 0) return DCN_E_INVALID;
     if (blocked && groups == 2 && ((rows / groups) % 4) != 0) return DCN_E_INVALID;
-    if (!dx && !(hl_dx && !keep_dx)) return DCN_E_INVALID;
+    if (!dx && !(hl_dx && !keep_dx) && !(blocked && keep_dx < 0)) return DCN_E_INVALID;
     float* partial = (float*)workspace;
     float* k123 = partial + (size_t)groups * dcn::bn_bwd_chunks(rows / groups) * 4 * c;
     dcn::launch_bn_bwd({.dy = dy, .dy2 = dy2, .relu_out = relu_out, .relu_mask = relu_mask, .x = x, .stats = stats, .gamma = gamma,
                         .C = c, .rows = rows, .groups = groups, .partial = partial, .k123 = k123, .dgamma = dgamma, .dbeta = dbeta,
                         .dx = dx, .g_out = g_out, .absmax = absmax, .dq = dq, .hl_dx = hl_dx, .skip_fp32_dx = !keep_dx,
-                        .lean = standalone_lean()}, (hipStream_t)stream);
+                        .no_fp32_reader = keep_dx < 0, .lean = standalone_lean()}, (hipStream_t)stream);
     return dcn::check_launch();
 }
 
@@ -1247,6 +1609,21 @@
     return dcn::check_launch();
 }
 
+extern "C" int dcn_maxpool_forward_hl(const float* in, const float* bn_stats, int groups, int n, int hin, int win, int c,
+                                      float* out, unsigned char* argmax, unsigned char* relu_mask, void* hl_out,
+                                      const float* hl_absmax, void* stream) {
+    if (!in || !out || n < 1 || hin < 1 || win < 1 || c < 32 || (c % 32) != 0 || !hl_out || !hl_absmax) return DCN_E_INVALID;
+    if ((groups != 1 && groups != 2) || (n % groups) != 0) return DCN_E_INVALID;
+    if (relu_mask && !bn_stats) return DCN_E_INVALID;
+    const int hout = (hin + 2 - 3) / 2 + 1, wout = (win + 2 - 3) / 2 + 1;
+    if (!dcn::launch_maxpool_fwd(in, out, argmax, n, hin, win, hout, wout, c, (hipStream_t)stream, bn_stats, groups, relu_mask, hl_out,
+                                 hl_absmax)) {
+        const int rc = dcn_split_act_hl32(out, hl_absmax, hl_out, (int64_t)n * hout * wout, c, stream);
+        if (rc != 0) return rc;
+    }
+    return dcn::check_launch();
+}
+
 extern "C" int dcn_maxpool_backward_full(const float* gout, const float* gout2, const unsigned char* argmax, int n, int hin,
                                          int win, int c, float* gin, void* stream) {
     if (!gout || !argmax || !gin || n < 1 || hin < 1 || win < 1 || c < 4 || (c % 4) != 0) return DCN_E_INVALID;
@@ -1276,6 +1653,14 @@
     return dcn::check_launch();
 }
 
+extern "C" int dcn_image_pair_to_nhwc4(const float* img, const float* img_b, int n, int hw, float* out, float* absmax,
+                                       void* stream) {
+    if (!img || !out || n < 1 || hw < 1) return DCN_E_INVALID;
+    if (img_b && (n % 2) != 0) return DCN_E_INVALID;
+    dcn::launch_nchw3_to_nhwc4(img, out, n, hw, absmax, (hipStream_t)stream, img_b);
+    return dcn::check_launch();
+}
+
 extern "C" int dcn_pad_c3_to_c4(const float* src, float* dst, int64_t rows, void* stream) {
     if (!src || !dst || rows < 1) return DCN_E_INVALID;
     dcn::launch_pad_c3_to_c4(src, dst, rows, (hipStream_t)stream);
diff --git a/pytorch-dense-correspondence_amd/dcn_hip/_lib.py b/pytorch-dense-correspondence_amd/dcn_hip/_lib.py
--- a/pytorch-dense-correspondence_amd/dcn_hip/_lib.py
+++ b/pytorch-dense-correspondence_amd/dcn_hip/_lib.py
@@ -176,10 +176,13 @@
     "dcn_upsample_backward_tmp_bytes": (c_size_t, [c_int, c_int, c_int, c_int]),
     "dcn_maxpool_forward_full": (c_int, [c_void_p, c_void_p, c_int, c_int, c_int, c_int, c_int, c_void_p, c_void_p, c_void_p,
                                          c_void_p]),
+    "dcn_maxpool_forward_hl": (c_int, [c_void_p, c_void_p, c_int, c_int, c_int, c_int, c_int, c_void_p, c_void_p, c_void_p,
+                                       c_void_p, c_void_p, c_void_p]),
     "dcn_maxpool_backward_full": (c_int, [c_void_p, c_void_p, c_void_p, c_int, c_int, c_int, c_int, c_void_p, c_void_p]),
     "dcn_normalize_backward": (c_int, [c_void_p] + [c_int] * 7 + [c_void_p, c_void_p, c_void_p]),
     "dcn_upsample_backward_full": (c_int, [c_void_p, c_void_p] + [c_int] * 7 + [c_void_p] * 4),
     "dcn_image_to_nhwc4": (c_int, [c_void_p, c_int, c_int, c_void_p, c_void_p, c_void_p]),
+    "dcn_image_pair_to_nhwc4": (c_int, [c_void_p, c_void_p, c_int, c_int, c_void_p, c_void_p, c_void_p]),
     "dcn_pad_c3_to_c4": (c_int, [c_void_p, c_void_p, c_int64, c_void_p]),
     "dcn_unpad_c4_to_c3": (c_int, [c_void_p, c_void_p, c_int64, c_void_p]),
     "dcn_pad_rows": (c_int, [c_void_p, c_void_p, c_int64, c_int, c_int, c_void_p]),
```

New measurement: 468.3 (median of 6 runs). No clear change (+0.7%).
